# Orbiter-Finance/Plonky2-lib

Hardware: AMD Instinct MI355X
Metric: proofs/sec for secp256k1 ECDSA-verify circuit; Goldilocks NTT GB/s vs HBM peak (higher is better)
Workload: dtype u64 (Goldilocks, 64-bit modular integer)

## Files before the change

### plonky2-lib_amd/csrc/prover.hip

```cpp
#include <algorithm>
#include <string.h>
#include "batch.h"
#include "common.h"
#include "merkle.h"
#include "ntt.h"
#include "poseidon.h"
#include "prover_types.h"

namespace {
void make_layout(const glp_circuit_desc &c, Layout &L) {
    const u32 cap = 1u << c.cap_height, nch = c.num_challenges;
    memset(&L, 0, sizeof(L));
    L.oracle_cols[0] = c.num_constants + c.num_routed_wires;
    L.oracle_cols[1] = c.num_wires;
    L.oracle_cols[2] = nch * (1 + c.num_partial_products);
    L.oracle_cols[3] = nch * c.quotient_degree_factor;
    L.nopen = (size_t)c.num_constants + c.num_routed_wires + c.num_wires + 2 * nch + nch * c.num_partial_products +
              nch * c.quotient_degree_factor;
    L.openings = 3 * (size_t)cap * 4;
    L.fri_caps = L.openings + 2 * L.nopen;
    L.queries = L.fri_caps + (size_t)c.num_reductions * cap * 4;
    const u32 lgN = c.degree_bits + c.rate_bits;
    L.depth0 = lgN - c.cap_height;
    size_t q = 0;
// ... 113 lines not shown
            const u32 col = (u32)chunk < a.npp ? nch + c * a.npp + chunk : c;
            const size_t o = (size_t)col * n + i;
            const u64 v = mul(a.zp[o], ipd);
            a.zp[o] = v;
            if ((u32)chunk == a.npp) rowp[(size_t)c * n + i] = v;
            ipd = mul(ipd, dn[(size_t)chunk * n]);
        }
    }
    __syncthreads();
    if (threadIdx.x < nch) {
        const u32 c = threadIdx.x;
        u64 acc = 1;
        for (u32 i = 0; i < n; i++) { const u64 r = rowp[(size_t)c * n + i]; zrow[(size_t)c * n + i] = acc; acc = mul(acc, r); }
    }
    __syncthreads();
    for (u32 u = threadIdx.x; u < units; u += 256) {
        const u32 i = u % n, k = (u / n) % nchunks, c = u / (n * nchunks);
        const u64 z = zrow[(size_t)c * n + i];
        if (k < a.npp) { const size_t o = (size_t)(nch + c * a.npp + k) * n + i; a.zp[o] = mul(a.zp[o], z); }
        else a.zp[(size_t)c * n + i] = z;
    }
}
__global__ __launch_bounds__(256) void k_pp_block_tot(const u64 *zp, u64 *tot, u32 lg, u32 nblocks, size_t zp_stride) {
    __shared__ u64 sh[256];
    zp += (size_t)blockIdx.z * zp_stride; tot += (size_t)blockIdx.z * gridDim.y * nblocks;
    const size_t n = (size_t)1 << lg;
    const u32 c = blockIdx.y, b = blockIdx.x, t = threadIdx.x;
    const size_t i = (size_t)b * 256 + t;
    sh[t] = i < n ? zp[(size_t)c * n + i] : 1;
    __syncthreads();
    for (int s = 128; s > 0; s >>= 1) { if (t < s) sh[t] = mul(sh[t], sh[t + s]); __syncthreads(); }
    if (t == 0) tot[(size_t)c * nblocks + b] = sh[0];
}
__global__ __launch_bounds__(256) void k_pp_scan_tot(u64 *tot, u32 nblocks) {
    __shared__ u64 sh[256];
    const u32 c = blockIdx.x, t = threadIdx.x;
    u64 *v = tot + ((size_t)blockIdx.y * gridDim.x + c) * nblocks;
    const u32 m = (nblocks + 255) / 256;
    u64 loc = 1;
    for (u32 k = t * m; k < min((t + 1) * m, nblocks); k++) loc = mul(loc, v[k]);
    sh[t] = loc;
    __syncthreads();
    if (t == 0) { u64 acc = 1; for (int k = 0; k < 256; k++) { u64 x = sh[k]; sh[k] = acc; acc = mul(acc, x); } }
    __syncthreads();
    u64 acc = sh[t];
    for (u32 k = t * m; k < min((t + 1) * m, nblocks); k++) { u64 x = v[k]; v[k] = acc; acc = mul(acc, x); }
}
__global__ __launch_bounds__(256) void k_pp_apply(u64 *zp, const u64 *tot, u32 lg, u32 nblocks, u32 nch, u32 npp, size_t zp_stride) {
    __shared__ u64 sh[2][256];
    zp += (size_t)blockIdx.z * zp_stride; tot += (size_t)blockIdx.z * gridDim.y * nblocks;
    const size_t n = (size_t)1 << lg;
    const u32 c = blockIdx.y, b = blockIdx.x, t = threadIdx.x;
    const size_t i = (size_t)b * 256 + t;
    const u64 mine = i < n ? zp[(size_t)c * n + i] : 1;
    int cur = 0;
    sh[0][t] = mine;
    __syncthreads();
    for (int off = 1; off < 256; off <<= 1) {
        u64 v = sh[cur][t];
        if (t >= off) v = mul(sh[cur][t - off], v);
        sh[cur ^ 1][t] = v;
        cur ^= 1;
        __syncthreads();
    }
    const u64 excl = t ? sh[cur][t - 1] : 1;
    if (i >= n) return;
    const u64 z = mul(tot[(size_t)c * nblocks + b], excl);
    zp[(size_t)c * n + i] = z;
    for (u32 k = 0; k < npp; k++) {
        const size_t o = (size_t)(nch + c * npp + k) * n + i;
        zp[o] = mul(zp[o], z);
    }
}

__device__ __forceinline__ u64 range_product(u64 v, u32 bound) {
    if (bound == 4) {
        const u64 u = mul_nc(v, add_cnc(v, P - 3));
        return mul_nc(u, add_cnc(2, u));
    }
    u64 p = v;
    for (u32 x = 1; x + 1 < bound; x++) p = mul(p, sub(v, (u64)x));
    return bound > 1 ? mul_nc(p, sub(v, (u64)(bound - 1))) : p;
}
struct Base4Sum { u64 lo, hi; };
__device__ __forceinline__ void b4_zero(Base4Sum &b) { b.lo = 0; b.hi = 0; }
__device__ __forceinline__ void b4_add(Base4Sum &b, u64 limb, u32 j ) {
    const u32 w = 1u << (2 * j);
    b.lo += (u64)(u32)limb * w;
    b.hi += (u64)(u32)(limb >> 32) * w;
}
__device__ __forceinline__ u64 b4_value(const Base4Sum &b) {
    const u64 l = b.lo + (b.hi << 32);
    const u32 h = (u32)(b.hi >> 32) + (l < b.lo ? 1u : 0u);
    return canon(fold96_nc(l, h));
}
struct Acc160 { u32 w0, w1, w2, w3, w4; };
__device__ __forceinline__ void acc_zero(Acc160 &a) { a.w0 = a.w1 = a.w2 = a.w3 = a.w4 = 0; }
__device__ __forceinline__ void acc_fma(Acc160 &a, u64 v, u64 m) {
    const u32 v0 = (u32)v, v1 = (u32)(v >> 32), m0 = (u32)m, m1 = (u32)(m >> 32);
    const u64 p00 = (u64)v0 * m0;
    const u64 p01 = (u64)v0 * m1 + (p00 >> 32);
    const u64 p10 = (u64)v1 * m0 + (u32)p01;
    const u64 p11 = (u64)v1 * m1 + (p01 >> 32) + (p10 >> 32);
    u32 c;
    a.w0 = __builtin_addc(a.w0, (u32)p00, 0u, &c);
    a.w1 = __builtin_addc(a.w1, (u32)p10, c, &c);
    a.w2 = __builtin_addc(a.w2, (u32)p11, c, &c);
    a.w3 = __builtin_addc(a.w3, (u32)(p11 >> 32), c, &c);
    a.w4 += c;
}
__device__ __forceinline__ u64 acc_reduce(const Acc160 &a) {
    const u64 h = fold96_nc(((u64)a.w3 << 32) | a.w2, a.w4);
    return canon(fold128_nc(a.w0, a.w1, (u32)h, (u32)(h >> 32)));
}

constexpr u32 ACC_MAX_TERMS = 1024;
struct AccLimb { u64 a00, a01, a10, a11, a20, a21; };
__device__ __forceinline__ void acc2_zero(AccLimb &a) { a.a00 = a.a01 = a.a10 = a.a11 = a.a20 = a.a21 = 0; }
__device__ __forceinline__ void acc2_fma(AccLimb &a, u32 v0, u32 v1, u32 v2, u64 m) {
    const u32 m0 = (u32)m, m1 = (u32)(m >> 32);
    a.a00 += (u64)v0 * m0; a.a01 += (u64)v0 * m1;
    a.a10 += (u64)v1 * m0; a.a11 += (u64)v1 * m1;
    a.a20 += (u64)v2 * m0; a.a21 += (u64)v2 * m1;
}
template <int E> __device__ __forceinline__ void acc_add_shifted(Acc160 &w, u64 x) {
    constexpr int idx = E / 32, sh = E % 32;
    const u64 lo = x << sh;
    const u32 t0 = (u32)lo, t1 = (u32)(lo >> 32);
    u32 t2 = 0;
    if constexpr (sh != 0) t2 = (u32)(x >> (64 - sh));
    u32 *W[5] = {&w.w0, &w.w1, &w.w2, &w.w3, &w.w4};
    u32 c;
    *W[idx] = __builtin_addc(*W[idx], t0, 0u, &c);
    *W[idx + 1] = __builtin_addc(*W[idx + 1], t1, c, &c);
    *W[idx + 2] = __builtin_addc(*W[idx + 2], t2, c, &c);
    if constexpr (idx + 3 < 5) *W[idx + 3] = __builtin_addc(*W[idx + 3], 0u, c, &c);
    if constexpr (idx + 4 < 5) *W[idx + 4] = __builtin_addc(*W[idx + 4], 0u, c, &c);
}
__device__ __forceinline__ u64 acc2_reduce(const AccLimb &a) {
    Acc160 w;
    acc_zero(w);
    acc_add_shifted<0>(w, a.a00); acc_add_shifted<22>(w, a.a10); acc_add_shifted<32>(w, a.a01);
    acc_add_shifted<44>(w, a.a20); acc_add_shifted<54>(w, a.a11); acc_add_shifted<76>(w, a.a21);
    return acc_reduce(w);
}

struct AccHL { u64 c0, c1, c2; };
constexpr u32 ACC3_MAX_TERMS = 512;
inline void apl_words(u64 m, u64 out[4]) {
    const u64 mp = glf::mul(m, 1ull << 32);
    out[0] = (m & 0x3FFFFFull) | (((m >> 22) & 0x3FFFFFull) << 32); out[1] = m >> 44;
    out[2] = (mp & 0x3FFFFFull) | (((mp >> 22) & 0x3FFFFFull) << 32); out[3] = mp >> 44;
}
__device__ __forceinline__ void acc3_zero(AccHL &a) { a.c0 = a.c1 = a.c2 = 0; }
__device__ __forceinline__ void acc3_fma(AccHL &a, u64 v, const u64 *ml) {
    const u32 vlo = (u32)v, vhi = (u32)(v >> 32);
    const u64 w0 = ml[0], w1 = ml[1], w2 = ml[2], w3 = ml[3];
    a.c0 += (u64)vlo * (u32)w0; a.c1 += (u64)vlo * (u32)(w0 >> 32); a.c2 += (u64)vlo * (u32)w1;
    a.c0 += (u64)vhi * (u32)w2; a.c1 += (u64)vhi * (u32)(w2 >> 32); a.c2 += (u64)vhi * (u32)w3;
}
__device__ __forceinline__ u64 acc3_reduce(const AccHL &a) {
    Acc160 w;
    acc_zero(w);
    acc_add_shifted<0>(w, a.c0); acc_add_shifted<22>(w, a.c1); acc_add_shifted<44>(w, a.c2);
    return acc_reduce(w);
}

struct QArgs {
    const u64 *cs;
    const DevGate *gates;
    const u64 *k_is;
    u64 shift_r[MAXR], zh[MAXR], zh_inv[MAXR];
    u64 w_n, n_field;
    u32 lg, rb, step, nc, nsel, nr, nw, nch, npp, qdf, num_gates, nterms, many_selectors, gate_mode;
    u32 k_ratio;
    const u64 *l0;
};
struct QProof {
    const u64 *wl, *zl;
    u64 *out;
    const u64 *apow;
    const u64 *apl;
    u64 betas[MAXCH], gammas[MAXCH], pih[4];
};
struct QBatch { const u64 *pp; size_t wl_stride, zl_stride, out_stride, apow_stride; };
static_assert(MAXCH == 4, "pp layout: 4 betas, 4 gammas, 4 words of the public-input hash");
__device__ __forceinline__ QProof q_proof(const QProof &p0, const QBatch &b) {
    QProof p = p0;
    if (b.pp) {
        const size_t k = blockIdx.z;
        p.wl += k * b.wl_stride; p.zl += k * b.zl_stride; p.out += k * b.out_stride; p.apow += k * b.apow_stride; p.apl += APL_WORDS * k * b.apow_stride;
        const u64 *q = b.pp + k * 3 * MAXCH;
        _Pragma("unroll") for (int c = 0; c < MAXCH; c++) { p.betas[c] = q[c]; p.gammas[c] = q[MAXCH + c]; p.pih[c] = q[2 * MAXCH + c]; }
    }
    return p;
}
__global__ __launch_bounds__(256) void k_l0_table(QArgs a, u64 *out, u32 Rq) {
    const size_t n = (size_t)1 << a.lg;
    const size_t q = (size_t)blockIdx.x * 256 + threadIdx.x;
    if (q >= n) return;
    const u64 wq = dpow(a.w_n, q);
    u64 d[MAXR], pre[MAXR];
    u64 run = 1;
    for (u32 rq = 0; rq < Rq; rq++) {
        d[rq] = mul(a.n_field, sub(mul(a.shift_r[rq], wq), 1));
        pre[rq] = run;
        run = mul(run, d[rq]);
    }
    u64 iv = inv(run);
    for (int rq = (int)Rq - 1; rq >= 0; rq--) {
        out[(size_t)rq * n + q] = mul(a.zh[rq], mul(iv, pre[rq]));
        iv = mul(iv, d[rq]);
    }
}
__device__ __forceinline__ u64 gate_filter(const QArgs &a, const DevGate &g, size_t N, size_t slot) {
    const u64 s = a.cs[(size_t)g.selector_index * N + slot];
    u64 filter = 1;
    for (u32 i = g.group_start; i < g.group_end; i++)
        if (i != g.row) filter = mul(filter, sub((u64)i, s));
    if (a.many_selectors) filter = mul(filter, sub(0xFFFFFFFFull, s));
    return filter;
}
template <int NCH, int TYPE, bool HEAD_ONLY = false>
__device__ __forceinline__ void gate_terms(const QArgs &a, const QProof &p, const DevGate &g, size_t N, size_t slot, u32 k0, AccHL (&ga)[MAXCH]) {
    const u32 nt = a.nterms;
    const u64 *W = p.wl + slot;
    const u64 *GC = a.cs + (size_t)a.nsel * N + slot;
    {
        const u64 *ap = p.apl + APL_WORDS * (size_t)k0;
#define EMIT(k, v)                                                                     \
    do {                                                                               \
        const u64 _v = (v);                                                            \
        _Pragma("unroll") for (int c2 = 0; c2 < NCH; c2++) acc3_fma(ga[c2], _v, ap + APL_WORDS * ((size_t)c2 * nt + (k)));   \
    } while (0)
#define LIMBS4_DESC(LIMBS, COUNT, SPLIT, KIDX, ACCLO, ACCHI)                                                      \
    {                                                                                                             \
        Base4Sum _slo, _shi;                                                                                      \
        b4_zero(_slo); b4_zero(_shi);                                                                             \
        for (int _j0 = (int)(COUNT); _j0 > 0; _j0 -= 8) {                                                         \
            u64 _lv[8];                                                                                            \
            _Pragma("unroll") for (int _t = 0; _t < 8; _t++) if (_t < _j0) _lv[_t] = (LIMBS)[(size_t)(_j0 - 1 - _t) * N]; \
            _Pragma("unroll") for (int _t = 0; _t < 8; _t++) if (_t < _j0) {                                      \
                const int _j = _j0 - 1 - _t;                                                                      \
                EMIT((KIDX), range_product(_lv[_t], 4));                                                           \
                if (_j < (int)(SPLIT)) b4_add(_slo, _lv[_t], (u32)_j); else b4_add(_shi, _lv[_t], (u32)(_j - (int)(SPLIT))); \
            }                                                                                                     \
        }                                                                                                         \
        ACCLO = b4_value(_slo);                                                                                   \
        if ((int)(COUNT) > (int)(SPLIT)) ACCHI = b4_value(_shi);                                                  \
    }
        switch (TYPE >= 0 ? (u32)TYPE : g.type) {
        case GLP_GATE_CONSTANT:
            for (u32 i = 0; i < g.p0; i++) EMIT(i, sub(GC[(size_t)i * N], W[(size_t)i * N]));
            break;
        case GLP_GATE_PUBLIC_INPUT:
            for (u32 i = 0; i < 4; i++) EMIT(i, sub(W[(size_t)i * N], p.pih[i]));
            break;
        case GLP_GATE_ARITHMETIC: {
            const u64 c0 = GC[0], c1 = GC[N];
            for (u32 i = 0; i < g.p0; i++) {
                const u64 m0 = W[(size_t)(4 * i) * N], m1 = W[(size_t)(4 * i + 1) * N];
                const u64 ad = W[(size_t)(4 * i + 2) * N], o = W[(size_t)(4 * i + 3) * N];
                EMIT(i, sub(o, add(mul(mul(m0, m1), c0), mul(ad, c1))));
            }
            break;
        }
        case GLP_GATE_POSEIDON: {
#if defined(__HIP_DEVICE_COMPILE__)
            u32 k = 0;
            u64 st[12];
            const u64 swap = W[(size_t)24 * N];
            EMIT(k, mul_nc(swap, sub(swap, 1))); k++;
            for (u32 i = 0; i < 4; i++) {
                const u64 lhs = W[(size_t)i * N], rhs = W[(size_t)(i + 4) * N], dl = W[(size_t)(25 + i) * N];
                EMIT(k, sub(mul(swap, sub(rhs, lhs)), dl)); k++;
                st[i] = add(lhs, dl); st[i + 4] = sub(rhs, dl);
            }
            for (u32 i = 8; i < 12; i++) st[i] = W[(size_t)i * N];
            for (u32 i = 0; i < 12; i++) st[i] = add(st[i], pos::RC[i]);
            pos::sbox_layer_nc(st);
            pos::mds_add_nc(st, pos::RCN.k[0]);
            for (u32 r = 1; r < 4; r++) {
                for (u32 i = 0; i < 12; i++) { const u64 in = W[(size_t)(29 + 12 * (r - 1) + i) * N]; EMIT(k, add_cnc(neg(in), st[i])); k++; st[i] = in; }
                pos::sbox_layer_nc(st);
                if (r < 3) pos::mds_add_nc(st, pos::RCN.k[r]);
            }
            u32 pr = 0;
            auto wire_in = [&](int j, u64 z) {
                const u64 in = W[(size_t)(65 + pr + (u32)j) * N];
                EMIT(k, add_cnc(neg(in), z)); k++;
                return in;
            };
            pos::partial_block_nc<3, true>(st, pos::PBM[0], wire_in); pr += 3;
            for (int b = 0; b < 4; b++) { pos::partial_block_nc<4, false>(st, pos::PB4[b], wire_in); pr += 4; }
            pos::partial_block_nc<3, false>(st, pos::PB3[0], wire_in);
            for (u32 r = 0; r < 4; r++) {
                for (u32 i = 0; i < 12; i++) { const u64 in = W[(size_t)(87 + 12 * r + i) * N]; EMIT(k, add_cnc(neg(in), st[i])); k++; st[i] = in; }
                pos::sbox_layer_nc(st);
                pos::mds_add_nc(st, r < 3 ? pos::RCN.k[4 + r] : pos::RC_ZERO);
            }
            for (u32 i = 0; i < 12; i++) { EMIT(k, add_cnc(neg(W[(size_t)(12 + i) * N]), st[i])); k++; }
#endif
            break;
        }
        case GLP_GATE_U32_INTERLEAVE: {
            u32 k = 0;
            for (u32 i = 0; i < g.p0; i++) {
                const u64 xw = W[(size_t)(2 * i) * N], xi = W[(size_t)(2 * i + 1) * N];
                const u64 *bits = W + (size_t)(2 * g.p0 + 32 * i) * N;
                u64 cx = 0, cxi = 0;
                const u32 kb = k + 2;
                for (u32 b = 0; b < 32; b++) {
                    const u64 bit = bits[(size_t)b * N];
                    cx = add(dbl(cx), bit);
                    cxi = add(dbl(dbl(cxi)), bit);
                    EMIT(kb + b, mul_nc(bit, sub(bit, 1)));
                }
                EMIT(k, sub(cx, xw));
                EMIT(k + 1, sub(cxi, xi));
                k += 34;
            }
            break;
        }
        case GLP_GATE_UNINTERLEAVE_U32:
        case GLP_GATE_UNINTERLEAVE_B32: {
            u32 k = 0;
            for (u32 i = 0; i < g.p0; i++) {
                const u64 xi = W[(size_t)(3 * i) * N], xe = W[(size_t)(3 * i + 1) * N], xo = W[(size_t)(3 * i + 2) * N];
                const u64 *bits = W + (size_t)(3 * g.p0 + 64 * i) * N;
                u64 cxi = 0, ce = 0, co = 0;
                const u32 kb = k + 3;
                for (u32 j = 0; j < 32; j++) {
                    const u64 be = bits[(size_t)(2 * j) * N], bo = bits[(size_t)(2 * j + 1) * N];
                    cxi = add(dbl(add(dbl(cxi), be)), bo);
                    if (g.type == GLP_GATE_UNINTERLEAVE_U32) { ce = add(dbl(ce), be); co = add(dbl(co), bo); }
                    else { ce = add(dbl(dbl(ce)), be); co = add(dbl(dbl(co)), bo); }
                    EMIT(kb + 2 * j, mul_nc(be, sub(be, 1)));
                    EMIT(kb + 2 * j + 1, mul_nc(bo, sub(bo, 1)));
                }
                EMIT(k, sub(cxi, xi));
                EMIT(k + 1, sub(ce, xe));
                EMIT(k + 2, sub(co, xo));
                k += 67;
            }
// ... 142 lines not shown
                        l2[q4] = add(f0, mul(b1, sub(f1, f0)));
                    }
                    const u64 g0 = add(l2[0], mul(b2, sub(l2[1], l2[0]))), g1 = add(l2[2], mul(b2, sub(l2[3], l2[2])));
                    sel = add(g0, mul(b3, sub(g1, g0)));
                } else {
                    for (u32 b = 0; b < bits; b++) { const u64 bit = bw[(size_t)b * N]; EMIT(k, mul_nc(bit, sub(bit, 1))); k++; }
                    for (int b = (int)bits - 1; b >= 0; b--) idx = add(dbl(idx), bw[(size_t)b * N]);
                    EMIT(k, sub(idx, bse[0])); k++;
                    sel = 0;
                    for (u32 j = 0; j < vs; j++) {
                        u64 ind = 1;
                        for (u32 b = 0; b < bits; b++) { const u64 bit = bw[(size_t)b * N]; ind = mul(ind, ((j >> b) & 1) ? bit : sub(1, bit)); }
                        sel = add(sel, mul(ind, bse[(size_t)(2 + j) * N]));
                    }
                }
                EMIT(k, sub(sel, bse[N])); k++;
            }
            for (u32 e = 0; e < nextra; e++) { EMIT(k, sub(GC[(size_t)e * N], W[(size_t)((2 + vs) * copies + e) * N])); k++; }
            break;
        }
        default: break;
        }
#undef LIMBS4_DESC
#undef EMIT
    }
}
template <int NCH, int TYPE>
__device__ __forceinline__ void gate_contrib(const QArgs &a, const QProof &p, const DevGate &g, size_t N, size_t slot, u32 k0, u64 (&acc)[MAXCH]) {
    const u64 filter = gate_filter(a, g, N, slot);
    AccHL ga[MAXCH];
    _Pragma("unroll") for (int c = 0; c < NCH; c++) acc3_zero(ga[c]);
    gate_terms<NCH, TYPE, false>(a, p, g, N, slot, k0, ga);
    _Pragma("unroll") for (int c = 0; c < NCH; c++) acc[c] = add(acc[c], mul(filter, acc3_reduce(ga[c])));
}

struct LightArgs { u32 count; u32 gi[8]; u32 arith_gi, arith_ops; };
template <int NCH>
__device__ __forceinline__ void light_gates(const QArgs &a, const QProof &p, const LightArgs &la, size_t N, size_t slot, u32 k0, u64 (&acc)[MAXCH]) {
    for (u32 t = 0; t < la.count; t++) {
        const DevGate g = a.gates[la.gi[t]];
        switch (g.type) {
        case GLP_GATE_CONSTANT: gate_contrib<NCH, GLP_GATE_CONSTANT>(a, p, g, N, slot, k0, acc); break;
        case GLP_GATE_PUBLIC_INPUT: gate_contrib<NCH, GLP_GATE_PUBLIC_INPUT>(a, p, g, N, slot, k0, acc); break;
        case GLP_GATE_ARITHMETIC: gate_contrib<NCH, GLP_GATE_ARITHMETIC>(a, p, g, N, slot, k0, acc); break;
        case GLP_GATE_BASE_SUM: gate_contrib<NCH, GLP_GATE_BASE_SUM>(a, p, g, N, slot, k0, acc); break;
        case GLP_GATE_RANDOM_ACCESS: gate_contrib<NCH, GLP_GATE_RANDOM_ACCESS>(a, p, g, N, slot, k0, acc); break;
        default: break;
        }
    }
}
template <int NCH, int GATES>
__global__ __launch_bounds__(256, GATES == 1 ? 3 : 4) void k_quotient(QArgs a, QProof p0, QBatch qb, LightArgs la) {
    const QProof p = q_proof(p0, qb);
    const size_t n = (size_t)1 << a.lg, N = n << a.rb;
    const size_t q = (size_t)blockIdx.x * 256 + threadIdx.x;
    if (q >= n) return;
    const u32 rq = blockIdx.y, r = rq * a.step;
    const size_t slot = (size_t)r * n + q, slot_next = (size_t)r * n + ((q + 1) & (n - 1));
    const u64 x = mul(a.shift_r[rq], dpow(a.w_n, q));
    constexpr u32 nch = NCH; const u32 nchunks = a.npp + 1, nt = a.nterms;
    u64 acc[MAXCH], zx[MAXCH], zg[MAXCH];
    Acc160 pa[MAXCH];
    _Pragma("unroll") for (int c = 0; c < NCH; c++) { acc_zero(pa[c]); zx[c] = p.zl[(size_t)c * N + slot]; zg[c] = p.zl[(size_t)c * N + slot_next]; }
    const u64 l0 = a.l0[(size_t)rq * n + q];
    _Pragma("unroll") for (int c = 0; c < NCH; c++) {
        const u64 t = mul(l0, sub(zx[c], 1));
        _Pragma("unroll") for (int c2 = 0; c2 < NCH; c2++) acc_fma(pa[c2], t, p.apow[c2 * nt + c]);
    }
    u64 bkx[MAXCH];
    _Pragma("unroll") for (int c = 0; c < NCH; c++) bkx[c] = mul_nc(p.betas[c], x);
    const u32 k0 = nch + nch * nchunks;
    const u32 ar_ops = GATES == 2 ? la.arith_ops : 0;
    AccHL gar[MAXCH];
    u64 ar_c0 = 0, ar_c1 = 0;
    if (GATES == 2) {
        _Pragma("unroll") for (int c = 0; c < NCH; c++) acc3_zero(gar[c]);
        if (ar_ops) { ar_c0 = a.cs[(size_t)a.nsel * N + slot]; ar_c1 = a.cs[(size_t)(a.nsel + 1) * N + slot]; }
    }
    for (u32 chunk = 0; chunk < nchunks; chunk++) {
        u64 num[MAXCH], den[MAXCH];
        _Pragma("unroll") for (int c = 0; c < NCH; c++) { num[c] = 1; den[c] = 1; }
        const u32 j0 = chunk * a.qdf, j1 = min((chunk + 1) * a.qdf, a.nr);
        for (u32 jb = j0; jb < j1; jb += 8) {
            u64 w8[8], s8[8];
#pragma unroll
            for (int t = 0; t < 8; t++)
                if (jb + t < j1) { w8[t] = p.wl[(size_t)(jb + t) * N + slot]; s8[t] = a.cs[(size_t)(a.nc + jb + t) * N + slot]; }
            if (GATES == 2 && ar_ops) {
#pragma unroll
                for (int t = 0; t < 8; t += 4)
                    if (jb + t + 3 < j1 && (jb + t) / 4 < ar_ops) {
                        const u32 i = (jb + t) / 4;
                        const u64 v = sub(w8[t + 3], add(mul(mul(w8[t], w8[t + 1]), ar_c0), mul(w8[t + 2], ar_c1)));
                        _Pragma("unroll") for (int c2 = 0; c2 < NCH; c2++) acc3_fma(gar[c2], v, p.apl + APL_WORDS * ((size_t)c2 * nt + k0 + i));
                    }
            }
#pragma unroll
            for (int t = 0; t < 8; t++)
                if (jb + t < j1) {
                    u64 kx = 0;
                    if (!a.k_ratio) kx = mul_nc(a.k_is[jb + t], x);
                    _Pragma("unroll") for (int c = 0; c < NCH; c++) {
                        const u64 wg = add(w8[t], p.gammas[c]);
                        const u64 bk = a.k_ratio ? bkx[c] : mul_nc(p.betas[c], kx);
                        num[c] = mul_nc_cc(num[c], add_cnc(wg, bk));
                        den[c] = mul_nc_cc(den[c], add_cnc(wg, mul_nc_cc(p.betas[c], s8[t])));
                        if (a.k_ratio) bkx[c] = mul_small_nc(bkx[c], a.k_ratio);
                    }
                }
        }
        _Pragma("unroll") for (int c = 0; c < NCH; c++) {
            const u64 prev = chunk == 0 ? zx[c] : p.zl[(size_t)(nch + c * a.npp + chunk - 1) * N + slot];
            const u64 next = chunk == nchunks - 1 ? zg[c] : p.zl[(size_t)(nch + c * a.npp + chunk) * N + slot];
            const u64 t = sub(mul(prev, num[c]), mul(next, den[c]));
            const u32 k = nch + c * nchunks + chunk;
            _Pragma("unroll") for (int c2 = 0; c2 < NCH; c2++) acc_fma(pa[c2], t, p.apow[c2 * nt + k]);
        }
    }
    _Pragma("unroll") for (int c = 0; c < NCH; c++) acc[c] = acc_reduce(pa[c]);
    if (GATES == 2 && ar_ops) {
        const u64 filter = gate_filter(a, a.gates[la.arith_gi], N, slot);
        _Pragma("unroll") for (int c = 0; c < NCH; c++) acc[c] = add(acc[c], mul(filter, acc3_reduce(gar[c])));
    }
    if constexpr (GATES == 1) {
        for (u32 gi = 0; gi < a.num_gates; gi++) {
            const DevGate g = a.gates[gi];
            gate_contrib<NCH, -1>(a, p, g, N, slot, k0, acc);
        }
    }
    if constexpr (GATES == 2) light_gates<NCH>(a, p, la, N, slot, k0, acc);
    const size_t Rq = (size_t)gridDim.y;
    _Pragma("unroll") for (int c = 0; c < NCH; c++) p.out[((size_t)c * Rq + rq) * n + q] = mul(acc[c], a.zh_inv[rq]);
}

template <int NCH, int TYPE>
__global__ __launch_bounds__(256) void k_quotient_gate(QArgs a, QProof p0, QBatch qb, u32 gi) {
    const QProof p = q_proof(p0, qb);
    const size_t n = (size_t)1 << a.lg, N = n << a.rb;
    const size_t q = (size_t)blockIdx.x * 256 + threadIdx.x;
    if (q >= n) return;
    const u32 rq = blockIdx.y, r = rq * a.step;
    const size_t slot = (size_t)r * n + q;
    u64 acc[MAXCH];
    _Pragma("unroll") for (int c = 0; c < NCH; c++) acc[c] = 0;
    const DevGate g = a.gates[gi];
    gate_contrib<NCH, TYPE>(a, p, g, N, slot, (u32)NCH + (u32)NCH * (a.npp + 1), acc);
    const size_t Rq = (size_t)gridDim.y;
    _Pragma("unroll") for (int c = 0; c < NCH; c++) {
        u64 *o = p.out + ((size_t)c * Rq + rq) * n + q;
        *o = add(*o, mul(acc[c], a.zh_inv[rq]));
    }
}

constexpr int LIMB_SLOTS = 5, LIMB_GROUPS = 4;
struct LimbArgs { const u64 *desc; u32 groups, num_wires; u32 count[LIMB_GROUPS], jlo[LIMB_GROUPS], jhi[LIMB_GROUPS]; u32 gi[LIMB_GROUPS][LIMB_SLOTS]; u32 extra_count, extra_gi[4]; };
inline void limb_args(const glp_circuit *cc, LimbArgs &la) {
    la.desc = cc->dev_limb_desc; la.groups = cc->limb_groups; la.num_wires = cc->d.num_wires;
    for (int g = 0; g < LIMB_GROUPS; g++) {
        la.count[g] = cc->limb_gcount[g]; la.jlo[g] = cc->limb_jlo[g]; la.jhi[g] = cc->limb_jhi[g];
        for (int i = 0; i < LIMB_SLOTS; i++) la.gi[g][i] = cc->limb_gi[g * LIMB_SLOTS + i];
    }
}
template <int NCH>
__global__ __launch_bounds__(256, 2) void k_quotient_limbs(QArgs a, QProof p0, QBatch qb, LimbArgs la) {
    const QProof p = q_proof(p0, qb);
    const size_t n = (size_t)1 << a.lg, N = n << a.rb;
    const size_t q = (size_t)blockIdx.x * 256 + threadIdx.x;
    if (q >= n) return;
    const u32 rq = blockIdx.y, r = rq * a.step;
    const size_t slot = (size_t)r * n + q;
    const u32 k0 = (u32)NCH + (u32)NCH * (a.npp + 1), nt = a.nterms;
    const u64 *W = p.wl + slot;
    const u64 *ap = p.apl + APL_WORDS * (size_t)k0;
    u64 acc[MAXCH];
    _Pragma("unroll") for (int c = 0; c < NCH; c++) acc[c] = 0;
#define LIMB_EMIT(S, K, V)                                                                                     \
    do {                                                                                                       \
        const u64 _v = (V);                                                                                    \
        _Pragma("unroll") for (int c2 = 0; c2 < NCH; c2++) acc3_fma(ga[S][c2], _v, ap + APL_WORDS * ((size_t)c2 * nt + (K)));   \
    } while (0)
#pragma unroll 1
    for (u32 grp = 0; grp < la.groups; grp++) {
        const u32 gcount = la.count[grp], jlo = la.jlo[grp], jhi = la.jhi[grp];
        const u64 *desc = la.desc + (size_t)grp * la.num_wires * LIMB_SLOTS;
        AccHL ga[LIMB_SLOTS][MAXCH];
        Base4Sum bs[LIMB_SLOTS];
        _Pragma("unroll") for (int s = 0; s < LIMB_SLOTS; s++) {
            b4_zero(bs[s]);
            _Pragma("unroll") for (int c = 0; c < NCH; c++) acc3_zero(ga[s][c]);
        }
        _Pragma("unroll") for (int s = 0; s < LIMB_SLOTS; s++) {
            if ((u32)s < gcount) {
                const DevGate g = a.gates[la.gi[grp][s]];
                switch (g.type) {
                case GLP_GATE_U32_ARITHMETIC: gate_terms<NCH, GLP_GATE_U32_ARITHMETIC, true>(a, p, g, N, slot, k0, ga[s]); break;
                case GLP_GATE_U32_ADD_MANY: gate_terms<NCH, GLP_GATE_U32_ADD_MANY, true>(a, p, g, N, slot, k0, ga[s]); break;
                case GLP_GATE_U32_SUBTRACTION: gate_terms<NCH, GLP_GATE_U32_SUBTRACTION, true>(a, p, g, N, slot, k0, ga[s]); break;
                default: break;
                }
            }
        }
        for (u32 j0 = jlo; j0 <= jhi; j0 += 8) {
            u64 lv[8];
            _Pragma("unroll") for (int t = 0; t < 8; t++) if (j0 + t <= jhi) lv[t] = W[(size_t)(j0 + t) * N];
            _Pragma("unroll") for (int t = 0; t < 8; t++) if (j0 + t <= jhi) {
                const u64 v = lv[t];
                const u64 *dj = desc + (size_t)(j0 + t) * LIMB_SLOTS;
                const u64 rp = range_product(v, 4);
                _Pragma("unroll") for (int s = 0; s < LIMB_SLOTS; s++) {
                    const u64 d = dj[s];
                    if (d & 1) {
                        const u32 kl = (u32)(d >> 6) & 0x3FFu;
                        _Pragma("unroll") for (int c2 = 0; c2 < NCH; c2++) acc3_fma(ga[s][c2], rp, ap + APL_WORDS * ((size_t)c2 * nt + kl));
                        b4_add(bs[s], v, (u32)(d >> 1) & 15u);
                        if (d & 32) {
                            const u32 kf = (u32)(d >> 16) & 0x3FFu, ref = (u32)(d >> 26) & 0xFFu;
                            LIMB_EMIT(s, kf, sub(b4_value(bs[s]), W[(size_t)ref * N]));
                            b4_zero(bs[s]);
                        }
                    }
                }
            }
        }
        _Pragma("unroll") for (int s = 0; s < LIMB_SLOTS; s++) {
            if ((u32)s < gcount) {
                const u64 filter = gate_filter(a, a.gates[la.gi[grp][s]], N, slot);
                _Pragma("unroll") for (int c = 0; c < NCH; c++) acc[c] = add(acc[c], mul(filter, acc3_reduce(ga[s][c])));
            }
        }
    }
#undef LIMB_EMIT
    for (u32 t = 0; t < la.extra_count; t++) {
        const DevGate g = a.gates[la.extra_gi[t]];
        if (g.type == GLP_GATE_COMPARISON) gate_contrib<NCH, GLP_GATE_COMPARISON>(a, p, g, N, slot, k0, acc);
    }
    const size_t Rq = (size_t)gridDim.y;
    _Pragma("unroll") for (int c = 0; c < NCH; c++) {
        u64 *o = p.out + ((size_t)c * Rq + rq) * n + q;
        *o = add(*o, mul(acc[c], a.zh_inv[rq]));
    }
}

struct QCArgs { const u64 *V; u64 *out; u64 wM_inv, wR_inv, g_inv, rq_inv; u64 gn_inv_pow[MAXR]; u32 lg, Rq; };
__global__ __launch_bounds__(256) void k_quotient_combine(QCArgs a) {
    const size_t n = (size_t)1 << a.lg;
    const size_t p = (size_t)blockIdx.x * 256 + threadIdx.x;
    if (p >= n) return;
    const u32 ch = blockIdx.y, Rq = a.Rq;
    const u32 kp = bitrev32((u32)p, a.lg);
    const u64 tw = dpow(a.wM_inv, kp);
    const u64 gk = mul(dpow(a.g_inv, kp), a.rq_inv);
    u64 y[MAXR];
    u64 t = 1;
    for (u32 r = 0; r < Rq; r++) { y[r] = mul(a.V[((size_t)ch * Rq + r) * n + p], t); t = mul(t, tw); }
    u64 wc = 1;
    for (u32 c = 0; c < Rq; c++) {
        u64 s = 0, w = 1;
        for (u32 r = 0; r < Rq; r++) { s = add(s, mul(y[r], w)); w = mul(w, wc); }
        a.out[((size_t)ch * Rq + c) * n + p] = mul(s, mul(gk, a.gn_inv_pow[c]));
        wc = mul(wc, a.wR_inv);
    }
}

struct ZTArgs { u64 *zt; ext2 zp2[24]; u32 lg; const u64 *zeta_b; size_t zeta_stride; };
template <bool BATCH>
__global__ __launch_bounds__(256) void k_zeta_table(ZTArgs a) {
    const size_t n = (size_t)1 << a.lg;
    const size_t p = (size_t)blockIdx.x * 256 + threadIdx.x;
    if (p >= n) return;
    const u32 k = bitrev32((u32)p, a.lg);
    ext2 acc = e_from(1);
    if constexpr (BATCH) {
        const u64 *z = a.zeta_b + (size_t)blockIdx.y * a.zeta_stride;
        ext2 sq = e_make(z[0], z[1]);
        for (u32 b = 0; b < a.lg; b++) { if ((k >> b) & 1) acc = e_mul(acc, sq); sq = e_sqr(sq); }
        a.zt += (size_t)blockIdx.y * 2 * n;
    } else {
        for (u32 b = 0; b < a.lg; b++) if ((k >> b) & 1) acc = e_mul(acc, a.zp2[b]);
    }
    a.zt[2 * p] = acc.a; a.zt[2 * p + 1] = acc.b;
}
constexpr int OPEN_BLOCKS = 32;
inline u32 open_blocks(size_t n) { return (u32)std::max<size_t>(1, std::min<size_t>(OPEN_BLOCKS, n / 256)); }
__global__ __launch_bounds__(256) void k_open_dot(const u64 *coeffs, const u64 *zt, u64 *partial, u32 lg, size_t coeffs_bstride,
                                                  size_t zt_bstride, size_t partial_bstride) {
    __shared__ u64 sa[256], sb[256];
    coeffs += (size_t)blockIdx.z * coeffs_bstride; zt += (size_t)blockIdx.z * zt_bstride; partial += (size_t)blockIdx.z * partial_bstride;
    const size_t n = (size_t)1 << lg;
    const u32 col = blockIdx.y, t = threadIdx.x;
    u64 a = 0, b = 0;
    AccLimb xa, xb;
    acc2_zero(xa); acc2_zero(xb);
    u32 terms = 0;
    for (size_t p = (size_t)blockIdx.x * 256 + t; p < n; p += (size_t)gridDim.x * 256) {
        const u64 c = coeffs[(size_t)col * n + p];
        const u32 c0 = (u32)c & 0x3FFFFFu, c1 = (u32)(c >> 22) & 0x3FFFFFu, c2 = (u32)(c >> 44);
        acc2_fma(xa, c0, c1, c2, zt[2 * p]);
        acc2_fma(xb, c0, c1, c2, zt[2 * p + 1]);
        if (++terms == ACC_MAX_TERMS) {
            a = add(a, acc2_reduce(xa)); b = add(b, acc2_reduce(xb));
            acc2_zero(xa); acc2_zero(xb); terms = 0;
        }
    }
    a = add(a, acc2_reduce(xa)); b = add(b, acc2_reduce(xb));
    sa[t] = a; sb[t] = b;
    __syncthreads();
    for (int s = 128; s > 0; s >>= 1) { if (t < s) { sa[t] = add(sa[t], sa[t + s]); sb[t] = add(sb[t], sb[t + s]); } __syncthreads(); }
    if (t == 0) { partial[2 * ((size_t)col * gridDim.x + blockIdx.x)] = sa[0]; partial[2 * ((size_t)col * gridDim.x + blockIdx.x) + 1] = sb[0]; }
}

struct FVArgs {
    const u64 *lde[4]; u32 ncols[4];
    const u64 *apow;
    u64 *out;
    ext2 red0, red1, zeta, zeta_next, shift_acc;
    u64 w_n, g;
    u32 lg, rb, nch;
    const u64 *pp;
    size_t lde_stride[4], apow_stride, out_stride;
};
__global__ __launch_bounds__(256) void k_final_values(FVArgs a) {
    const size_t n = (size_t)1 << a.lg, N = n << a.rb;
    const size_t q = (size_t)blockIdx.x * 256 + threadIdx.x;
    if (q >= n) return;
    if (a.pp) {
        const size_t pk = blockIdx.y;
        const u64 *v = a.pp + pk * 10;
        a.red0 = e_make(v[0], v[1]); a.red1 = e_make(v[2], v[3]); a.zeta = e_make(v[4], v[5]); a.zeta_next = e_make(v[6], v[7]);
        a.shift_acc = e_make(v[8], v[9]);
        _Pragma("unroll") for (int k = 0; k < 4; k++) a.lde[k] += pk * a.lde_stride[k];
        a.apow += pk * a.apow_stride; a.out += pk * a.out_stride;
    }
    ext2 acc0 = e_from(0), acc1 = e_from(0);
    AccLimb xa, xb;
    acc2_zero(xa); acc2_zero(xb);
    u32 j = 0, terms = 0;
    for (int k = 0; k < 4; k++) {
        const u64 *l = a.lde[k] + q;
        for (u32 c = 0; c < a.ncols[k]; c++, j++) {
            const u64 v = l[(size_t)c * N];
            const u32 v0 = (u32)v & 0x3FFFFFu, v1 = (u32)(v >> 22) & 0x3FFFFFu, v2 = (u32)(v >> 44);
            acc2_fma(xa, v0, v1, v2, a.apow[2 * j]);
            acc2_fma(xb, v0, v1, v2, a.apow[2 * j + 1]);
            if (++terms == ACC_MAX_TERMS) {
                acc0 = e_add(acc0, e_make(acc2_reduce(xa), acc2_reduce(xb)));
                acc2_zero(xa); acc2_zero(xb); terms = 0;
            }
            if (k == 2 && c < a.nch) {
                const ext2 ap1 = e_make(a.apow[2 * c], a.apow[2 * c + 1]);
                acc1 = e_add(acc1, e_scale(ap1, v));
            }
        }
    }
    acc0 = e_add(acc0, e_make(acc2_reduce(xa), acc2_reduce(xb)));
    const u64 x = mul(a.g, dpow(a.w_n, q));
    const ext2 d0 = e_inv(e_sub(e_from(x), a.zeta)), d1 = e_inv(e_sub(e_from(x), a.zeta_next));
    ext2 f = e_mul(e_mul(e_sub(acc0, a.red0), d0), a.shift_acc);
    f = e_add(f, e_mul(e_sub(acc1, a.red1), d1));
    a.out[q] = f.a; a.out[n + q] = f.b;
}

__global__ __launch_bounds__(256) void k_final_values_small(FVArgs a) {
    const u32 n = 1u << a.lg, lpp = 256u >> a.lg;
    const size_t N = (size_t)n << a.rb;
    const u32 q = threadIdx.x / lpp, t = threadIdx.x % lpp;
    if (a.pp) {
        const size_t pk = blockIdx.y;
        const u64 *v = a.pp + pk * 10;
        a.red0 = e_make(v[0], v[1]); a.red1 = e_make(v[2], v[3]); a.zeta = e_make(v[4], v[5]); a.zeta_next = e_make(v[6], v[7]);
        a.shift_acc = e_make(v[8], v[9]);
        _Pragma("unroll") for (int k = 0; k < 4; k++) a.lde[k] += pk * a.lde_stride[k];
        a.apow += pk * a.apow_stride; a.out += pk * a.out_stride;
    }
    ext2 acc0 = e_from(0), acc1 = e_from(0);
    AccLimb xa, xb;
    acc2_zero(xa); acc2_zero(xb);
    u32 base = 0;
    for (int k = 0; k < 4; k++) {
        const u64 *l = a.lde[k] + q;
        for (u32 c = t; c < a.ncols[k]; c += lpp) {
            const u32 j = base + c;
            const u64 v = l[(size_t)c * N];
            const u32 v0 = (u32)v & 0x3FFFFFu, v1 = (u32)(v >> 22) & 0x3FFFFFu, v2 = (u32)(v >> 44);
            acc2_fma(xa, v0, v1, v2, a.apow[2 * j]);
            acc2_fma(xb, v0, v1, v2, a.apow[2 * j + 1]);
            if (k == 2 && c < a.nch) acc1 = e_add(acc1, e_scale(e_make(a.apow[2 * c], a.apow[2 * c + 1]), v));
        }
        base += a.ncols[k];
    }
    acc0 = e_make(acc2_reduce(xa), acc2_reduce(xb));
    for (u32 m = lpp >> 1; m >= 1; m >>= 1) {
        acc0 = e_add(acc0, e_make(pos::shfl_xor64(acc0.a, (int)m), pos::shfl_xor64(acc0.b, (int)m)));
// ... 274 lines not shown
    ~BatchHolder() { batch_destroy(b); }
};
inline unsigned nblk(size_t n) { return (unsigned)((n + 255) / 256); }
int pow_batch_launch(glp_ctx *c, Tmp &tmp, const u64 *dev_pst, const u32 *dev_ppos, u32 bits, u64 *dev_best, u64 *dev_next, u32 K) {
    u64 *dev_k;
    GLP_TRY(tmp.get(&dev_k, (size_t)K * 12 + 1));
    hipLaunchKernelGGL(k_pow_prepare, dim3((K + 63) / 64), dim3(64), 0, c->stream, dev_pst, dev_ppos, dev_k, K);
    GLP_HIP(hipGetLastError());
    constexpr u32 CHUNKS = 8;
    const double expected = (double)K * (bits >= 8 ? (double)(1ull << (bits - 8)) : 1.0);
    const u32 tail = (u32)c->num_cus * 4;
    const u32 body = (u32)std::min<double>(4.0 * expected / CHUNKS + 1.0, (double)(1u << 22));
    hipLaunchKernelGGL(k_pow_batch2, dim3(body + tail), dim3(256), 0, c->stream, dev_k, dev_ppos, bits,
                       (unsigned long long *)dev_best, (unsigned long long *)dev_next, K, CHUNKS, body);
    GLP_HIP(hipGetLastError());
    return GLP_OK;
}
int d2h(glp_ctx *c, void *dst, const void *src, size_t bytes) {
    GLP_HIP(hipMemcpyAsync(dst, src, bytes, hipMemcpyDeviceToHost, c->stream));
    GLP_HIP(hipStreamSynchronize(c->stream));
    return GLP_OK;
}
int h2d(glp_ctx *c, void *dst, const void *src, size_t bytes) {
    GLP_HIP(hipMemcpyAsync(dst, src, bytes, hipMemcpyHostToDevice, c->stream));
    GLP_HIP(hipStreamSynchronize(c->stream));
    return GLP_OK;
}
int batch_cap_host(glp_ctx *c, const glp_batch *b, std::vector<u64> &cap) {
    const size_t N = (size_t)1 << (b->lg + b->rate_bits);
    cap.resize((size_t)4 << b->cap_height);
    return d2h(c, cap.data(), b->digests + 4 * merkle_cap_offset(N, b->cap_height), cap.size() * 8);
}
int open_batch_launch(glp_ctx *c, const glp_batch *b, const u64 *dev_zt, u64 *dev_partial, u32 first_cols = 0 ) {
    dim3 g(open_blocks((size_t)1 << b->lg), first_cols ? first_cols : b->ncols);
    hipLaunchKernelGGL(k_open_dot, g, dim3(256), 0, c->stream, b->coeffs, dev_zt, dev_partial, (u32)b->lg, (size_t)0, (size_t)0, (size_t)0);
    GLP_HIP(hipGetLastError());
    return GLP_OK;
}
void open_batch_finish(const u64 *h, u32 ncols, u32 nob, std::vector<ext2> &out) {
    out.resize(ncols);
    for (u32 col = 0; col < ncols; col++) {
        u64 a = 0, bb = 0;
        for (u32 k = 0; k < nob; k++) { a = add(a, h[2 * ((size_t)col * nob + k)]); bb = add(bb, h[2 * ((size_t)col * nob + k) + 1]); }
        out[col] = e_make(a, bb);
    }
}
int zeta_table(glp_ctx *c, ext2 z, int lg, u64 *dev_zt) {
    ZTArgs za;
    za.zt = dev_zt; za.lg = (u32)lg; za.zeta_b = nullptr; za.zeta_stride = 0;
    ext2 p = z;
    for (int b = 0; b < 24; b++) { za.zp2[b] = p; p = e_sqr(p); }
    hipLaunchKernelGGL(HIP_KERNEL_NAME(k_zeta_table<false>), dim3(nblk((size_t)1 << lg)), dim3(256), 0, c->stream, za);
    GLP_HIP(hipGetLastError());
    return GLP_OK;
}
}

struct glp_session {
    glp_ctx *c;
    const glp_circuit *cc;
    const glp_circuit_desc &d;
    const Layout &L;
    const int lg, rb;
    const size_t n, N;
    const u32 nch, nr, nw, nc, qdf, npp, capn, nzp;
    const int hasher;
    Tmp tmp;
    u64 *owned_wires = nullptr;
    const u64 *dev_wires = nullptr;
    u64 pih[4] = {0, 0, 0, 0};
    BatchHolder wb, zb, qb;
    u64 betas[MAXCH] = {}, gammas[MAXCH] = {}, alphas[MAXCH] = {};
    ext2 zeta = {0, 0}, zeta_next = {0, 0};
    const glp_batch *ob[4] = {nullptr, nullptr, nullptr, nullptr};
    std::vector<ext2> open[4], zs_next;
    u64 *fcoef = nullptr;
    struct Layer { u64 *vals; u64 *dig; u32 lgL, ab; };
    std::vector<Layer> layers;
    u64 *cur = nullptr;
    int lgcur = 0;
    u64 shift = GEN;
    bool layer_open = false;
    std::vector<u64> proof_words;
    std::vector<u64> cap;
    enum Stage { S_NEW, S_WIRES, S_ZS, S_QUOTIENT, S_OPEN, S_FRI, S_FINAL, S_DONE } stage = S_NEW;

    glp_session(glp_ctx *ctx, const glp_circuit *circ)
        : c(ctx), cc(circ), d(circ->d), L(circ->L), lg((int)circ->d.degree_bits), rb((int)circ->d.rate_bits),
          n((size_t)1 << circ->d.degree_bits), N(((size_t)1 << circ->d.degree_bits) << circ->d.rate_bits),
          nch(circ->d.num_challenges), nr(circ->d.num_routed_wires), nw(circ->d.num_wires), nc(circ->d.num_constants),
          qdf(circ->d.quotient_degree_factor), npp(circ->d.num_partial_products), capn(1u << circ->d.cap_height),
          nzp(circ->d.num_challenges * (1 + circ->d.num_partial_products)), hasher((int)circ->d.hasher), tmp(ctx) {}
    ~glp_session() { if (owned_wires) { (void)hipStreamSynchronize(c->stream); c->release(owned_wires); } }
    u64 *proof() { return proof_words.data(); }

    int begin(const u64 *wires_dev, const u64 *public_inputs, const u64 *host_wires = nullptr) {
        GLP_REQUIRE(stage == S_NEW, "session already begun");
        proof_words.assign(L.total, 0);
        dev_wires = wires_dev;
        host_hash_no_pad(public_inputs, d.num_public_inputs, pih);
        if (d.num_public_inputs) memcpy(proof() + L.pis, public_inputs, (size_t)d.num_public_inputs * 8);
        GLP_TRY(batch_build(c, dev_wires, BATCH_VALUES, nw, lg, rb, (int)d.cap_height, &wb.b, host_wires, 1, hasher));
        GLP_TRY(batch_cap_host(c, wb.b, cap));
        memcpy(proof() + L.caps, cap.data(), capn * 32);
        stage = S_WIRES;
        return GLP_OK;
    }
    int partial_products(const u64 *betas_in, const u64 *gammas_in) {
        GLP_REQUIRE(stage == S_WIRES, "partial_products: call after begin");
        for (u32 i = 0; i < nch; i++) { betas[i] = betas_in[i]; gammas[i] = gammas_in[i]; }
        u64 *zp, *tot;
        const u32 nblocks = nblk(n);
        u64 *dens;
        GLP_TRY(tmp.get(&zp, (size_t)nzp * n));
        GLP_TRY(tmp.get(&dens, (size_t)nzp * n));
        GLP_TRY(tmp.get(&tot, (size_t)nch * nblocks));
        {
            StageScope st(c, "partial_products", 8.0 * n * (2.0 * nr + nzp));
            PPArgs a;
            a.wires = dev_wires; a.sigmas = cc->dev_sigmas; a.k_is = cc->dev_k_is; a.zp = zp; a.dens = dens;
            for (u32 i = 0; i < nch; i++) { a.betas[i] = betas[i]; a.gammas[i] = gammas[i]; }
            a.w_n = root_of_unity(lg); a.lg = (u32)lg; a.nr = nr; a.nch = nch; a.npp = npp; a.qdf = qdf;
            a.chal = nullptr; a.wires_stride = 0; a.zp_stride = 0;
            const size_t small_lds = (size_t)2 * nch * (npp + 2) * n * sizeof(u64);
            const bool small = lg <= 7 && small_lds <= 64 * 1024;
            if (small) hipLaunchKernelGGL(k_pp_rows_small, dim3(1, 1), dim3(256), small_lds, c->stream, a);
            else switch (nch) {
            case 1: hipLaunchKernelGGL(HIP_KERNEL_NAME(k_pp_rows<1>), dim3(nblocks), dim3(256), 0, c->stream, a); break;
            case 2: hipLaunchKernelGGL(HIP_KERNEL_NAME(k_pp_rows<2>), dim3(nblocks), dim3(256), 0, c->stream, a); break;
            case 3: hipLaunchKernelGGL(HIP_KERNEL_NAME(k_pp_rows<3>), dim3(nblocks), dim3(256), 0, c->stream, a); break;
            default: hipLaunchKernelGGL(HIP_KERNEL_NAME(k_pp_rows<4>), dim3(nblocks), dim3(256), 0, c->stream, a); break;
            }
            GLP_HIP(hipGetLastError());
            if (!small) {
                hipLaunchKernelGGL(k_pp_block_tot, dim3(nblocks, nch), dim3(256), 0, c->stream, zp, tot, (u32)lg, nblocks, (size_t)0);
                hipLaunchKernelGGL(k_pp_scan_tot, dim3(nch), dim3(256), 0, c->stream, tot, nblocks);
                hipLaunchKernelGGL(k_pp_apply, dim3(nblocks, nch), dim3(256), 0, c->stream, zp, tot, (u32)lg, nblocks, nch, npp, (size_t)0);
                GLP_HIP(hipGetLastError());
            }
        }
        GLP_TRY(batch_build(c, zp, BATCH_VALUES, nzp, lg, rb, (int)d.cap_height, &zb.b, nullptr, 1, hasher));
        GLP_TRY(batch_cap_host(c, zb.b, cap));
        memcpy(proof() + L.caps + capn * 4, cap.data(), capn * 32);
        stage = S_ZS;
        return GLP_OK;
    }
    int quotient(const u64 *alphas_in) {
        GLP_REQUIRE(stage == S_ZS, "quotient: call after partial_products");
        for (u32 i = 0; i < nch; i++) alphas[i] = alphas_in[i];
        int qdb = 0;
        while ((1u << qdb) < qdf) qdb++;
        const u32 Rq = 1u << qdb, step = 1u << (rb - qdb);
        const u32 nchunks = npp + 1, nterms = nch + nch * nchunks + d.num_gate_constraints;
        std::vector<u64> apow((size_t)(1 + APL_WORDS) * nch * nterms);
        for (u32 i = 0; i < nch; i++) {
            u64 x = 1;
            for (u32 k = 0; k < nterms; k++) {
                const size_t e = (size_t)i * nterms + k;
                apow[e] = x;
                apl_words(x, &apow[(size_t)nch * nterms + APL_WORDS * e]);
                x = mul(x, alphas[i]);
            }
        }
        u64 *dev_apow, *qv, *qV, *qc;
        GLP_TRY(tmp.get(&dev_apow, apow.size()));
        GLP_TRY(h2d(c, dev_apow, apow.data(), apow.size() * 8));
        GLP_TRY(tmp.get(&qv, (size_t)nch * Rq * n));
        GLP_TRY(tmp.get(&qV, (size_t)nch * Rq * n));
        GLP_TRY(tmp.get(&qc, (size_t)nch * Rq * n));
        QArgs a;
        QProof qp;
        QBatch qbt;
        memset(&qp, 0, sizeof(qp));
        memset(&qbt, 0, sizeof(qbt));
        a.cs = cc->cs->lde; qp.wl = wb.b->lde; qp.zl = zb.b->lde; qp.out = qv;
        a.gates = cc->dev_gates; a.k_is = cc->dev_k_is; qp.apow = dev_apow; qp.apl = dev_apow + (size_t)nch * nterms; a.k_ratio = cc->k_ratio;
        for (u32 i = 0; i < nch; i++) { qp.betas[i] = betas[i]; qp.gammas[i] = gammas[i]; }
        memcpy(qp.pih, pih, 32);
        const u64 WN = root_of_unity(lg + rb), gn = pow(GEN, (u64)n), wR = root_of_unity(rb);
        for (u32 rq = 0; rq < Rq; rq++) {
            const u32 r = rq * step;
            a.shift_r[rq] = mul(GEN, pow(WN, (u64)r));
            a.zh[rq] = sub(mul(gn, pow(wR, (u64)r)), 1);
            a.zh_inv[rq] = inv(a.zh[rq]);
        }
        a.w_n = root_of_unity(lg); a.n_field = (u64)n % P;
        a.lg = (u32)lg; a.rb = (u32)rb; a.step = step; a.nc = nc; a.nsel = d.num_selectors; a.nr = nr; a.nw = nw;
        a.nch = nch; a.npp = npp; a.qdf = qdf; a.num_gates = d.num_gates; a.nterms = nterms;
        a.many_selectors = d.num_selectors > 1;
        {
            StageScope st(c, "quotient_eval", 8.0 * n * Rq * (nc + nr + nw + nzp + 2.0 * nch));
            a.gate_mode = nch == 2 ? 1 : 0;
            u64 *l0t;
            GLP_TRY(tmp.get(&l0t, (size_t)Rq * n));
            a.l0 = l0t;
            hipLaunchKernelGGL(k_l0_table, dim3(nblk(n)), dim3(256), 0, c->stream, a, l0t, Rq);
            GLP_HIP(hipGetLastError());
            LightArgs lg_;
            lg_.count = cc->light_count; lg_.arith_gi = cc->arith_gi; lg_.arith_ops = cc->arith_ops;
            for (u32 i = 0; i < 8; i++) lg_.gi[i] = cc->light_gi[i];
            switch (nch) {
            case 1: hipLaunchKernelGGL(HIP_KERNEL_NAME(k_quotient<1, 1>), dim3(nblk(n), Rq), dim3(256), 0, c->stream, a, qp, qbt, lg_); break;
            case 2:
                if (cc->light_count || cc->arith_ops) hipLaunchKernelGGL(HIP_KERNEL_NAME(k_quotient<2, 2>), dim3(nblk(n), Rq), dim3(256), 0, c->stream, a, qp, qbt, lg_);
                else hipLaunchKernelGGL(HIP_KERNEL_NAME(k_quotient<2, 0>), dim3(nblk(n), Rq), dim3(256), 0, c->stream, a, qp, qbt, lg_);
                break;
            case 3: hipLaunchKernelGGL(HIP_KERNEL_NAME(k_quotient<3, 1>), dim3(nblk(n), Rq), dim3(256), 0, c->stream, a, qp, qbt, lg_); break;
            default: hipLaunchKernelGGL(HIP_KERNEL_NAME(k_quotient<4, 1>), dim3(nblk(n), Rq), dim3(256), 0, c->stream, a, qp, qbt, lg_); break;
            }
            GLP_HIP(hipGetLastError());
            if (a.gate_mode == 1) {
                if (cc->limb_count) {
                    LimbArgs la;
                    limb_args(cc, la);
                    la.extra_count = cc->limb_extra_count;
                    for (int i = 0; i < 4; i++) la.extra_gi[i] = cc->limb_extra_gi[i];
                    hipLaunchKernelGGL(HIP_KERNEL_NAME(k_quotient_limbs<2>), dim3(nblk(n), Rq), dim3(256), 0, c->stream, a, qp, qbt, la);
                    GLP_HIP(hipGetLastError());
                }
                for (u32 gi : cc->single_gates) {
#define GLP_GATE_LAUNCH(T) case T: hipLaunchKernelGGL(HIP_KERNEL_NAME(k_quotient_gate<2, T>), dim3(nblk(n), Rq), dim3(256), 0, c->stream, a, qp, qbt, gi); break;
                    switch (cc->gates[gi].type) {
                        GLP_GATE_LAUNCH(GLP_GATE_CONSTANT) GLP_GATE_LAUNCH(GLP_GATE_PUBLIC_INPUT) GLP_GATE_LAUNCH(GLP_GATE_ARITHMETIC)
                        GLP_GATE_LAUNCH(GLP_GATE_POSEIDON) GLP_GATE_LAUNCH(GLP_GATE_U32_INTERLEAVE) GLP_GATE_LAUNCH(GLP_GATE_UNINTERLEAVE_U32)
                        GLP_GATE_LAUNCH(GLP_GATE_UNINTERLEAVE_B32) GLP_GATE_LAUNCH(GLP_GATE_U32_ARITHMETIC) GLP_GATE_LAUNCH(GLP_GATE_U32_ADD_MANY)
                        GLP_GATE_LAUNCH(GLP_GATE_U32_SUBTRACTION) GLP_GATE_LAUNCH(GLP_GATE_U32_RANGE_CHECK) GLP_GATE_LAUNCH(GLP_GATE_COMPARISON)
                        GLP_GATE_LAUNCH(GLP_GATE_BASE_SUM) GLP_GATE_LAUNCH(GLP_GATE_RANDOM_ACCESS)
                    default: break;
                    }
#undef GLP_GATE_LAUNCH
                    GLP_HIP(hipGetLastError());
                }
            }
            GLP_HIP(hipGetLastError());
        }
        {
            StageScope st(c, "quotient_intt", 16.0 * n * Rq * nch);
            GLP_TRY(intt_values_to_coeffs(c, qv, qV, nch * Rq, lg));
            QCArgs q;
            q.V = qV; q.out = qc; q.lg = (u32)lg; q.Rq = Rq;
            q.wM_inv = inv(root_of_unity(lg + qdb)); q.wR_inv = inv(root_of_unity(qdb)); q.g_inv = inv(GEN);
            q.rq_inv = inv((u64)Rq);
            const u64 gni = inv(gn);
            u64 x = 1;
            for (u32 cidx = 0; cidx < Rq; cidx++) { q.gn_inv_pow[cidx] = x; x = mul(x, gni); }
            hipLaunchKernelGGL(k_quotient_combine, dim3(nblk(n), nch), dim3(256), 0, c->stream, q);
            GLP_HIP(hipGetLastError());
        }
        GLP_TRY(batch_build(c, qc, BATCH_COEFFS_BITREV, nch * qdf, lg, rb, (int)d.cap_height, &qb.b, nullptr, 1, hasher));
        GLP_TRY(batch_cap_host(c, qb.b, cap));
        memcpy(proof() + L.caps + 2 * capn * 4, cap.data(), capn * 32);
        stage = S_QUOTIENT;
        return GLP_OK;
    }
    int open_at(ext2 zeta_in) {
        GLP_REQUIRE(stage == S_QUOTIENT, "open: call after quotient");
        zeta = zeta_in;
        {
            ext2 zp = zeta;
            for (int i = 0; i < lg; i++) zp = e_sqr(zp);
            if (e_eq(zp, e_from(1))) return set_error(GLP_ERR_PROVE, "Opening point is in the subgroup.");
        }
        zeta_next = e_scale(zeta, root_of_unity(lg));
        ob[0] = cc->cs; ob[1] = wb.b; ob[2] = zb.b; ob[3] = qb.b;
        {
        StageScope st(c, "openings", 8.0 * n * (L.oracle_cols[0] + L.oracle_cols[1] + L.oracle_cols[2] + L.oracle_cols[3] + nch));
        u64 *zt, *partial;
        GLP_TRY(tmp.get(&zt, 2 * n));
        const u32 nob = open_blocks(n);
        size_t poff[6] = {0, 0, 0, 0, 0, 0};
        for (int k = 0; k < 5; k++) poff[k + 1] = poff[k] + (size_t)(k < 4 ? ob[k]->ncols : nch) * nob * 2;
        GLP_TRY(tmp.get(&partial, poff[5]));
        GLP_TRY(zeta_table(c, zeta, lg, zt));
        for (int k = 0; k < 4; k++) GLP_TRY(open_batch_launch(c, ob[k], zt, partial + poff[k]));
        GLP_TRY(zeta_table(c, zeta_next, lg, zt));
        GLP_TRY(open_batch_launch(c, zb.b, zt, partial + poff[4], nch));
        std::vector<u64> hp(poff[5]);
        GLP_TRY(d2h(c, hp.data(), partial, hp.size() * 8));
        for (int k = 0; k < 4; k++) open_batch_finish(hp.data() + poff[k], ob[k]->ncols, nob, open[k]);
        std::vector<ext2> all;
        open_batch_finish(hp.data() + poff[4], nch, nob, all);
        zs_next.assign(all.begin(), all.begin() + nch);
    }
        {
            u64 *op = proof() + L.openings;
            size_t o = 0;
            auto put = [&](ext2 e) { op[o++] = e.a; op[o++] = e.b; };
            for (u32 k = 0; k < nc + nr; k++) put(open[0][k]);
            for (u32 k = 0; k < nw; k++) put(open[1][k]);
            for (u32 k = 0; k < nch; k++) put(open[2][k]);
            for (u32 k = 0; k < nch; k++) put(zs_next[k]);
            for (u32 k = 0; k < nch * npp; k++) put(open[2][nch + k]);
            for (u32 k = 0; k < nch * qdf; k++) put(open[3][k]);
        }
        stage = S_OPEN;
        return GLP_OK;
    }
    int fri_combine(ext2 alpha) {
        GLP_REQUIRE(stage == S_OPEN, "fri_combine: call after open");
        GLP_TRY(tmp.get(&fcoef, 2 * n));
    {
        StageScope st(c, "fri_combine", 8.0 * n * (L.oracle_cols[0] + L.oracle_cols[1] + L.oracle_cols[2] + L.oracle_cols[3]));
        size_t total_cols = 0;
        for (int k = 0; k < 4; k++) total_cols += ob[k]->ncols;
        std::vector<u64> ap(2 * total_cols);
        ext2 x = e_from(1), red0 = e_from(0), red1 = e_from(0);
        size_t j = 0;
        for (int k = 0; k < 4; k++)
            for (u32 col = 0; col < ob[k]->ncols; col++, j++) {
                ap[2 * j] = x.a; ap[2 * j + 1] = x.b;
                red0 = e_add(red0, e_mul(x, open[k][col]));
                x = e_mul(x, alpha);
            }
        x = e_from(1);
        for (u32 col = 0; col < nch; col++) { red1 = e_add(red1, e_mul(x, zs_next[col])); x = e_mul(x, alpha); }
        u64 *dev_ap, *fv;
        GLP_TRY(tmp.get(&dev_ap, ap.size()));
        GLP_TRY(h2d(c, dev_ap, ap.data(), ap.size() * 8));
        GLP_TRY(tmp.get(&fv, 2 * n));
        FVArgs a;
        for (int k = 0; k < 4; k++) { a.lde[k] = ob[k]->lde; a.ncols[k] = ob[k]->ncols; }
        a.apow = dev_ap; a.out = fv; a.red0 = red0; a.red1 = red1; a.zeta = zeta; a.zeta_next = zeta_next;
        a.shift_acc = e_pow(alpha, nch);
        a.w_n = root_of_unity(lg); a.g = GEN; a.lg = (u32)lg; a.rb = (u32)rb; a.nch = nch;
        a.pp = nullptr; a.apow_stride = a.out_stride = 0;
        for (int k = 0; k < 4; k++) a.lde_stride[k] = 0;
        if (lg >= 2 && lg <= 7) hipLaunchKernelGGL(k_final_values_small, dim3(1, 1), dim3(256), 0, c->stream, a);
        else hipLaunchKernelGGL(k_final_values, dim3(nblk(n)), dim3(256), 0, c->stream, a);
        GLP_HIP(hipGetLastError());
        GLP_TRY(intt_values_to_coeffs(c, fv, fcoef, 2, lg));
        hipLaunchKernelGGL(k_scale_bitrev_pow, dim3(nblk(n), 2), dim3(256), 0, c->stream, fcoef, inv(GEN), (u32)lg);
        GLP_HIP(hipGetLastError());
    }

        cur = fcoef; lgcur = lg; shift = GEN;
        stage = S_FRI;
        return GLP_OK;
    }
    int fri_commit_layer() {
        GLP_REQUIRE(stage == S_FRI && !layer_open && layers.size() < d.num_reductions, "fri_commit: no layer left or beta pending");
        StageScope st(c, "fri_commit", 0.0);
        const u32 r = (u32)layers.size();
        const u32 ab = d.reduction_arity_bits[r];
        const u32 lgL = (u32)(lgcur + rb);
        const size_t Lsz = (size_t)1 << lgL, nleaves = Lsz >> ab;
        Layer ly;
        ly.lgL = lgL; ly.ab = ab;
        GLP_TRY(tmp.get(&ly.vals, 2 * Lsz));
        GLP_TRY(tmp.get(&ly.dig, merkle_num_digests(nleaves, (int)d.cap_height) * 4));
        GLP_TRY(lde_coeffs(c, cur, ly.vals, 2, lgcur, rb, shift));
        if (hasher == GLP_HASH_KECCAK25)
            hipLaunchKernelGGL(k_fri_leaf_hash_keccak, dim3(nblk(nleaves)), dim3(256), 0, c->stream, ly.vals, ly.dig, lgL, (u32)rb, ab, (size_t)0,
                               (size_t)0);
        else if (nleaves <= c->merkle_coop_max)
            hipLaunchKernelGGL(k_fri_leaf_hash_coop, dim3((unsigned)((nleaves + 15) / 16)), dim3(256), 0, c->stream, ly.vals, ly.dig, lgL,
                               (u32)rb, ab, (size_t)0, (size_t)0);
        else if (nleaves <= c->merkle_quad_max)
            hipLaunchKernelGGL(k_fri_leaf_hash_quad, dim3((unsigned)((nleaves + 63) / 64)), dim3(256), 0, c->stream, ly.vals, ly.dig, lgL,
                               (u32)rb, ab, (size_t)0, (size_t)0);
        else
            hipLaunchKernelGGL(k_fri_leaf_hash, dim3(nblk(nleaves)), dim3(256), 0, c->stream, ly.vals, ly.dig, lgL, (u32)rb, ab, (size_t)0,
                               (size_t)0);
        GLP_HIP(hipGetLastError());
        GLP_TRY(merkle_levels(c, ly.dig, nleaves, (int)d.cap_height, 1, 0, hasher));
        cap.resize((size_t)capn * 4);
        GLP_TRY(d2h(c, cap.data(), ly.dig + 4 * merkle_cap_offset(nleaves, (int)d.cap_height), (size_t)capn * 32));
        memcpy(proof() + L.fri_caps + (size_t)r * capn * 4, cap.data(), (size_t)capn * 32);
        layers.push_back(ly);
        layer_open = true;
// ... 20 lines not shown
        std::vector<u64> h(2 * fl);
        GLP_TRY(d2h(c, h.data(), cur, h.size() * 8));
        for (size_t p = 0; p < fl; p++) {
            const size_t k = bitrev32((u32)p, lgcur);
            proof()[L.final_poly + 2 * k] = h[p];
            proof()[L.final_poly + 2 * k + 1] = h[fl + p];
        }
        stage = S_FINAL;
        return GLP_OK;
    }
    int queries(u64 pow_witness, const u64 *indices, u32 nq) {
        GLP_REQUIRE(stage == S_FINAL, "queries: call after fri_final_poly");
        GLP_REQUIRE(nq == d.num_query_rounds, "queries: %u indices, the circuit has %u query rounds", nq, d.num_query_rounds);
        proof()[L.pow] = pow_witness;
        StageScope st(c, "fri_queries", 0.0);
        std::vector<u64> xi(indices, indices + nq);
        for (u32 q = 0; q < nq; q++) GLP_REQUIRE(xi[q] < (u64)N, "query index %llu outside the LDE domain", (unsigned long long)xi[q]);
        u64 *dev_idx, *dev_q;
        const size_t stride = L.query_stride;
        GLP_TRY(tmp.get(&dev_idx, nq));
        GLP_TRY(tmp.get(&dev_q, (size_t)nq * stride));
        GLP_TRY(h2d(c, dev_idx, xi.data(), nq * 8));
        size_t off = 0;
        for (int k = 0; k < 4; k++) {
            const u32 ncol = ob[k]->ncols;
            GLP_TRY(merkle_gather_lde_rows(c, ob[k]->lde, ncol, lg, rb, dev_idx, nq, dev_q + off, stride));
            off += ncol;
            GLP_TRY(merkle_gather_paths(c, ob[k]->digests, N, (int)d.cap_height, dev_idx, nq, dev_q + off, stride, 0));
            off += 4 * (size_t)L.depth0;
        }
        u32 shift_bits = 0;
        for (size_t r = 0; r < layers.size(); r++) {
            const Layer &ly = layers[r];
            const u32 arity = 1u << ly.ab;
            const size_t nleaves = ((size_t)1 << ly.lgL) >> ly.ab;
            shift_bits += ly.ab;
            hipLaunchKernelGGL(k_fri_gather_leaf, dim3(nblk((size_t)nq * arity)), dim3(256), 0, c->stream, ly.vals, ly.lgL, (u32)rb,
                               ly.ab, dev_idx, shift_bits, nq, dev_q + off, stride, (size_t)0, (size_t)0);
            GLP_HIP(hipGetLastError());
            off += 2 * (size_t)arity;
            GLP_TRY(merkle_gather_paths(c, ly.dig, nleaves, (int)d.cap_height, dev_idx, nq, dev_q + off, stride, shift_bits));
            off += 4 * (size_t)L.step_depth[r];
        }
        if (off != stride) return set_error(GLP_ERR_ARG, "internal: query record layout mismatch");
        GLP_TRY(d2h(c, proof() + L.queries, dev_q, (size_t)nq * stride * 8));
        stage = S_DONE;
        return GLP_OK;
    }
};

constexpr u32 POW_MAX_BITS = 32;
static int pow_search(glp_ctx *c, const u64 st[12], const u64 *pending, u32 npending, u32 bits, u64 *witness, int hasher = GLP_HASH_POSEIDON) {
    StageScope stg(c, "fri_pow", 0.0);
    GLP_REQUIRE(npending < 8, "proof of work: %u pending inputs (the rate is 8)", npending);
    PowArgs a;
    memcpy(a.st, st, 96);
    for (u32 i = 0; i < npending; i++) a.st[i] = pending[i];
    a.pos = npending; a.bits = bits;
    Tmp tmp(c);
    u64 *best;
    GLP_TRY(tmp.get(&best, 1));
    a.best = (unsigned long long *)best;
    const u64 none = ~0ull;
    u64 found = none;
    const u64 batch = 1ull << std::min<u32>(20, std::max<u32>(14, bits + 2));
    for (u64 base = 0; found == none; base += batch) {
        if (base >= (1ull << 40)) return set_error(GLP_ERR_PROVE, "Proof of work failed. This is highly unlikely!");
        GLP_TRY(h2d(c, best, &none, 8));
        a.base = base;
        if (hasher == GLP_HASH_KECCAK25) hipLaunchKernelGGL(HIP_KERNEL_NAME(k_pow<GLP_HASH_KECCAK25>), dim3((unsigned)(batch / 256)), dim3(256), 0, c->stream, a);
        else hipLaunchKernelGGL(HIP_KERNEL_NAME(k_pow<GLP_HASH_POSEIDON>), dim3((unsigned)(batch / 256)), dim3(256), 0, c->stream, a);
        GLP_HIP(hipGetLastError());
        GLP_TRY(d2h(c, &found, best, 8));
    }
    *witness = found;
    return GLP_OK;
}

static int prove_impl(glp_ctx *c, const glp_circuit *cc, const u64 *dev_wires, const u64 *public_inputs, u64 *proof,
                      const u64 *host_wires = nullptr) {
    glp_session s(c, cc);
    const glp_circuit_desc &d = cc->d;
    const Layout &L = cc->L;
    const u32 nch = s.nch, nr = s.nr, nw = s.nw, nc = s.nc, qdf = s.qdf, npp = s.npp, capn = s.capn;
    GLP_TRY(s.begin(dev_wires, public_inputs, host_wires));
    Challenger ch((int)d.hasher);
    ch.observe_hashes(cc->digest, 1);
    ch.observe(s.pih, 4);
    ch.observe_hashes(s.cap.data(), capn);
    u64 betas[MAXCH], gammas[MAXCH], alphas[MAXCH];
    for (u32 i = 0; i < nch; i++) betas[i] = ch.get();
    for (u32 i = 0; i < nch; i++) gammas[i] = ch.get();
    GLP_TRY(s.partial_products(betas, gammas));
    ch.observe_hashes(s.cap.data(), capn);
    for (u32 i = 0; i < nch; i++) alphas[i] = ch.get();
    GLP_TRY(s.quotient(alphas));
    ch.observe_hashes(s.cap.data(), capn);
    GLP_TRY(s.open_at(ch.get_ext()));
    {
        const u64 *op = s.proof() + L.openings;
        const u64 *p_cs = op, *p_w = op + 2 * (nc + nr), *p_zs = p_w + 2 * nw, *p_zn = p_zs + 2 * nch;
        const u64 *p_pp = p_zn + 2 * nch, *p_q = p_pp + 2 * nch * npp;
        ch.observe(p_cs, 2 * (nc + nr)); ch.observe(p_w, 2 * nw); ch.observe(p_zs, 2 * nch);
        ch.observe(p_pp, 2 * (size_t)nch * npp); ch.observe(p_q, 2 * (size_t)nch * qdf); ch.observe(p_zn, 2 * nch);
    }
    GLP_TRY(s.fri_combine(ch.get_ext()));
    for (u32 r = 0; r < d.num_reductions; r++) {
        GLP_TRY(s.fri_commit_layer());
        ch.observe_hashes(s.cap.data(), capn);
        GLP_TRY(s.fri_fold(ch.get_ext()));
    }
    GLP_TRY(s.fri_final_poly());
    ch.observe(s.proof() + L.final_poly, 2 * L.final_len);
    u64 found;
    GLP_TRY(pow_search(c, ch.st, ch.in, (u32)ch.nin, d.proof_of_work_bits, &found, (int)d.hasher));
    ch.observe(&found, 1);
    const u64 resp = ch.get();
    if (d.proof_of_work_bits && (resp >> (64 - d.proof_of_work_bits)) != 0)
        return set_error(GLP_ERR_PROVE, "proof-of-work response check failed");
    std::vector<u64> xi(d.num_query_rounds);
    for (u32 q = 0; q < d.num_query_rounds; q++) xi[q] = ch.get() % (u64)s.N;
    GLP_TRY(s.queries(found, xi.data(), d.num_query_rounds));
    memcpy(proof, s.proof(), L.total * 8);
    return GLP_OK;
}

namespace {
enum { PW_FIELD = 0, PW_DIGESTS = 1, PW_PATH = 2 };
template <class F> void walk_proof(const glp_circuit *cc, F f) {
    const Layout &L = cc->L;
    const glp_circuit_desc &d = cc->d;
    f((size_t)0, L.openings, PW_DIGESTS);
    f(L.openings, L.fri_caps - L.openings, PW_FIELD);
    f(L.fri_caps, L.queries - L.fri_caps, PW_DIGESTS);
    for (u32 q = 0; q < d.num_query_rounds; q++) {
        size_t o = L.queries + (size_t)q * L.query_stride;
        for (int k = 0; k < 4; k++) {
            f(o, (size_t)L.oracle_cols[k], PW_FIELD); o += L.oracle_cols[k];
            f(o, 4 * (size_t)L.depth0, PW_PATH); o += 4 * (size_t)L.depth0;
        }
        for (u32 r = 0; r < d.num_reductions; r++) {
            const size_t ev = (size_t)2 << d.reduction_arity_bits[r];
            f(o, ev, PW_FIELD); o += ev;
            f(o, 4 * (size_t)L.step_depth[r], PW_PATH); o += 4 * (size_t)L.step_depth[r];
        }
    }
    f(L.final_poly, L.total - L.final_poly, PW_FIELD);
}
}


static int build_quotient_plan(glp_ctx *c, glp_circuit *cc) {
    const glp_circuit_desc &d = cc->d;
    std::vector<u64> desc((size_t)LIMB_GROUPS * d.num_wires * LIMB_SLOTS, 0);
    for (int g = 0; g < LIMB_GROUPS; g++) { cc->limb_jlo[g] = d.num_wires; cc->limb_jhi[g] = 0; }
    auto put = [&](u32 s, u32 col, u32 pos, u32 kl, bool flush, u32 kf, u32 ref) {
        const u32 grp = s / LIMB_SLOTS, slot = s % LIMB_SLOTS;
        desc[((size_t)grp * d.num_wires + col) * LIMB_SLOTS + slot] = 1ull | ((u64)pos << 1) | (flush ? 32ull : 0ull) | ((u64)kl << 6) | ((u64)kf << 16) | ((u64)ref << 26);
        cc->limb_jlo[grp] = std::min(cc->limb_jlo[grp], col); cc->limb_jhi[grp] = std::max(cc->limb_jhi[grp], col);
    };
    std::vector<u32> limb_list;
    auto fill = [&](u32 s, u32 gi) {
        const glp_gate &g = cc->gates[gi];
        cc->limb_gi[s] = gi;
        if (g.type == GLP_GATE_U32_ARITHMETIC) {
            for (u32 i = 0; i < g.p0; i++)
                for (u32 j = 0; j < 32; j++)
                    put(s, 6 * g.p0 + 32 * i + j, j & 15, 36 * i + 2 + (31 - j), (j & 15) == 15, 36 * i + 34 + (j >> 4), 6 * i + 3 + (j >> 4));
        } else if (g.type == GLP_GATE_U32_ADD_MANY) {
            const u32 na = g.p0, nops = g.p1, wd = na + 3;
            for (u32 i = 0; i < nops; i++)
                for (u32 j = 0; j < 18; j++)
                    put(s, wd * nops + 18 * i + j, j & 15, 21 * i + 1 + (17 - j), j == 15 || j == 17, 21 * i + 19 + (j >> 4), wd * i + na + 1 + (j >> 4));
        } else if (g.type == GLP_GATE_U32_SUBTRACTION) {
            for (u32 i = 0; i < g.p0; i++)
                for (u32 j = 0; j < 16; j++)
                    put(s, 5 * g.p0 + 16 * i + j, j, 19 * i + 1 + (15 - j), j == 15, 19 * i + 17, 5 * i + 3);
        } else {
            for (u32 i = 0; i < g.p0; i++)
                for (u32 j = 0; j < 16; j++)
                    put(s, g.p0 + 16 * i + j, j, 17 * i + 1 + j, j == 15, 17 * i, i);
        }
    };
    auto limb_weight = [&](u32 gi) -> u32 {
        const glp_gate &g = cc->gates[gi];
        return g.type == GLP_GATE_U32_ARITHMETIC ? 32 * g.p0 : g.type == GLP_GATE_U32_ADD_MANY ? 18 * g.p1 : 16 * g.p0;
    };
    for (u32 gi = 0; gi < d.num_gates; gi++) {
        const glp_gate &g = cc->gates[gi];
        const bool limb_gate = g.type == GLP_GATE_U32_ARITHMETIC || g.type == GLP_GATE_U32_ADD_MANY ||
                               g.type == GLP_GATE_U32_SUBTRACTION || g.type == GLP_GATE_U32_RANGE_CHECK;
        const bool light = g.type == GLP_GATE_CONSTANT || g.type == GLP_GATE_PUBLIC_INPUT || g.type == GLP_GATE_ARITHMETIC ||
                           g.type == GLP_GATE_BASE_SUM || g.type == GLP_GATE_RANDOM_ACCESS;
        if (limb_gate && limb_list.size() < (size_t)(LIMB_SLOTS * LIMB_GROUPS) && d.num_wires <= 256) {
            limb_list.push_back(gi);
        } else if (g.type == GLP_GATE_ARITHMETIC && cc->arith_ops == 0 && 4 * g.p0 <= d.num_routed_wires && d.quotient_degree_factor % 4 == 0 &&
                   d.num_selectors + 2 <= d.num_constants) {
            cc->arith_gi = gi; cc->arith_ops = g.p0;
        } else if (light && cc->light_count < 8) {
            cc->light_gi[cc->light_count++] = gi;
        } else if (g.type != GLP_GATE_NOOP) {
            cc->single_gates.push_back(gi);
        }
    }
    if (limb_list.size() == 1) {
        cc->single_gates.push_back(limb_list[0]);
        limb_list.clear();
    }
    if (!limb_list.empty()) {
        const u32 cnt = (u32)limb_list.size();
        const u32 G = (cnt + LIMB_SLOTS - 1) / LIMB_SLOTS;
        u32 used[LIMB_GROUPS] = {0, 0, 0, 0};
        auto limb_start = [&](u32 gi) -> u32 {
            const glp_gate &g = cc->gates[gi];
            return g.type == GLP_GATE_U32_ARITHMETIC ? 6 * g.p0 : g.type == GLP_GATE_U32_ADD_MANY ? (g.p0 + 3) * g.p1 : g.type == GLP_GATE_U32_SUBTRACTION ? 5 * g.p0 : g.p0;
        };
        std::stable_sort(limb_list.begin(), limb_list.end(), [&](u32 x, u32 y) {
            return limb_start(x) != limb_start(y) ? limb_start(x) < limb_start(y) : limb_weight(x) > limb_weight(y); });
        for (u32 t = 0; t < cnt; t++) {
            const u32 grp = t / LIMB_SLOTS;
            fill(grp * LIMB_SLOTS + used[grp], limb_list[t]);
            used[grp]++;
        }
        cc->limb_count = cnt; cc->limb_groups = G;
        for (u32 g = 0; g < G; g++) cc->limb_gcount[g] = used[g];
    }
    if (cc->limb_count) {
        std::vector<u32> keep;
        for (u32 gi : cc->single_gates) {
            if (cc->gates[gi].type == GLP_GATE_COMPARISON && cc->limb_extra_count < 4) cc->limb_extra_gi[cc->limb_extra_count++] = gi;
            else keep.push_back(gi);
        }
        cc->single_gates.swap(keep);
    }
    if (cc->limb_count) {
        GLP_TRY(c->alloc((void **)&cc->dev_limb_desc, desc.size() * 8));
        GLP_TRY(h2d(c, cc->dev_limb_desc, desc.data(), desc.size() * 8));
    }
    return GLP_OK;
}

extern "C" {

void glp_circuit_free(glp_circuit *cc) {
    if (!cc) return;
    glp_ctx *c = cc->ctx;
    (void)hipSetDevice(c->device);
    (void)hipStreamSynchronize(c->stream);
    batch_destroy(cc->cs);
    c->release(cc->dev_sigmas);
    c->release(cc->dev_k_is);
    c->release(cc->dev_gates);
    c->release(cc->dev_limb_desc);
    c->release(cc->dev_consts);
    delete cc;
}

int glp_circuit_create(glp_ctx *c, const glp_circuit_desc *desc, glp_circuit **out) {
    GLP_REQUIRE(c && desc && out, "null argument");
    *out = nullptr;
    GLP_TRY(bind(c));
    const glp_circuit_desc &d = *desc;
    GLP_REQUIRE(d.gates && d.k_is && d.constants && d.sigmas, "null array in circuit description");
    GLP_REQUIRE(d.num_challenges >= 1 && d.num_challenges <= (u32)MAXCH, "num_challenges=%u outside 1..%d", d.num_challenges, MAXCH);
    if (d.hasher != GLP_HASH_POSEIDON && d.hasher != GLP_HASH_KECCAK25) return set_error(GLP_ERR_UNSUPPORTED, "hasher %u is not one of GLP_HASH_*", d.hasher);
    GLP_REQUIRE(d.rate_bits >= 1 && d.rate_bits <= 4, "rate_bits=%u outside 1..4", d.rate_bits);
    GLP_REQUIRE(d.num_routed_wires <= d.num_wires && d.num_routed_wires > 0, "bad wire counts");
    if ((int)d.degree_bits > NTT_MAX_LG) return set_error(GLP_ERR_UNSUPPORTED, "degree_bits=%u > %d", d.degree_bits, NTT_MAX_LG);
    const u32 qdf = d.quotient_degree_factor;
    if (qdf == 0 || (qdf & (qdf - 1)) || qdf > (1u << d.rate_bits))
        return set_error(GLP_ERR_UNSUPPORTED, "quotient_degree_factor=%u must be a power of two <= 2^rate_bits", qdf);
    GLP_REQUIRE(d.num_partial_products == (d.num_routed_wires + qdf - 1) / qdf - 1, "num_partial_products inconsistent");
    GLP_REQUIRE(d.num_reductions <= 16 && d.cap_height <= d.degree_bits + d.rate_bits, "bad FRI parameters");
    GLP_REQUIRE(d.proof_of_work_bits <= POW_MAX_BITS, "proof_of_work_bits=%u: this build searches at most 2^40 candidates and accepts up to %u bits",
                d.proof_of_work_bits, POW_MAX_BITS);
    u32 sum_ab = 0;
    for (u32 i = 0; i < d.num_reductions; i++) {
        GLP_REQUIRE(d.reduction_arity_bits[i] >= 1 && d.reduction_arity_bits[i] <= 5, "arity_bits outside 1..5");
        sum_ab += d.reduction_arity_bits[i];
        GLP_REQUIRE(sum_ab <= d.degree_bits && d.degree_bits + d.rate_bits - sum_ab >= d.cap_height, "FRI reduction deeper than the domain");
    }
    auto gate_shape = [](const glp_gate &g, u32 &wires, u32 &consts, u32 &constraints) -> bool {
        const u32 p0 = g.p0, p1 = g.p1;
        consts = 0;
        switch (g.type) {
        case GLP_GATE_NOOP: wires = 0; constraints = 0; return true;
        case GLP_GATE_CONSTANT: wires = p0; consts = p0; constraints = p0; return true;
        case GLP_GATE_PUBLIC_INPUT: wires = 4; constraints = 4; return true;
        case GLP_GATE_ARITHMETIC: wires = 4 * p0; consts = 2; constraints = p0; return true;
        case GLP_GATE_POSEIDON: wires = 135; constraints = 123; return true;
        case GLP_GATE_U32_INTERLEAVE: wires = 34 * p0; constraints = 34 * p0; return true;
        case GLP_GATE_UNINTERLEAVE_U32: case GLP_GATE_UNINTERLEAVE_B32: wires = 67 * p0; constraints = 67 * p0; return true;
        case GLP_GATE_U32_ARITHMETIC: wires = 38 * p0; constraints = 36 * p0; return true;
        case GLP_GATE_U32_ADD_MANY: wires = (p0 + 3 + 18) * p1; constraints = 21 * p1; return p0 >= 1 && p0 <= 16;
        case GLP_GATE_U32_SUBTRACTION: wires = 21 * p0; constraints = 19 * p0; return true;
        case GLP_GATE_U32_RANGE_CHECK: wires = 17 * p0; constraints = 17 * p0; return true;
        case GLP_GATE_COMPARISON: {
            if (p1 == 0 || p0 == 0 || p0 > 64) return false;
            const u32 cb = (p0 + p1 - 1) / p1;
            if (cb > 4) return false;
            wires = 4 + 5 * p1 + cb + 1; constraints = 2 + 5 * p1 + 1 + (cb + 1) + 2; return true;
        }
        case GLP_GATE_BASE_SUM: wires = 1 + p0; constraints = 1 + p0; return p1 >= 2 && p1 <= 16;
        case GLP_GATE_RANDOM_ACCESS: {
            const u32 copies = p1 & 0xFFFF, nextra = p1 >> 16;
            if (p0 < 1 || p0 > 5) return false;
            wires = (2 + (1u << p0)) * copies + nextra + p0 * copies; consts = nextra; constraints = copies * (p0 + 2) + nextra;
            return true;
        }
        default: return false;
        }
    };
    u32 maxc = 0;
    for (u32 i = 0; i < d.num_gates; i++) {
        const glp_gate &g = d.gates[i];
        {
            u32 gw = 0, gcn = 0, gk = 0;
            if (!gate_shape(g, gw, gcn, gk))
                return set_error(g.type > GLP_GATE_RANDOM_ACCESS ? GLP_ERR_UNSUPPORTED : GLP_ERR_ARG,
                                 "gate %u: type %u with parameters (%u, %u) is not supported", i, g.type, g.p0, g.p1);
            GLP_REQUIRE(gw <= d.num_wires, "gate %u (type %u) needs %u wires, circuit has %u", i, g.type, gw, d.num_wires);
            GLP_REQUIRE(d.num_selectors + gcn <= d.num_constants, "gate %u (type %u) needs %u constants", i, g.type, gcn);
            GLP_REQUIRE(gk == g.num_constraints, "gate %u (type %u): num_constraints %u, expected %u", i, g.type, g.num_constraints, gk);
        }
        switch (g.type) {
        case GLP_GATE_NOOP: case GLP_GATE_CONSTANT: case GLP_GATE_PUBLIC_INPUT: case GLP_GATE_ARITHMETIC:
        case GLP_GATE_POSEIDON: if (g.type == GLP_GATE_POSEIDON && d.num_wires < 135) return set_error(GLP_ERR_ARG, "PoseidonGate needs 135 wires"); break;
        case GLP_GATE_U32_INTERLEAVE: case GLP_GATE_UNINTERLEAVE_U32: case GLP_GATE_UNINTERLEAVE_B32: break;
        case GLP_GATE_U32_ARITHMETIC: case GLP_GATE_U32_ADD_MANY: case GLP_GATE_U32_SUBTRACTION:
        case GLP_GATE_U32_RANGE_CHECK: case GLP_GATE_COMPARISON: case GLP_GATE_BASE_SUM: break;
        case GLP_GATE_RANDOM_ACCESS:
            GLP_REQUIRE(g.p0 >= 1 && g.p0 <= 5, "RandomAccessGate bits outside 1..5");
            break;
        default: break;
        }
        GLP_REQUIRE(g.selector_index < d.num_selectors && g.group_start <= g.row && g.row < g.group_end, "bad selector data for gate %u", i);
        GLP_REQUIRE(g.num_constraints <= ACC3_MAX_TERMS, "gate %u: %u constraints exceed the %u the quotient accumulators hold", i,
                    g.num_constraints, ACC3_MAX_TERMS);
        maxc = std::max(maxc, g.num_constraints);
    }
    GLP_REQUIRE(maxc <= d.num_gate_constraints, "num_gate_constraints smaller than a gate's constraint count");
    {
        const size_t nrows = (size_t)1 << d.degree_bits;
        const u64 *sec[3] = {d.k_is, d.constants, d.sigmas};
        const size_t cnt[3] = {d.num_routed_wires, (size_t)d.num_constants * nrows, (size_t)d.num_routed_wires * nrows};
        const char *names[3] = {"k_is", "constants", "sigmas"};
        for (int i = 0; i < 3; i++) {
            const size_t bad = first_noncanonical(sec[i], cnt[i]);
            GLP_REQUIRE(bad == cnt[i], "%s[%zu] = 0x%016llx is not a canonical field element (>= p)", names[i], bad, (unsigned long long)sec[i][bad]);
        }
    }

    std::unique_ptr<glp_circuit, void (*)(glp_circuit *)> cc(new glp_circuit(), glp_circuit_free);
    cc->ctx = c;
    cc->d = d;
    cc->gates.assign(d.gates, d.gates + d.num_gates);
    cc->k_is.assign(d.k_is, d.k_is + d.num_routed_wires);
    if (cc->k_is.size() >= 2 && cc->k_is[0] == 1 && cc->k_is[1] > 1 && cc->k_is[1] < (1ull << 32)) {
        cc->k_ratio = (u32)cc->k_is[1];
        for (size_t j = 1; j < cc->k_is.size(); j++)
            if (cc->k_is[j] != mul(cc->k_is[j - 1], (u64)cc->k_ratio)) { cc->k_ratio = 0; break; }
    }
    cc->d.gates = cc->gates.data(); cc->d.k_is = cc->k_is.data(); cc->d.constants = nullptr; cc->d.sigmas = nullptr;
    make_layout(cc->d, cc->L);
    const size_t n = (size_t)1 << d.degree_bits;
    const u32 nc = d.num_constants, nr = d.num_routed_wires;
    GLP_TRY(c->alloc((void **)&cc->dev_gates, sizeof(DevGate) * std::max<u32>(d.num_gates, 1)));
    GLP_TRY(c->alloc((void **)&cc->dev_k_is, (size_t)nr * 8));
    GLP_TRY(c->alloc((void **)&cc->dev_sigmas, (size_t)nr * n * 8));
    static_assert(sizeof(DevGate) == sizeof(glp_gate), "gate layout");
    GLP_TRY(h2d(c, cc->dev_gates, cc->gates.data(), sizeof(DevGate) * d.num_gates));
    GLP_TRY(h2d(c, cc->dev_k_is, cc->k_is.data(), (size_t)nr * 8));
    GLP_TRY(h2d(c, cc->dev_sigmas, d.sigmas, (size_t)nr * n * 8));
    GLP_TRY(c->alloc((void **)&cc->dev_consts, (size_t)nc * n * 8));
    GLP_TRY(h2d(c, cc->dev_consts, d.constants, (size_t)nc * n * 8));
    GLP_TRY(build_quotient_plan(c, cc.get()));
    {
        void *v = nullptr;
        GLP_TRY(c->alloc(&v, (size_t)(nc + nr) * n * 8));
        u64 *csv = (u64 *)v;
        int rc = GLP_OK;
        {
            hipError_t e = hipMemcpyAsync(csv, cc->dev_consts, (size_t)nc * n * 8, hipMemcpyDeviceToDevice, c->stream);
            if (e != hipSuccess) rc = set_error(GLP_ERR_HIP, "D2D copy: %s", hipGetErrorString(e));
        }
        if (rc == GLP_OK) {
            hipError_t e = hipMemcpyAsync(csv + (size_t)nc * n, cc->dev_sigmas, (size_t)nr * n * 8, hipMemcpyDeviceToDevice, c->stream);
            if (e != hipSuccess) rc = set_error(GLP_ERR_HIP, "D2D copy: %s", hipGetErrorString(e));
        }
        if (rc == GLP_OK) rc = batch_build(c, csv, BATCH_VALUES, nc + nr, (int)d.degree_bits, (int)d.rate_bits, (int)d.cap_height, &cc->cs, nullptr, 1, (int)d.hasher);
// ... 291 lines not shown
```

### plonky2-lib_amd/csrc/prover_batch.inc

```
#include <chrono>
#include "host_pool.h"

namespace {

int caps_to_host(glp_ctx *c, const u64 *dev_digests, size_t dig_stride_words, size_t cap_off_digests, u32 capn, u32 K, std::vector<u64> &out) {
    out.resize((size_t)K * capn * 4);
    GLP_HIP(hipMemcpy2DAsync(out.data(), (size_t)capn * 32, dev_digests + 4 * cap_off_digests, dig_stride_words * 8, (size_t)capn * 32, K,
                             hipMemcpyDeviceToHost, c->stream));
    GLP_HIP(hipStreamSynchronize(c->stream));
    return GLP_OK;
}

int prove_batch_impl(glp_ctx *c, const glp_circuit *cc, u32 K, const u64 *dev_wires, const u64 *public_inputs, u64 *proofs_out) {
    const glp_circuit_desc &d = cc->d;
    const Layout &L = cc->L;
    const int lg = (int)d.degree_bits, rb = (int)d.rate_bits;
    const size_t n = (size_t)1 << lg, N = n << rb;
    const u32 nch = d.num_challenges, nr = d.num_routed_wires, nw = d.num_wires, nc = d.num_constants, qdf = d.quotient_degree_factor;
    const u32 npp = d.num_partial_products, capn = 1u << d.cap_height, nzp = nch * (1 + npp), npi = d.num_public_inputs;
    const u32 nred = d.num_reductions, nq = d.num_query_rounds;
    GLP_REQUIRE(nch == 2, "glp_prove_batch: num_challenges = %u (the batch path evaluates the quotient with the two-challenge kernels)", nch);
    GLP_REQUIRE(K >= 1 && K <= 4096, "glp_prove_batch: batch of %u proofs outside 1..4096", K);
    GLP_REQUIRE((size_t)K * nw * N * 8 <= ((size_t)64 << 30), "glp_prove_batch: batch too large (K * num_wires * 2^(degree_bits + rate_bits) words)");
    HostPool &pool = ctx_host_pool(c);
    const bool trace = getenv("GLP_BATCH_TRACE") != nullptr;
    auto t_last = std::chrono::steady_clock::now();
    auto mark = [&](const char *what) {
        if (!trace) return;
        (void)hipStreamSynchronize(c->stream);
        const auto now = std::chrono::steady_clock::now();
        fprintf(stderr, "[glp_prove_batch K=%u] %-28s %8.3f ms\n", K, what, std::chrono::duration<double, std::milli>(now - t_last).count());
        t_last = now;
    };
    Tmp tmp(c);
    auto P = [&](u32 k) { return proofs_out + (size_t)k * L.total; };
    const int hasher = (int)d.hasher;
    std::vector<Challenger> ch(K, Challenger(hasher));
    std::vector<u64> pih((size_t)K * 4, 0), caps;
    BatchHolder wb, zb, qb;

    pool.run(K, [&](size_t k) {
        host_hash_no_pad(public_inputs + k * npi, npi, &pih[4 * k]);
        if (npi) memcpy(P((u32)k) + L.pis, public_inputs + k * npi, (size_t)npi * 8);
    });
    mark("pi hashes (host)");
    GLP_TRY(batch_build(c, dev_wires, BATCH_VALUES, nw, lg, rb, (int)d.cap_height, &wb.b, nullptr, K, hasher));
    const size_t ndig = wb.b->ndigests, cap_off = merkle_cap_offset(N, (int)d.cap_height);
    GLP_TRY(caps_to_host(c, wb.b->digests, ndig * 4, cap_off, capn, K, caps));
    mark("wires commit + caps");
    std::vector<u64> chal((size_t)K * 2 * MAXCH, 0);
    pool.run(K, [&](size_t k) {
        memcpy(P((u32)k) + L.caps, &caps[k * capn * 4], (size_t)capn * 32);
        ch[k].observe_hashes(cc->digest, 1);
        ch[k].observe(&pih[4 * k], 4);
        ch[k].observe_hashes(&caps[k * capn * 4], capn);
        for (u32 i = 0; i < nch; i++) chal[k * 2 * MAXCH + i] = ch[k].get();
        for (u32 i = 0; i < nch; i++) chal[k * 2 * MAXCH + MAXCH + i] = ch[k].get();
    });

    mark("transcript 1 (host)");
    u64 *dev_chal, *zp, *dens, *tot;
    const u32 nblocks = nblk(n);
    GLP_TRY(tmp.get(&dev_chal, chal.size()));
    GLP_TRY(h2d(c, dev_chal, chal.data(), chal.size() * 8));
    GLP_TRY(tmp.get(&zp, (size_t)K * nzp * n));
    GLP_TRY(tmp.get(&dens, (size_t)K * nzp * n));
    GLP_TRY(tmp.get(&tot, (size_t)K * nch * nblocks));
    {
        PPArgs a;
        a.wires = dev_wires; a.sigmas = cc->dev_sigmas; a.k_is = cc->dev_k_is; a.zp = zp; a.dens = dens;
        for (int i = 0; i < MAXCH; i++) a.betas[i] = a.gammas[i] = 0;
        a.w_n = root_of_unity(lg); a.lg = (u32)lg; a.nr = nr; a.nch = nch; a.npp = npp; a.qdf = qdf;
        a.chal = dev_chal; a.wires_stride = (size_t)nw * n; a.zp_stride = (size_t)nzp * n;
        hipLaunchKernelGGL(HIP_KERNEL_NAME(k_pp_rows<2>), dim3(nblocks, K), dim3(256), 0, c->stream, a);
        GLP_HIP(hipGetLastError());
        hipLaunchKernelGGL(k_pp_block_tot, dim3(nblocks, nch, K), dim3(256), 0, c->stream, zp, tot, (u32)lg, nblocks, a.zp_stride);
        hipLaunchKernelGGL(k_pp_scan_tot, dim3(nch, K), dim3(256), 0, c->stream, tot, nblocks);
        hipLaunchKernelGGL(k_pp_apply, dim3(nblocks, nch, K), dim3(256), 0, c->stream, zp, tot, (u32)lg, nblocks, nch, npp, a.zp_stride);
        GLP_HIP(hipGetLastError());
    }
    GLP_TRY(batch_build(c, zp, BATCH_VALUES, nzp, lg, rb, (int)d.cap_height, &zb.b, nullptr, K, hasher));
    GLP_TRY(caps_to_host(c, zb.b->digests, ndig * 4, cap_off, capn, K, caps));

    mark("partial products + commit");
    int qdb = 0;
    while ((1u << qdb) < qdf) qdb++;
    const u32 Rq = 1u << qdb, step = 1u << (rb - qdb);
    const u32 nchunks = npp + 1, nterms = nch + nch * nchunks + d.num_gate_constraints;
    const size_t apn = (size_t)nch * nterms;
    std::vector<u64> apow((size_t)(1 + APL_WORDS) * K * apn), qpp((size_t)K * 3 * MAXCH, 0);
    pool.run(K, [&](size_t k) {
        memcpy(P((u32)k) + L.caps + capn * 4, &caps[k * capn * 4], (size_t)capn * 32);
        ch[k].observe_hashes(&caps[k * capn * 4], capn);
        for (u32 i = 0; i < nch; i++) {
            const u64 alpha = ch[k].get();
            u64 x = 1;
            for (u32 t = 0; t < nterms; t++) {
                const size_t e = (k * nch + i) * nterms + t;
                apow[e] = x;
                apl_words(x, &apow[(size_t)K * apn + APL_WORDS * e]);
                x = mul(x, alpha);
            }
        }
        for (u32 i = 0; i < nch; i++) { qpp[k * 3 * MAXCH + i] = chal[k * 2 * MAXCH + i]; qpp[k * 3 * MAXCH + MAXCH + i] = chal[k * 2 * MAXCH + MAXCH + i]; }
        memcpy(&qpp[k * 3 * MAXCH + 2 * MAXCH], &pih[4 * k], 32);
    });
    mark("transcript 2 + alpha powers (host)");
    u64 *dev_apow, *dev_qpp, *qv, *qV, *qc, *l0t;
    GLP_TRY(tmp.get(&dev_apow, apow.size()));
    GLP_TRY(h2d(c, dev_apow, apow.data(), apow.size() * 8));
    GLP_TRY(tmp.get(&dev_qpp, qpp.size()));
    GLP_TRY(h2d(c, dev_qpp, qpp.data(), qpp.size() * 8));
    const size_t qstride = (size_t)nch * Rq * n;
    GLP_TRY(tmp.get(&qv, (size_t)K * qstride));
    GLP_TRY(tmp.get(&qV, (size_t)K * qstride));
    GLP_TRY(tmp.get(&qc, (size_t)K * qstride));
    GLP_TRY(tmp.get(&l0t, (size_t)Rq * n));
    const u64 gn = pow(GEN, (u64)n);
    {
        QArgs a;
        QProof qp;
        QBatch qbt;
        memset(&qp, 0, sizeof(qp));
        a.cs = cc->cs->lde; a.gates = cc->dev_gates; a.k_is = cc->dev_k_is; a.k_ratio = cc->k_ratio;
        qp.wl = wb.b->lde; qp.zl = zb.b->lde; qp.out = qv; qp.apow = dev_apow; qp.apl = dev_apow + (size_t)K * apn;
        qbt.pp = dev_qpp; qbt.wl_stride = (size_t)nw * N; qbt.zl_stride = (size_t)nzp * N; qbt.out_stride = qstride; qbt.apow_stride = (size_t)nch * nterms;
        const u64 WN = root_of_unity(lg + rb), wR = root_of_unity(rb);
        for (u32 rq = 0; rq < Rq; rq++) {
            const u32 r = rq * step;
            a.shift_r[rq] = mul(GEN, pow(WN, (u64)r));
            a.zh[rq] = sub(mul(gn, pow(wR, (u64)r)), 1);
            a.zh_inv[rq] = inv(a.zh[rq]);
        }
        a.w_n = root_of_unity(lg); a.n_field = (u64)n % glf::P;
        a.lg = (u32)lg; a.rb = (u32)rb; a.step = step; a.nc = nc; a.nsel = d.num_selectors; a.nr = nr; a.nw = nw;
        a.nch = nch; a.npp = npp; a.qdf = qdf; a.num_gates = d.num_gates; a.nterms = nterms;
        a.many_selectors = d.num_selectors > 1; a.gate_mode = 1; a.l0 = l0t;
        hipLaunchKernelGGL(k_l0_table, dim3(nblk(n)), dim3(256), 0, c->stream, a, l0t, Rq);
        GLP_HIP(hipGetLastError());
        LightArgs lg_;
        lg_.count = cc->light_count; lg_.arith_gi = cc->arith_gi; lg_.arith_ops = cc->arith_ops;
        for (u32 i = 0; i < 8; i++) lg_.gi[i] = cc->light_gi[i];
        const dim3 g(nblk(n), Rq, K);
        if (cc->light_count || cc->arith_ops) hipLaunchKernelGGL(HIP_KERNEL_NAME(k_quotient<2, 2>), g, dim3(256), 0, c->stream, a, qp, qbt, lg_);
        else hipLaunchKernelGGL(HIP_KERNEL_NAME(k_quotient<2, 0>), g, dim3(256), 0, c->stream, a, qp, qbt, lg_);
        GLP_HIP(hipGetLastError());
        if (cc->limb_count) {
            LimbArgs la;
            limb_args(cc, la);
            la.extra_count = cc->limb_extra_count;
            for (int i = 0; i < 4; i++) la.extra_gi[i] = cc->limb_extra_gi[i];
            hipLaunchKernelGGL(HIP_KERNEL_NAME(k_quotient_limbs<2>), g, dim3(256), 0, c->stream, a, qp, qbt, la);
            GLP_HIP(hipGetLastError());
        }
        for (u32 gi : cc->single_gates) {
#define GLP_GATE_LAUNCH(T) case T: hipLaunchKernelGGL(HIP_KERNEL_NAME(k_quotient_gate<2, T>), g, dim3(256), 0, c->stream, a, qp, qbt, gi); break;
            switch (cc->gates[gi].type) {
                GLP_GATE_LAUNCH(GLP_GATE_CONSTANT) GLP_GATE_LAUNCH(GLP_GATE_PUBLIC_INPUT) GLP_GATE_LAUNCH(GLP_GATE_ARITHMETIC)
                GLP_GATE_LAUNCH(GLP_GATE_POSEIDON) GLP_GATE_LAUNCH(GLP_GATE_U32_INTERLEAVE) GLP_GATE_LAUNCH(GLP_GATE_UNINTERLEAVE_U32)
                GLP_GATE_LAUNCH(GLP_GATE_UNINTERLEAVE_B32) GLP_GATE_LAUNCH(GLP_GATE_U32_ARITHMETIC) GLP_GATE_LAUNCH(GLP_GATE_U32_ADD_MANY)
                GLP_GATE_LAUNCH(GLP_GATE_U32_SUBTRACTION) GLP_GATE_LAUNCH(GLP_GATE_U32_RANGE_CHECK) GLP_GATE_LAUNCH(GLP_GATE_COMPARISON)
                GLP_GATE_LAUNCH(GLP_GATE_BASE_SUM) GLP_GATE_LAUNCH(GLP_GATE_RANDOM_ACCESS)
            default: break;
            }
#undef GLP_GATE_LAUNCH
            GLP_HIP(hipGetLastError());
        }
    }
    {
        GLP_TRY(intt_values_to_coeffs(c, qv, qV, K * nch * Rq, lg));
        QCArgs q;
        q.V = qV; q.out = qc; q.lg = (u32)lg; q.Rq = Rq;
        q.wM_inv = inv(root_of_unity(lg + qdb)); q.wR_inv = inv(root_of_unity(qdb)); q.g_inv = inv(GEN);
        q.rq_inv = inv((u64)Rq);
        const u64 gni = inv(gn);
        u64 x = 1;
        for (u32 cidx = 0; cidx < Rq; cidx++) { q.gn_inv_pow[cidx] = x; x = mul(x, gni); }
        hipLaunchKernelGGL(k_quotient_combine, dim3(nblk(n), K * nch), dim3(256), 0, c->stream, q);
        GLP_HIP(hipGetLastError());
    }
    GLP_TRY(batch_build(c, qc, BATCH_COEFFS_BITREV, nch * qdf, lg, rb, (int)d.cap_height, &qb.b, nullptr, K, hasher));
    GLP_TRY(caps_to_host(c, qb.b->digests, ndig * 4, cap_off, capn, K, caps));

    mark("quotient + commit");
    std::vector<u64> zetas((size_t)K * 4);
    std::vector<int> err(K, 0);
    const u64 wn = root_of_unity(lg);
    pool.run(K, [&](size_t k) {
        memcpy(P((u32)k) + L.caps + 2 * capn * 4, &caps[k * capn * 4], (size_t)capn * 32);
        ch[k].observe_hashes(&caps[k * capn * 4], capn);
        const ext2 zeta = ch[k].get_ext();
        ext2 zp2 = zeta;
        for (int i = 0; i < lg; i++) zp2 = e_sqr(zp2);
        if (e_eq(zp2, e_from(1))) err[k] = 1;
        const ext2 zn = e_scale(zeta, wn);
        zetas[4 * k] = zeta.a; zetas[4 * k + 1] = zeta.b; zetas[4 * k + 2] = zn.a; zetas[4 * k + 3] = zn.b;
    });
    for (u32 k = 0; k < K; k++) if (err[k]) return set_error(GLP_ERR_PROVE, "Opening point is in the subgroup. (proof %u of the batch)", k);
    mark("transcript 3 (host)");
    const glp_batch *ob[4] = {cc->cs, wb.b, zb.b, qb.b};
    const size_t ostride[4] = {0, 1, 1, 1};
    u64 *dev_zetas, *zt, *partial;
    GLP_TRY(tmp.get(&dev_zetas, zetas.size()));
    GLP_TRY(h2d(c, dev_zetas, zetas.data(), zetas.size() * 8));
    GLP_TRY(tmp.get(&zt, (size_t)K * 2 * n));
    const u32 nob = open_blocks(n);
    size_t poff[6] = {0, 0, 0, 0, 0, 0};
    for (int b = 0; b < 5; b++) poff[b + 1] = poff[b] + (size_t)(b < 4 ? ob[b]->ncols : nch) * nob * 2;
    GLP_TRY(tmp.get(&partial, (size_t)K * poff[5]));
    auto zeta_tables = [&](size_t which) -> int {
        ZTArgs za;
        za.zt = zt; za.lg = (u32)lg; za.zeta_b = dev_zetas + 2 * which; za.zeta_stride = 4;
        for (int b = 0; b < 24; b++) za.zp2[b] = e_from(0);
        hipLaunchKernelGGL(HIP_KERNEL_NAME(k_zeta_table<true>), dim3(nblk(n), K), dim3(256), 0, c->stream, za);
        GLP_HIP(hipGetLastError());
        return GLP_OK;
    };
    auto open_launch = [&](const glp_batch *b, size_t bstride, size_t off, u32 cols) -> int {
        hipLaunchKernelGGL(k_open_dot, dim3(nob, cols, K), dim3(256), 0, c->stream, b->coeffs, zt, partial + off, (u32)lg,
                           bstride * b->ncols * n, (size_t)2 * n, poff[5]);
        GLP_HIP(hipGetLastError());
        return GLP_OK;
    };
    GLP_TRY(zeta_tables(0));
    for (int b = 0; b < 4; b++) GLP_TRY(open_launch(ob[b], ostride[b], poff[b], ob[b]->ncols));
    GLP_TRY(zeta_tables(1));
    GLP_TRY(open_launch(zb.b, 1, poff[4], nch));
    std::vector<u64> hp((size_t)K * poff[5]);
    GLP_TRY(d2h(c, hp.data(), partial, hp.size() * 8));
    mark("openings (device + copy)");
    size_t total_cols = 0;
    for (int b = 0; b < 4; b++) total_cols += ob[b]->ncols;
    std::vector<u64> fap((size_t)K * 2 * total_cols), fpp((size_t)K * 10);
    pool.run(K, [&](size_t k) {
        const u64 *h = hp.data() + k * poff[5];
        std::vector<ext2> open[4], all;
        for (int b = 0; b < 4; b++) open_batch_finish(h + poff[b], ob[b]->ncols, nob, open[b]);
        open_batch_finish(h + poff[4], nch, nob, all);
        u64 *op = P((u32)k) + L.openings;
        size_t o = 0;
        auto put = [&](ext2 e) { op[o++] = e.a; op[o++] = e.b; };
        for (u32 i = 0; i < nc + nr; i++) put(open[0][i]);
        for (u32 i = 0; i < nw; i++) put(open[1][i]);
        for (u32 i = 0; i < nch; i++) put(open[2][i]);
        for (u32 i = 0; i < nch; i++) put(all[i]);
        for (u32 i = 0; i < nch * npp; i++) put(open[2][nch + i]);
        for (u32 i = 0; i < nch * qdf; i++) put(open[3][i]);
        const u64 *p_cs = op, *p_w = op + 2 * (nc + nr), *p_zs = p_w + 2 * nw, *p_zn = p_zs + 2 * nch;
        const u64 *p_pp = p_zn + 2 * nch, *p_q = p_pp + 2 * nch * npp;
        ch[k].observe(p_cs, 2 * (nc + nr)); ch[k].observe(p_w, 2 * nw); ch[k].observe(p_zs, 2 * nch);
        ch[k].observe(p_pp, 2 * (size_t)nch * npp); ch[k].observe(p_q, 2 * (size_t)nch * qdf); ch[k].observe(p_zn, 2 * nch);
        const ext2 alpha = ch[k].get_ext();
        u64 *ap = &fap[k * 2 * total_cols];
        ext2 x = e_from(1), red0 = e_from(0), red1 = e_from(0);
        size_t j = 0;
        for (int b = 0; b < 4; b++)
            for (u32 col = 0; col < ob[b]->ncols; col++, j++) {
                ap[2 * j] = x.a; ap[2 * j + 1] = x.b;
                red0 = e_add(red0, e_mul(x, open[b][col]));
                x = e_mul(x, alpha);
            }
        x = e_from(1);
        for (u32 col = 0; col < nch; col++) { red1 = e_add(red1, e_mul(x, all[col])); x = e_mul(x, alpha); }
        const ext2 sa = e_pow(alpha, nch);
        u64 *v = &fpp[k * 10];
        v[0] = red0.a; v[1] = red0.b; v[2] = red1.a; v[3] = red1.b;
        v[4] = zetas[4 * k]; v[5] = zetas[4 * k + 1]; v[6] = zetas[4 * k + 2]; v[7] = zetas[4 * k + 3];
        v[8] = sa.a; v[9] = sa.b;
    });

    mark("transcript 4 + fri alpha powers (host)");
    u64 *dev_fap, *dev_fpp, *fv, *fcoef;
    GLP_TRY(tmp.get(&dev_fap, fap.size()));
    GLP_TRY(h2d(c, dev_fap, fap.data(), fap.size() * 8));
    GLP_TRY(tmp.get(&dev_fpp, fpp.size()));
    GLP_TRY(h2d(c, dev_fpp, fpp.data(), fpp.size() * 8));
    GLP_TRY(tmp.get(&fv, (size_t)K * 2 * n));
    GLP_TRY(tmp.get(&fcoef, (size_t)K * 2 * n));
    {
        FVArgs a;
        for (int b = 0; b < 4; b++) { a.lde[b] = ob[b]->lde; a.ncols[b] = ob[b]->ncols; a.lde_stride[b] = ostride[b] * ob[b]->ncols * N; }
        a.apow = dev_fap; a.out = fv;
        a.red0 = a.red1 = a.zeta = a.zeta_next = a.shift_acc = e_from(0);
        a.w_n = wn; a.g = GEN; a.lg = (u32)lg; a.rb = (u32)rb; a.nch = nch;
        a.pp = dev_fpp; a.apow_stride = 2 * total_cols; a.out_stride = 2 * n;
        hipLaunchKernelGGL(k_final_values, dim3(nblk(n), K), dim3(256), 0, c->stream, a);
        GLP_HIP(hipGetLastError());
        GLP_TRY(intt_values_to_coeffs(c, fv, fcoef, 2 * K, lg));
        hipLaunchKernelGGL(k_scale_bitrev_pow, dim3(nblk(n), 2 * K), dim3(256), 0, c->stream, fcoef, inv(GEN), (u32)lg);
        GLP_HIP(hipGetLastError());
    }
    struct BLayer { u64 *vals, *dig; u32 lgL, ab; size_t ndig; };
    std::vector<BLayer> layers;
    u64 *cur = fcoef;
    int lgcur = lg;
    u64 shift = GEN;
    u64 *dev_betas;
    GLP_TRY(tmp.get(&dev_betas, (size_t)K * 2));
    std::vector<u64> betas_h((size_t)K * 2);
    for (u32 r = 0; r < nred; r++) {
        const u32 ab = d.reduction_arity_bits[r], lgL = (u32)(lgcur + rb);
        const size_t Lsz = (size_t)1 << lgL, nleaves = Lsz >> ab;
        BLayer ly;
        ly.lgL = lgL; ly.ab = ab; ly.ndig = merkle_num_digests(nleaves, (int)d.cap_height);
// ... 128 lines not shown
```

### plonky2-lib_amd/csrc/prover_batch_dev.inc

```
#include "transcript_dev.h"
namespace {

int prove_batch_impl_dev(glp_ctx *c, const glp_circuit *cc, u32 K, const u64 *dev_wires, const u64 *public_inputs, u64 *proofs_out) {
    const glp_circuit_desc &d = cc->d;
    const Layout &L = cc->L;
    const int lg = (int)d.degree_bits, rb = (int)d.rate_bits;
    const size_t n = (size_t)1 << lg, N = n << rb;
    const u32 nch = d.num_challenges, nr = d.num_routed_wires, nw = d.num_wires, nc = d.num_constants, qdf = d.quotient_degree_factor;
    const u32 npp = d.num_partial_products, capn = 1u << d.cap_height, nzp = nch * (1 + npp), npi = d.num_public_inputs;
    const u32 nred = d.num_reductions, nq = d.num_query_rounds;
    GLP_REQUIRE(nch == 2, "glp_prove_batch: num_challenges = %u (the batch path evaluates the quotient with the two-challenge kernels)", nch);
    GLP_REQUIRE(K >= 1 && K <= 4096, "glp_prove_batch: batch of %u proofs outside 1..4096", K);
    GLP_REQUIRE((size_t)K * nw * N * 8 <= ((size_t)64 << 30), "glp_prove_batch: batch too large (K * num_wires * 2^(degree_bits + rate_bits) words)");
    const bool trace = getenv("GLP_BATCH_TRACE") != nullptr;
    auto t_last = std::chrono::steady_clock::now();
    auto mark = [&](const char *what) {
        if (!trace) return;
        (void)hipStreamSynchronize(c->stream);
        const auto now = std::chrono::steady_clock::now();
        fprintf(stderr, "[glp_prove_batch K=%u dev] %-28s %8.3f ms\n", K, what, std::chrono::duration<double, std::milli>(now - t_last).count());
        t_last = now;
    };
    Tmp tmp(c);
    const int hasher = (int)d.hasher;
    BatchHolder wb, zb, qb;
    const unsigned tgrid = (K + 15) / 16;
    u64 *dch, *image;
    u32 *dev_err;
    GLP_TRY(tmp.get(&dch, (size_t)K * DCH_WORDS));
    GLP_TRY(tmp.get(&image, (size_t)K * L.total));
    { u64 *e; GLP_TRY(tmp.get(&e, (K + 1) / 2 + 1)); dev_err = (u32 *)e; }
    GLP_HIP(hipMemsetAsync(dev_err, 0, (size_t)K * 4, c->stream));
    if (npi) GLP_HIP(hipMemcpy2DAsync(image + L.pis, L.total * 8, public_inputs, (size_t)npi * 8, (size_t)npi * 8, K, hipMemcpyHostToDevice, c->stream));
    TrGeo g;
    g.dch = dch; g.image = image; g.total = L.total; g.K = K; g.capn = capn; g.nch = nch;

    GLP_TRY(batch_build(c, dev_wires, BATCH_VALUES, nw, lg, rb, (int)d.cap_height, &wb.b, nullptr, K, hasher));
    const size_t ndig = wb.b->ndigests, cap_off = merkle_cap_offset(N, (int)d.cap_height);
    u64 *dev_chal, *dev_qpp;
    GLP_TRY(tmp.get(&dev_chal, (size_t)K * 2 * MAXCH));
    GLP_TRY(tmp.get(&dev_qpp, (size_t)K * 3 * MAXCH));
    GLP_HIP(hipMemsetAsync(dev_chal, 0, (size_t)K * 2 * MAXCH * 8, c->stream));
    GLP_HIP(hipMemsetAsync(dev_qpp, 0, (size_t)K * 3 * MAXCH * 8, c->stream));
    hipLaunchKernelGGL(k_tr_begin, dim3(tgrid), dim3(256), 0, c->stream, g, cc->digest[0], cc->digest[1], cc->digest[2], cc->digest[3], L.pis, npi,
                       wb.b->digests + 4 * cap_off, ndig * 4, L.caps, dev_chal, dev_qpp);
    GLP_HIP(hipGetLastError());
    mark("wires commit + transcript 1");

    u64 *zp, *dens, *tot;
    const u32 nblocks = nblk(n);
    GLP_TRY(tmp.get(&zp, (size_t)K * nzp * n));
    GLP_TRY(tmp.get(&dens, (size_t)K * nzp * n));
    GLP_TRY(tmp.get(&tot, (size_t)K * nch * nblocks));
    {
        PPArgs a;
        a.wires = dev_wires; a.sigmas = cc->dev_sigmas; a.k_is = cc->dev_k_is; a.zp = zp; a.dens = dens;
        for (int i = 0; i < MAXCH; i++) a.betas[i] = a.gammas[i] = 0;
        a.w_n = root_of_unity(lg); a.lg = (u32)lg; a.nr = nr; a.nch = nch; a.npp = npp; a.qdf = qdf;
        a.chal = dev_chal; a.wires_stride = (size_t)nw * n; a.zp_stride = (size_t)nzp * n;
        const size_t small_lds = (size_t)2 * nch * (npp + 2) * n * sizeof(u64);
        if (lg <= 7 && small_lds <= 64 * 1024) {
            hipLaunchKernelGGL(k_pp_rows_small, dim3(1, K), dim3(256), small_lds, c->stream, a);
        } else {
            hipLaunchKernelGGL(HIP_KERNEL_NAME(k_pp_rows<2>), dim3(nblocks, K), dim3(256), 0, c->stream, a);
            GLP_HIP(hipGetLastError());
            hipLaunchKernelGGL(k_pp_block_tot, dim3(nblocks, nch, K), dim3(256), 0, c->stream, zp, tot, (u32)lg, nblocks, a.zp_stride);
            hipLaunchKernelGGL(k_pp_scan_tot, dim3(nch, K), dim3(256), 0, c->stream, tot, nblocks);
            hipLaunchKernelGGL(k_pp_apply, dim3(nblocks, nch, K), dim3(256), 0, c->stream, zp, tot, (u32)lg, nblocks, nch, npp, a.zp_stride);
        }
        GLP_HIP(hipGetLastError());
    }
    GLP_TRY(batch_build(c, zp, BATCH_VALUES, nzp, lg, rb, (int)d.cap_height, &zb.b, nullptr, K, hasher));
    int qdb = 0;
    while ((1u << qdb) < qdf) qdb++;
    const u32 Rq = 1u << qdb, step = 1u << (rb - qdb);
    const u32 nchunks = npp + 1, nterms = nch + nch * nchunks + d.num_gate_constraints;
    const size_t apn = (size_t)nch * nterms;
    u64 *dev_apow, *qv, *qV, *qc, *l0t;
    GLP_TRY(tmp.get(&dev_apow, (size_t)(1 + APL_WORDS) * K * apn));
    hipLaunchKernelGGL(k_tr_alphas, dim3(tgrid), dim3(256), 0, c->stream, g, zb.b->digests + 4 * cap_off, ndig * 4, L.caps + (size_t)capn * 4, nterms, dev_apow,
                       dev_apow + (size_t)K * apn);
    GLP_HIP(hipGetLastError());
    mark("partial products + commit + transcript 2");

    const size_t qstride = (size_t)nch * Rq * n;
    GLP_TRY(tmp.get(&qv, (size_t)K * qstride));
    GLP_TRY(tmp.get(&qV, (size_t)K * qstride));
    GLP_TRY(tmp.get(&qc, (size_t)K * qstride));
    GLP_TRY(tmp.get(&l0t, (size_t)Rq * n));
    const u64 gn = pow(GEN, (u64)n);
    {
        QArgs a;
        QProof qp;
        QBatch qbt;
        memset(&qp, 0, sizeof(qp));
        a.cs = cc->cs->lde; a.gates = cc->dev_gates; a.k_is = cc->dev_k_is; a.k_ratio = cc->k_ratio;
        qp.wl = wb.b->lde; qp.zl = zb.b->lde; qp.out = qv; qp.apow = dev_apow; qp.apl = dev_apow + (size_t)K * apn;
        qbt.pp = dev_qpp; qbt.wl_stride = (size_t)nw * N; qbt.zl_stride = (size_t)nzp * N; qbt.out_stride = qstride; qbt.apow_stride = (size_t)nch * nterms;
        const u64 WN = root_of_unity(lg + rb), wR = root_of_unity(rb);
        for (u32 rq = 0; rq < Rq; rq++) {
            const u32 r = rq * step;
            a.shift_r[rq] = mul(GEN, pow(WN, (u64)r));
            a.zh[rq] = sub(mul(gn, pow(wR, (u64)r)), 1);
            a.zh_inv[rq] = inv(a.zh[rq]);
        }
        a.w_n = root_of_unity(lg); a.n_field = (u64)n % glf::P;
        a.lg = (u32)lg; a.rb = (u32)rb; a.step = step; a.nc = nc; a.nsel = d.num_selectors; a.nr = nr; a.nw = nw;
        a.nch = nch; a.npp = npp; a.qdf = qdf; a.num_gates = d.num_gates; a.nterms = nterms;
        a.many_selectors = d.num_selectors > 1; a.gate_mode = 1; a.l0 = l0t;
        hipLaunchKernelGGL(k_l0_table, dim3(nblk(n)), dim3(256), 0, c->stream, a, l0t, Rq);
        GLP_HIP(hipGetLastError());
        LightArgs lg_;
        lg_.count = cc->light_count; lg_.arith_gi = cc->arith_gi; lg_.arith_ops = cc->arith_ops;
        for (u32 i = 0; i < 8; i++) lg_.gi[i] = cc->light_gi[i];
        const dim3 gq(nblk(n), Rq, K);
        if (cc->light_count || cc->arith_ops) hipLaunchKernelGGL(HIP_KERNEL_NAME(k_quotient<2, 2>), gq, dim3(256), 0, c->stream, a, qp, qbt, lg_);
        else hipLaunchKernelGGL(HIP_KERNEL_NAME(k_quotient<2, 0>), gq, dim3(256), 0, c->stream, a, qp, qbt, lg_);
        GLP_HIP(hipGetLastError());
        if (cc->limb_count) {
            LimbArgs la;
            limb_args(cc, la);
            la.extra_count = cc->limb_extra_count;
            for (int i = 0; i < 4; i++) la.extra_gi[i] = cc->limb_extra_gi[i];
            hipLaunchKernelGGL(HIP_KERNEL_NAME(k_quotient_limbs<2>), gq, dim3(256), 0, c->stream, a, qp, qbt, la);
            GLP_HIP(hipGetLastError());
        }
        for (u32 gi : cc->single_gates) {
#define GLP_GATE_LAUNCH(T) case T: hipLaunchKernelGGL(HIP_KERNEL_NAME(k_quotient_gate<2, T>), gq, dim3(256), 0, c->stream, a, qp, qbt, gi); break;
            switch (cc->gates[gi].type) {
                GLP_GATE_LAUNCH(GLP_GATE_CONSTANT) GLP_GATE_LAUNCH(GLP_GATE_PUBLIC_INPUT) GLP_GATE_LAUNCH(GLP_GATE_ARITHMETIC)
                GLP_GATE_LAUNCH(GLP_GATE_POSEIDON) GLP_GATE_LAUNCH(GLP_GATE_U32_INTERLEAVE) GLP_GATE_LAUNCH(GLP_GATE_UNINTERLEAVE_U32)
                GLP_GATE_LAUNCH(GLP_GATE_UNINTERLEAVE_B32) GLP_GATE_LAUNCH(GLP_GATE_U32_ARITHMETIC) GLP_GATE_LAUNCH(GLP_GATE_U32_ADD_MANY)
                GLP_GATE_LAUNCH(GLP_GATE_U32_SUBTRACTION) GLP_GATE_LAUNCH(GLP_GATE_U32_RANGE_CHECK) GLP_GATE_LAUNCH(GLP_GATE_COMPARISON)
                GLP_GATE_LAUNCH(GLP_GATE_BASE_SUM) GLP_GATE_LAUNCH(GLP_GATE_RANDOM_ACCESS)
            default: break;
            }
#undef GLP_GATE_LAUNCH
            GLP_HIP(hipGetLastError());
        }
    }
    {
        GLP_TRY(intt_values_to_coeffs(c, qv, qV, K * nch * Rq, lg));
        QCArgs q;
        q.V = qV; q.out = qc; q.lg = (u32)lg; q.Rq = Rq;
        q.wM_inv = inv(root_of_unity(lg + qdb)); q.wR_inv = inv(root_of_unity(qdb)); q.g_inv = inv(GEN);
        q.rq_inv = inv((u64)Rq);
        const u64 gni = inv(gn);
        u64 x = 1;
        for (u32 cidx = 0; cidx < Rq; cidx++) { q.gn_inv_pow[cidx] = x; x = mul(x, gni); }
        hipLaunchKernelGGL(k_quotient_combine, dim3(nblk(n), K * nch), dim3(256), 0, c->stream, q);
        GLP_HIP(hipGetLastError());
    }
    GLP_TRY(batch_build(c, qc, BATCH_COEFFS_BITREV, nch * qdf, lg, rb, (int)d.cap_height, &qb.b, nullptr, K, hasher));
    const u64 wn = root_of_unity(lg);
    u64 *dev_zetas;
    GLP_TRY(tmp.get(&dev_zetas, (size_t)K * 4));
    hipLaunchKernelGGL(k_tr_zeta, dim3(tgrid), dim3(256), 0, c->stream, g, qb.b->digests + 4 * cap_off, ndig * 4, L.caps + 2 * (size_t)capn * 4, (u32)lg, wn, dev_zetas,
                       dev_err);
    GLP_HIP(hipGetLastError());
    mark("quotient + commit + transcript 3");

    const glp_batch *ob[4] = {cc->cs, wb.b, zb.b, qb.b};
    const size_t ostride[4] = {0, 1, 1, 1};
    u64 *zt, *partial;
    GLP_TRY(tmp.get(&zt, (size_t)K * 2 * n));
    const u32 nob = open_blocks(n);
    OpenGeo og;
    og.poff[0] = 0;
    for (int b = 0; b < 5; b++) og.poff[b + 1] = og.poff[b] + (size_t)(b < 4 ? ob[b]->ncols : nch) * nob * 2;
    for (int b = 0; b < 4; b++) og.cols[b] = ob[b]->ncols;
    og.openings_off = L.openings; og.nob = nob; og.nch = nch; og.npp = npp; og.nopen = (u32)L.nopen;
    GLP_TRY(tmp.get(&partial, (size_t)K * og.poff[5]));
    auto zeta_tables = [&](size_t which) -> int {
        ZTArgs za;
        za.zt = zt; za.lg = (u32)lg; za.zeta_b = dev_zetas + 2 * which; za.zeta_stride = 4;
        for (int b = 0; b < 24; b++) za.zp2[b] = e_from(0);
        hipLaunchKernelGGL(HIP_KERNEL_NAME(k_zeta_table<true>), dim3(nblk(n), K), dim3(256), 0, c->stream, za);
        GLP_HIP(hipGetLastError());
        return GLP_OK;
    };
    auto open_launch = [&](const glp_batch *b, size_t bstride, size_t off, u32 cols) -> int {
        hipLaunchKernelGGL(k_open_dot, dim3(nob, cols, K), dim3(256), 0, c->stream, b->coeffs, zt, partial + off, (u32)lg,
                           bstride * b->ncols * n, (size_t)2 * n, og.poff[5]);
        GLP_HIP(hipGetLastError());
        return GLP_OK;
    };
    GLP_TRY(zeta_tables(0));
    for (int b = 0; b < 4; b++) GLP_TRY(open_launch(ob[b], ostride[b], og.poff[b], ob[b]->ncols));
    GLP_TRY(zeta_tables(1));
    GLP_TRY(open_launch(zb.b, 1, og.poff[4], nch));
    hipLaunchKernelGGL(k_open_reduce, dim3(nblk((size_t)K * L.nopen)), dim3(256), 0, c->stream, g, og, partial);
    GLP_HIP(hipGetLastError());
    size_t total_cols = 0;
    for (int b = 0; b < 4; b++) total_cols += ob[b]->ncols;
    u64 *dev_fap, *dev_fpp, *fv, *fcoef;
    GLP_TRY(tmp.get(&dev_fap, (size_t)K * 2 * total_cols));
    GLP_TRY(tmp.get(&dev_fpp, (size_t)K * 10));
    hipLaunchKernelGGL(k_tr_fri_alpha, dim3(tgrid), dim3(256), 0, c->stream, g, og, dev_zetas, dev_fap, dev_fpp);
    GLP_HIP(hipGetLastError());
    mark("openings + transcript 4");

    GLP_TRY(tmp.get(&fv, (size_t)K * 2 * n));
    GLP_TRY(tmp.get(&fcoef, (size_t)K * 2 * n));
    {
        FVArgs a;
        for (int b = 0; b < 4; b++) { a.lde[b] = ob[b]->lde; a.ncols[b] = ob[b]->ncols; a.lde_stride[b] = ostride[b] * ob[b]->ncols * N; }
        a.apow = dev_fap; a.out = fv;
        a.red0 = a.red1 = a.zeta = a.zeta_next = a.shift_acc = e_from(0);
        a.w_n = wn; a.g = GEN; a.lg = (u32)lg; a.rb = (u32)rb; a.nch = nch;
        a.pp = dev_fpp; a.apow_stride = 2 * total_cols; a.out_stride = 2 * n;
        if (lg >= 2 && lg <= 7) hipLaunchKernelGGL(k_final_values_small, dim3(1, K), dim3(256), 0, c->stream, a);
        else hipLaunchKernelGGL(k_final_values, dim3(nblk(n), K), dim3(256), 0, c->stream, a);
        GLP_HIP(hipGetLastError());
        GLP_TRY(intt_values_to_coeffs(c, fv, fcoef, 2 * K, lg));
        hipLaunchKernelGGL(k_scale_bitrev_pow, dim3(nblk(n), 2 * K), dim3(256), 0, c->stream, fcoef, inv(GEN), (u32)lg);
        GLP_HIP(hipGetLastError());
    }
    struct BLayer { u64 *vals, *dig; u32 lgL, ab; size_t ndig; };
    std::vector<BLayer> layers;
    u64 *cur = fcoef;
    int lgcur = lg;
    u64 shift = GEN;
    u64 *dev_betas;
    GLP_TRY(tmp.get(&dev_betas, (size_t)K * 2));
    for (u32 r = 0; r < nred; r++) {
        const u32 ab = d.reduction_arity_bits[r], lgL = (u32)(lgcur + rb);
        const size_t Lsz = (size_t)1 << lgL, nleaves = Lsz >> ab;
        BLayer ly;
        ly.lgL = lgL; ly.ab = ab; ly.ndig = merkle_num_digests(nleaves, (int)d.cap_height);
        GLP_TRY(tmp.get(&ly.vals, (size_t)K * 2 * Lsz));
        GLP_TRY(tmp.get(&ly.dig, (size_t)K * ly.ndig * 4));
        GLP_TRY(lde_coeffs(c, cur, ly.vals, 2 * K, lgcur, rb, shift));
        if (nleaves * K <= c->merkle_coop_max)
            hipLaunchKernelGGL(k_fri_leaf_hash_coop, dim3((unsigned)((nleaves + 15) / 16), K), dim3(256), 0, c->stream, ly.vals, ly.dig, lgL, (u32)rb,
                               ab, 2 * Lsz, ly.ndig * 4);
        else if (nleaves * K <= c->merkle_quad_max)
            hipLaunchKernelGGL(k_fri_leaf_hash_quad, dim3((unsigned)((nleaves + 63) / 64), K), dim3(256), 0, c->stream, ly.vals, ly.dig, lgL, (u32)rb,
                               ab, 2 * Lsz, ly.ndig * 4);
        else
            hipLaunchKernelGGL(k_fri_leaf_hash, dim3(nblk(nleaves), K), dim3(256), 0, c->stream, ly.vals, ly.dig, lgL, (u32)rb, ab, 2 * Lsz,
                               ly.ndig * 4);
        GLP_HIP(hipGetLastError());
        GLP_TRY(merkle_levels(c, ly.dig, nleaves, (int)d.cap_height, K, ly.ndig * 4, hasher));
        hipLaunchKernelGGL(k_tr_beta, dim3(tgrid), dim3(256), 0, c->stream, g, ly.dig + 4 * merkle_cap_offset(nleaves, (int)d.cap_height), ly.ndig * 4,
                           L.fri_caps + (size_t)r * capn * 4, dev_betas);
        GLP_HIP(hipGetLastError());
        u64 *nxt;
        const size_t nnew = ((size_t)1 << lgcur) >> ab;
        GLP_TRY(tmp.get(&nxt, (size_t)K * 2 * nnew));
        hipLaunchKernelGGL(k_fri_fold, dim3(nblk(nnew), K), dim3(256), 0, c->stream, cur, nxt, e_from(0), (u32)lgcur, ab, (const u64 *)dev_betas);
        GLP_HIP(hipGetLastError());
        cur = nxt; lgcur -= (int)ab;
        shift = pow(shift, (u64)1 << ab);
        layers.push_back(ly);
    }
    const size_t fl = (size_t)1 << lgcur;
    if (fl != L.final_len) return set_error(GLP_ERR_ARG, "reduction_arity_bits inconsistent with degree_bits");
    u64 *dev_pst, *dev_best, *dev_next, *dev_ppos;
    GLP_TRY(tmp.get(&dev_pst, (size_t)K * 12));
    GLP_TRY(tmp.get(&dev_best, K));
    GLP_TRY(tmp.get(&dev_next, K));
    GLP_TRY(tmp.get(&dev_ppos, (K + 1) / 2));
    GLP_HIP(hipMemsetAsync(dev_next, 0, (size_t)K * 8, c->stream));
    GLP_HIP(hipMemsetAsync(dev_best, 0xFF, (size_t)K * 8, c->stream));
    hipLaunchKernelGGL(k_tr_final, dim3(tgrid), dim3(256), 0, c->stream, g, cur, (u32)lgcur, L.final_poly, dev_pst, (u32 *)dev_ppos, dev_err);
    GLP_HIP(hipGetLastError());
    mark("fri combine + layers + transcript 5");

    GLP_TRY(pow_batch_launch(c, tmp, dev_pst, (const u32 *)dev_ppos, d.proof_of_work_bits, dev_best, dev_next, K));
    u64 *dev_idx;
    GLP_TRY(tmp.get(&dev_idx, (size_t)K * nq));
    hipLaunchKernelGGL(k_tr_queries, dim3(tgrid), dim3(256), 0, c->stream, g, dev_best, d.proof_of_work_bits, L.pow, nq, (u64)N, dev_idx, dev_err);
    GLP_HIP(hipGetLastError());
    mark("proof of work + transcript 6");

    u64 *dev_q = image + L.queries;
// ... 61 lines not shown
```

### plonky2-lib_amd/csrc/prover_types.h

```cpp
#pragma once
#include <algorithm>
#include <string.h>
#include <vector>
#include "batch.h"
#include "common.h"
#include "keccak.h"
#include "poseidon.h"

using namespace glp;
using namespace glf;

constexpr int MAXCH = 4;
constexpr int MAXR = 16;
constexpr u32 APL_WORDS = 4;

struct DevGate { u32 type, selector_index, group_start, group_end, row, num_constraints, p0, p1; };

struct Layout {
    size_t caps, openings, fri_caps, queries, final_poly, pow, pis, total, nopen, query_stride;
    u32 oracle_cols[4], depth0, step_depth[16], final_len;
};

struct glp_circuit {
    glp_ctx *ctx = nullptr;
    glp_circuit_desc d;
    std::vector<glp_gate> gates;
    std::vector<u64> k_is;
    u64 digest[4];
    DevGate *dev_gates = nullptr;
    u64 *dev_k_is = nullptr;
    u32 k_ratio = 0;
    u64 *dev_sigmas = nullptr;
    u64 *dev_consts = nullptr;
    u64 *dev_limb_desc = nullptr;
    u32 limb_count = 0, limb_groups = 0, limb_gcount[4] = {0, 0, 0, 0}, limb_gi[20] = {0}, limb_jlo[4] = {0, 0, 0, 0}, limb_jhi[4] = {0, 0, 0, 0};
    u32 limb_extra_count = 0, limb_extra_gi[4] = {0, 0, 0, 0};
    u32 arith_gi = 0, arith_ops = 0;
    u32 light_count = 0, light_gi[8] = {0, 0, 0, 0, 0, 0, 0, 0};
    std::vector<u32> single_gates;
    glp_batch *cs = nullptr;
    std::vector<u64> cs_cap;
    Layout L;
};

struct Challenger {
    u64 st[12]; u64 in[8]; int nin = 0; u64 out[8]; int nout = 0;
    int hasher = GLP_HASH_POSEIDON;
    explicit Challenger(int hasher_ = GLP_HASH_POSEIDON) : hasher(hasher_) { memset(st, 0, sizeof(st)); }
    void duplex() {
        for (int i = 0; i < nin; i++) st[i] = in[i];
        nin = 0;
        if (hasher == GLP_HASH_KECCAK25) kec::permute(st); else pos::permute(st);
        memcpy(out, st, 64); nout = 8;
    }
    void observe_hashes(const u64 *digests, size_t count) {
        for (size_t i = 0; i < count; i++) {
            if (hasher == GLP_HASH_KECCAK25) { u64 e[4]; kec::digest_to_elements(digests + 4 * i, e); observe(e, 4); }
            else observe(digests + 4 * i, 4);
        }
    }
    void observe(const u64 *e, size_t n) {
        for (size_t i = 0; i < n; i++) { nout = 0; in[nin++] = e[i]; if (nin == 8) duplex(); }
    }
    u64 get() { if (nin > 0 || nout == 0) duplex(); return out[--nout]; }
    ext2 get_ext() { u64 a = get(); u64 b = get(); return e_make(a, b); }
};
inline void host_hash_no_pad(const u64 *in, size_t len, u64 out[4]) {
    u64 st[12] = {0};
    for (size_t off = 0; off < len; off += 8) {
        size_t c = std::min<size_t>(8, len - off);
        for (size_t i = 0; i < c; i++) st[i] = in[off + i];
        pos::permute(st);
    }
    memcpy(out, st, 32);
}
```

### plonky2-lib_amd/csrc/transcript_dev.h

```cpp
#pragma once
#include "poseidon.h"
#include "prover_types.h"

namespace {
__device__ __forceinline__ u64 tr_pow(u64 b, u64 e) {
    u64 r = 1;
    while (e) { if (e & 1) r = mul(r, b); b = sqr(b); e >>= 1; }
    return r;
}
constexpr u32 DCH_WORDS = 32;
struct DSponge { u64 st, inb; u32 nin, nout; };
__device__ __forceinline__ void ds_load(DSponge &s, const u64 *p, int l) {
    s.st = l < 12 ? p[l] : 0; s.inb = l < 8 ? p[12 + l] : 0; s.nin = (u32)p[28]; s.nout = (u32)p[29];
}
__device__ __forceinline__ void ds_store(const DSponge &s, u64 *p, int l, bool live) {
    if (!live) return;
    if (l < 12) p[l] = s.st;
    if (l < 8) p[12 + l] = s.inb;
    if (l == 0) { p[28] = s.nin; p[29] = s.nout; }
}
__device__ __noinline__ void ds_duplex(DSponge &s, int l, int gb) {
    if ((u32)l < s.nin) s.st = s.inb;
    s.nin = 0;
    s.st = pos::permute_coop(s.st, l, gb);
    s.nout = 8;
}
template <class F>
__device__ __forceinline__ void ds_observe_f(DSponge &s, u32 n, int l, int gb, F fetch) {
    u32 i = 0;
    while (i < n) {
        const u32 take = min(8u - s.nin, n - i);
        if ((u32)l >= s.nin && (u32)l < s.nin + take) s.inb = fetch(i + (u32)l - s.nin);
        s.nin += take; i += take; s.nout = 0;
        if (s.nin == 8) ds_duplex(s, l, gb);
    }
}
__device__ __forceinline__ void ds_observe(DSponge &s, const u64 *p, u32 n, int l, int gb) {
    ds_observe_f(s, n, l, gb, [p](u32 i) { return p[i]; });
}
__device__ __forceinline__ void ds_observe1(DSponge &s, u64 v, int l, int gb) {
    if ((u32)l == s.nin) s.inb = v;
    s.nin++; s.nout = 0;
    if (s.nin == 8) ds_duplex(s, l, gb);
}
__device__ __forceinline__ u64 ds_get(DSponge &s, int l, int gb) {
    if (s.nin > 0 || s.nout == 0) ds_duplex(s, l, gb);
    s.nout--;
    return pos::shfl64(s.st, gb + (int)s.nout);
}
__device__ __forceinline__ ext2 ds_get_ext(DSponge &s, int l, int gb) { const u64 a = ds_get(s, l, gb); const u64 b = ds_get(s, l, gb); return e_make(a, b); }
__device__ __forceinline__ ext2 dgroup_sum(ext2 v) {
#pragma unroll
    for (int m = 8; m >= 1; m >>= 1) v = e_add(v, e_make(pos::shfl_xor64(v.a, m), pos::shfl_xor64(v.b, m)));
    return v;
}

struct TrGeo {
    u64 *dch;
    u64 *image;
    size_t total;
    u32 K, capn, nch;
};
#define TR_PROLOGUE                                                                           \
    const int tid = threadIdx.x, l = tid & 15, gb = (tid & 63) & ~15;                         \
    const u32 k0 = blockIdx.x * 16 + (tid >> 4);                                              \
    const bool live = k0 < g.K;                                                               \
    const u32 k = live ? k0 : 0;                                                              \
    u64 *dch = g.dch + (size_t)k * DCH_WORDS, *img = g.image + (size_t)k * g.total;           \
    (void)img
__device__ __forceinline__ void tr_cap(DSponge &s, const u64 *cap, u64 *dst, u32 capn, bool live, int l, int gb) {
    if (live) for (u32 i = (u32)l; i < 4 * capn; i += 16) dst[i] = cap[i];
    ds_observe(s, cap, 4 * capn, l, gb);
}

__global__ __launch_bounds__(256) void k_tr_begin(TrGeo g, u64 d0, u64 d1, u64 d2, u64 d3, size_t pis_off, u32 npi, const u64 *cap_b, size_t cap_stride,
                                                  size_t caps_off, u64 *chal, u64 *qpp) {
    TR_PROLOGUE;
    u64 x = 0;
    for (u32 c0 = 0; c0 < npi; c0 += 8) {
        if (l < 8 && c0 + (u32)l < npi) x = img[pis_off + c0 + l];
        x = pos::permute_coop(x, l, gb);
    }
    const u64 pih0 = pos::shfl64(x, gb), pih1 = pos::shfl64(x, gb + 1), pih2 = pos::shfl64(x, gb + 2), pih3 = pos::shfl64(x, gb + 3);
    DSponge s;
    s.st = 0; s.inb = 0; s.nin = 0; s.nout = 0;
    ds_observe1(s, d0, l, gb); ds_observe1(s, d1, l, gb); ds_observe1(s, d2, l, gb); ds_observe1(s, d3, l, gb);
    ds_observe1(s, pih0, l, gb); ds_observe1(s, pih1, l, gb); ds_observe1(s, pih2, l, gb); ds_observe1(s, pih3, l, gb);
    tr_cap(s, cap_b + (size_t)k * cap_stride, img + caps_off, g.capn, live, l, gb);
    u64 *ck = chal + (size_t)k * 2 * MAXCH, *qk = qpp + (size_t)k * 3 * MAXCH;
    for (u32 i = 0; i < g.nch; i++) { const u64 b = ds_get(s, l, gb); if (live && l == 0) { ck[i] = b; qk[i] = b; } }
    for (u32 i = 0; i < g.nch; i++) { const u64 b = ds_get(s, l, gb); if (live && l == 0) { ck[MAXCH + i] = b; qk[MAXCH + i] = b; } }
    if (live && l == 0) { qk[2 * MAXCH] = pih0; qk[2 * MAXCH + 1] = pih1; qk[2 * MAXCH + 2] = pih2; qk[2 * MAXCH + 3] = pih3; }
    ds_store(s, dch, l, live);
}
__global__ __launch_bounds__(256) void k_tr_alphas(TrGeo g, const u64 *cap_b, size_t cap_stride, size_t caps_off, u32 nterms, u64 *apow, u64 *apl) {
    TR_PROLOGUE;
    DSponge s;
    ds_load(s, dch, l);
    tr_cap(s, cap_b + (size_t)k * cap_stride, img + caps_off, g.capn, live, l, gb);
    for (u32 i = 0; i < g.nch; i++) {
        const u64 alpha = ds_get(s, l, gb);
        u64 a16 = alpha;
#pragma unroll
        for (int j = 0; j < 4; j++) a16 = sqr(a16);
        u64 x = tr_pow(alpha, (u64)l);
        for (u32 t = (u32)l; t < nterms; t += 16) {
            const size_t e = ((size_t)k * g.nch + i) * nterms + t;
            if (live) {
                apow[e] = x;
                const u64 mp = mul(x, 1ull << 32);
                u64 *o = apl + APL_WORDS * e;
                o[0] = (x & 0x3FFFFFull) | (((x >> 22) & 0x3FFFFFull) << 32); o[1] = x >> 44;
                o[2] = (mp & 0x3FFFFFull) | (((mp >> 22) & 0x3FFFFFull) << 32); o[3] = mp >> 44;
            }
            x = mul(x, a16);
        }
    }
    ds_store(s, dch, l, live);
}
__global__ __launch_bounds__(256) void k_tr_zeta(TrGeo g, const u64 *cap_b, size_t cap_stride, size_t caps_off, u32 lg, u64 wn, u64 *zetas, u32 *err) {
    TR_PROLOGUE;
    DSponge s;
    ds_load(s, dch, l);
    tr_cap(s, cap_b + (size_t)k * cap_stride, img + caps_off, g.capn, live, l, gb);
    const ext2 zeta = ds_get_ext(s, l, gb);
    ext2 zp = zeta;
    for (u32 i = 0; i < lg; i++) zp = e_sqr(zp);
    const ext2 zn = e_scale(zeta, wn);
    if (live && l == 0) {
        u64 *z = zetas + 4 * (size_t)k;
        z[0] = zeta.a; z[1] = zeta.b; z[2] = zn.a; z[3] = zn.b;
        if (zp.a == 1 && zp.b == 0) err[k] |= 1u;
    }
    ds_store(s, dch, l, live);
}
struct OpenGeo { size_t poff[6], openings_off; u32 cols[4], nob, nch, npp, nopen; };
__global__ __launch_bounds__(256) void k_open_reduce(TrGeo g, OpenGeo og, const u64 *partial) {
    const size_t id = (size_t)blockIdx.x * 256 + threadIdx.x;
    if (id >= (size_t)g.K * og.nopen) return;
    const u32 k = (u32)(id / og.nopen);
    u32 o = (u32)(id % og.nopen), b, col;
    const u32 nzs = og.nch, npps = og.nch * og.npp;
    if (o < og.cols[0]) { b = 0; col = o; }
    else if ((o -= og.cols[0]) < og.cols[1]) { b = 1; col = o; }
    else if ((o -= og.cols[1]) < nzs) { b = 2; col = o; }
    else if ((o -= nzs) < nzs) { b = 4; col = o; }
    else if ((o -= nzs) < npps) { b = 2; col = nzs + o; }
    else { o -= npps; b = 3; col = o; }
    const u64 *p = partial + (size_t)k * og.poff[5] + og.poff[b] + 2 * (size_t)col * og.nob;
    u64 a = 0, bb = 0;
    for (u32 j = 0; j < og.nob; j++) { a = add(a, p[2 * j]); bb = add(bb, p[2 * j + 1]); }
    u64 *dst = g.image + (size_t)k * g.total + og.openings_off + 2 * (id % og.nopen);
    dst[0] = a; dst[1] = bb;
}
__global__ __launch_bounds__(256) void k_tr_fri_alpha(TrGeo g, OpenGeo og, const u64 *zetas, u64 *fap, u64 *fpp) {
    TR_PROLOGUE;
    DSponge s;
    ds_load(s, dch, l);
    const u64 *op = img + og.openings_off;
    const u32 nzs = og.nch, npps = og.nch * og.npp;
    const u64 *p_cs = op, *p_w = p_cs + 2 * og.cols[0], *p_zs = p_w + 2 * og.cols[1], *p_zn = p_zs + 2 * nzs, *p_pp = p_zn + 2 * nzs, *p_q = p_pp + 2 * npps;
    ds_observe(s, p_cs, 2 * og.cols[0], l, gb); ds_observe(s, p_w, 2 * og.cols[1], l, gb); ds_observe(s, p_zs, 2 * nzs, l, gb);
    ds_observe(s, p_pp, 2 * npps, l, gb); ds_observe(s, p_q, 2 * og.cols[3], l, gb); ds_observe(s, p_zn, 2 * nzs, l, gb);
    const ext2 alpha = ds_get_ext(s, l, gb);
    ext2 a16 = alpha;
#pragma unroll
    for (int j = 0; j < 4; j++) a16 = e_sqr(a16);
    const u32 total_cols = og.cols[0] + og.cols[1] + og.cols[2] + og.cols[3];
    ext2 x = e_pow(alpha, (u64)l), r0 = e_from(0);
    u64 *ap = fap + (size_t)k * 2 * total_cols;
    for (u32 j = (u32)l; j < total_cols; j += 16) {
        const u64 *src;
        u32 c = j;
        if (c < og.cols[0]) src = p_cs + 2 * c;
        else if ((c -= og.cols[0]) < og.cols[1]) src = p_w + 2 * c;
        else if ((c -= og.cols[1]) < og.cols[2]) src = c < nzs ? p_zs + 2 * c : p_pp + 2 * (c - nzs);
        else src = p_q + 2 * (c - og.cols[2]);
        if (live) { ap[2 * j] = x.a; ap[2 * j + 1] = x.b; }
        r0 = e_add(r0, e_mul(x, e_make(src[0], src[1])));
        x = e_mul(x, a16);
    }
    r0 = dgroup_sum(r0);
    ext2 r1 = e_from(0), y = e_from(1);
    for (u32 j = 0; j < nzs; j++) { r1 = e_add(r1, e_mul(y, e_make(p_zn[2 * j], p_zn[2 * j + 1]))); y = e_mul(y, alpha); }
    if (live && l == 0) {
        u64 *v = fpp + (size_t)k * 10;
        const u64 *z = zetas + 4 * (size_t)k;
        v[0] = r0.a; v[1] = r0.b; v[2] = r1.a; v[3] = r1.b; v[4] = z[0]; v[5] = z[1]; v[6] = z[2]; v[7] = z[3]; v[8] = y.a; v[9] = y.b;
    }
    ds_store(s, dch, l, live);
}
__global__ __launch_bounds__(256) void k_tr_beta(TrGeo g, const u64 *cap_b, size_t cap_stride, size_t caps_off, u64 *betas) {
    TR_PROLOGUE;
    DSponge s;
    ds_load(s, dch, l);
    tr_cap(s, cap_b + (size_t)k * cap_stride, img + caps_off, g.capn, live, l, gb);
    const ext2 beta = ds_get_ext(s, l, gb);
    if (live && l == 0) { betas[2 * (size_t)k] = beta.a; betas[2 * (size_t)k + 1] = beta.b; }
    ds_store(s, dch, l, live);
}
__global__ __launch_bounds__(256) void k_tr_final(TrGeo g, const u64 *cur, u32 lgf, size_t final_off, u64 *pst, u32 *ppos, u32 *err) {
    TR_PROLOGUE;
    DSponge s;
    ds_load(s, dch, l);
    const u32 fl = 1u << lgf;
    const u64 *h = cur + (size_t)k * 2 * fl;
    u64 *pf = img + final_off;
    if (live) for (u32 p = (u32)l; p < fl; p += 16) { const u32 kk = bitrev32(p, (int)lgf); pf[2 * kk] = h[p]; pf[2 * kk + 1] = h[fl + p]; }
    ds_observe_f(s, 2 * fl, l, gb, [h, fl, lgf](u32 e) { return h[(e & 1 ? fl : 0) + bitrev32(e >> 1, (int)lgf)]; });
    if (live) {
        if (l < 12) pst[(size_t)k * 12 + l] = ((u32)l < s.nin) ? s.inb : s.st;
        if (l == 0) { ppos[k] = s.nin; if (s.nin >= 8) err[k] |= 2u; }
    }
    ds_store(s, dch, l, live);
}
__global__ __launch_bounds__(256) void k_tr_queries(TrGeo g, const u64 *best, u32 pow_bits, size_t pow_off, u32 nq, u64 Nmask_plus1, u64 *idx, u32 *err) {
    TR_PROLOGUE;
    DSponge s;
    ds_load(s, dch, l);
    const u64 w = best[k];
    if (live && l == 0) { img[pow_off] = w; if (w == ~0ull) err[k] |= 4u; }
    ds_observe1(s, w, l, gb);
    const u64 resp = ds_get(s, l, gb);
    if (live && l == 0 && pow_bits && (resp >> (64 - pow_bits)) != 0) err[k] |= 8u;
    for (u32 q = 0; q < nq; q++) {
        const u64 x = ds_get(s, l, gb) % Nmask_plus1;
        if (live && l == 0) idx[(size_t)k * nq + q] = x;
    }
    ds_store(s, dch, l, live);
}
#undef TR_PROLOGUE

#define TR_PROLOGUE                                                                           \
    const int tid = threadIdx.x, l = tid & 15, gb = (tid & 63) & ~15;                         \
    const u32 k0 = blockIdx.x * 16 + (tid >> 4);                                              \
    const bool live = k0 < g.K;                                                               \
    const u32 k = live ? k0 : 0;                                                              \
    u64 *dch = g.dch + (size_t)k * DCH_WORDS, *img = g.image + (size_t)k * g.total;           \
    (void)img
__global__ __launch_bounds__(256) void k_trv_final(TrGeo g, size_t final_off, u32 nwords) {
    TR_PROLOGUE;
    DSponge s;
    ds_load(s, dch, l);
    ds_observe(s, img + final_off, nwords, l, gb);
    ds_store(s, dch, l, live);
}
__global__ __launch_bounds__(256) void k_trv_queries(TrGeo g, u32 pow_bits, size_t pow_off, u32 nq, u64 N, u64 *idx, u32 *err) {
    TR_PROLOGUE;
    DSponge s;
    ds_load(s, dch, l);
    ds_observe1(s, img[pow_off], l, gb);
    const u64 resp = ds_get(s, l, gb);
    if (live && l == 0 && pow_bits && (resp >> (64 - pow_bits)) != 0) err[k] |= 8u;
    for (u32 q = 0; q < nq; q++) {
        const u64 x = ds_get(s, l, gb) % N;
        if (live && l == 0) idx[(size_t)k * nq + q] = x;
    }
    ds_store(s, dch, l, live);
}
#undef TR_PROLOGUE
__global__ __launch_bounds__(256) void k_trv_pack(u32 K, u32 vstride, const u64 *fap, u32 total_cols, const u64 *fpp, const u64 *betas, u32 nred,
                                                  const u64 *idx, u32 nq, u64 *vc) {
    const u32 k = blockIdx.x * 256 + threadIdx.x;
    if (k >= K) return;
    u64 *o = vc + (size_t)k * vstride;
    const u64 *v = fpp + (size_t)k * 10, *ap = fap + (size_t)k * 2 * total_cols;
    o[0] = ap[2]; o[1] = ap[3];
    o[2] = v[4]; o[3] = v[5]; o[4] = v[6]; o[5] = v[7];
// ... 7 lines not shown
```

### plonky2-lib_amd/csrc/verifier.hip

```cpp
#include <chrono>
#include <string>
#include <thread>
#include "merkle.h"
#include "prover_types.h"
#include "transcript_dev.h"

namespace {

struct E {
    ext2 v;
    E() : v(e_from(0)) {}
    E(ext2 x) : v(x) {}
    explicit E(u64 x) : v(e_from(x % P)) {}
};
inline E operator+(E a, E b) { return E(e_add(a.v, b.v)); }
inline E operator-(E a, E b) { return E(e_sub(a.v, b.v)); }
inline E operator*(E a, E b) { return E(e_mul(a.v, b.v)); }
inline E operator*(E a, u64 s) { return E(e_scale(a.v, s % P)); }
inline bool operator==(E a, E b) { return e_eq(a.v, b.v); }
inline E rd(const u64 *p) { return E(e_make(p[0], p[1])); }
inline E inv(E a) { return E(e_inv(a.v)); }
inline E epow(E a, u64 e) { return E(e_pow(a.v, e)); }
const E ONE = E((u64)1), ZERO = E((u64)0);

// ... 575 lines not shown
    const ext2 alpha = rd2(vc + VC_ALPHA), zeta = rd2(vc + VC_ZETA), zeta_next = rd2(vc + VC_ZETA_NEXT);
    const u32 capn4 = 4u << a.cap_height;
    u32 code = 0;
#define VQ_FAIL(C) do { if (code == 0) code = (C); } while (0)
    ext2 a16 = alpha;
#pragma unroll
    for (int i = 0; i < 4; i++) a16 = e_sqr(a16);
    const ext2 al = e_pow(alpha, (u64)l);
    ext2 r0 = e_from(0), r1 = e_from(0), off = e_from(1);
    for (int t = 0; t < 4; t++) {
        const u32 ncols = a.oracle_cols[t];
        const u64 *cap = t == 0 ? a.cs_cap : proof + a.caps + (size_t)(t - 1) * capn4;
        if (merkle_bad<HASHER>(w, ncols, x_index, w + ncols, a.depth0, cap, l, gb)) VQ_FAIL(1 + (u32)t);
        ext2 part = e_from(0);
        if ((u32)l < ncols)
            for (int j = (int)(((ncols - 1 - (u32)l) >> 4) << 4) + l; j >= 0; j -= 16) part = e_add(e_mul(part, a16), e_from(w[j]));
        r0 = e_add(r0, e_mul(off, group_sum(e_mul(part, al))));
        off = e_mul(off, e_pow(alpha, (u64)ncols));
        if (t == 2) { ext2 ap = e_from(1); for (u32 j = 0; j < a.nch; j++) { r1 = e_add(r1, e_scale(ap, w[j])); ap = e_mul(ap, alpha); } }
        w += ncols + 4 * (size_t)a.depth0;
    }
    u64 subgroup_x = mul(GEN, dvpow(a.wN, (u64)(__brevll((unsigned long long)x_index) >> (64 - a.lgN))));
    ext2 old_eval;
    {
        const ext2 d0 = e_sub(e_from(subgroup_x), zeta), d1 = e_sub(e_from(subgroup_x), zeta_next);
        if ((d0.a == 0 && d0.b == 0) || (d1.a == 0 && d1.b == 0)) VQ_FAIL(5);
        ext2 sum = e_mul(e_sub(r0, rd2(vc + VC_RED0)), e_inv(d0));
        sum = e_add(e_mul(sum, rd2(vc + VC_SHIFT1)), e_mul(e_sub(r1, rd2(vc + VC_RED1)), e_inv(d1)));
        old_eval = sum;
    }
    for (u32 r = 0; r < a.nred; r++) {
        const u32 ab = a.ab[r], arity = 1u << ab;
        const u64 *ev = w, *path = w + 2 * (size_t)arity;
        const size_t coset_index = x_index >> ab, within = x_index & (arity - 1);
        if (!e_eq(rd2(ev + 2 * within), old_eval)) VQ_FAIL(6 + 2 * r);
        {
            const u64 gA = a.gA[r];
            const u32 rw = (u32)(__brev((unsigned)within) >> (32 - ab));
            const u64 coset_start = mul(subgroup_x, dvpow(gA, (u64)(arity - rw)));
            const ext2 beta = rd2(vc + VC_BETAS + 2 * r);
            ext2 acc = e_from(0);
            for (u32 i = (u32)l; i < arity; i += 16) {
                const u64 pi = mul(coset_start, dvpow(gA, (u64)i));
                ext2 num = e_from(1);
                u64 den = 1, pj = coset_start;
                for (u32 j = 0; j < arity; j++) {
                    if (j != i) { num = e_mul(num, e_sub(beta, e_from(pj))); den = mul(den, sub(pi, pj)); }
                    pj = mul(pj, gA);
                }
                const u32 bi = (u32)(__brev((unsigned)i) >> (32 - ab));
                acc = e_add(acc, e_scale(e_mul(rd2(ev + 2 * bi), num), glf::inv(den)));
            }
            old_eval = group_sum(acc);
        }
        const u64 *cap = proof + a.fri_caps + (size_t)r * capn4;
        if (merkle_bad<HASHER>(ev, 2 * arity, coset_index, path, a.step_depth[r], cap, l, gb)) VQ_FAIL(7 + 2 * r);
        for (u32 i = 0; i < ab; i++) subgroup_x = sqr(subgroup_x);
        x_index = coset_index;
        w += 2 * (size_t)arity + 4 * (size_t)a.step_depth[r];
    }
    {
        ext2 acc = e_from(0);
        for (u32 i = a.final_len; i-- > 0;) acc = e_add(e_scale(acc, subgroup_x), rd2(proof + a.final_poly + 2 * (size_t)i));
        if (!e_eq(acc, old_eval)) VQ_FAIL(6 + 2 * a.nred);
    }
#undef VQ_FAIL
    if (live && l == 0) a.status[grp] = code;
}
}

#include "host_pool.h"
extern "C" int glp_verify_batch(glp_ctx *c, const glp_circuit *cc, uint32_t K, const uint64_t *proofs, int32_t *status_out, char *reasons_out) {
    GLP_REQUIRE(c && cc && proofs && status_out, "null argument");
    GLP_REQUIRE(cc->ctx == c, "circuit belongs to another context");
    GLP_REQUIRE(K >= 1 && K <= 65536, "glp_verify_batch: batch of %u proofs outside 1..65536", K);
    GLP_TRY(bind(c));
    const glp_circuit_desc &d = cc->d;
    const Layout &L = cc->L;
    const u32 nq = d.num_query_rounds, nred = d.num_reductions;
    const u32 vstride = (VC_XIDX + nq + 3) & ~3u;
    std::vector<VChal> vcs(K);
    std::vector<int> rc(K, GLP_OK);
    std::vector<std::string> why(K);
    std::vector<u64> hv((size_t)K * vstride, 0);
    struct Scratch { glp_ctx *c; std::vector<void *> p; ~Scratch() { (void)hipStreamSynchronize(c->stream); for (void *q : p) c->release(q); } } sc{c, {}};
    auto get = [&](void **p, size_t bytes) -> int { int r = c->alloc(p, bytes); if (r == GLP_OK) sc.p.push_back(*p); return r; };
    u64 *dev_proofs = nullptr, *dev_vc = nullptr;
    u32 *dev_status = nullptr;
    GLP_TRY(get((void **)&dev_proofs, (size_t)K * L.total * 8));
    GLP_TRY(get((void **)&dev_vc, hv.size() * 8));
    GLP_TRY(get((void **)&dev_status, (size_t)K * nq * 4));
    const bool trace = getenv("GLP_BATCH_TRACE") != nullptr;
    const auto t_start = std::chrono::steady_clock::now();
    auto since = [&]() { return std::chrono::duration<double, std::milli>(std::chrono::steady_clock::now() - t_start).count(); };
    hipError_t up_err = hipSuccess;
    std::thread uploader([&] {
        up_err = hipSetDevice(c->device);
        if (up_err == hipSuccess) up_err = hipMemcpyAsync(dev_proofs, proofs, (size_t)K * L.total * 8, hipMemcpyHostToDevice, c->stream);
    });
    const bool dev_tr = d.hasher == GLP_HASH_POSEIDON && getenv("GLP_VERIFY_HOST_TRANSCRIPT") == nullptr;
    const u32 nch = d.num_challenges, capn = 1u << d.cap_height;
    u64 *dev_chal = nullptr, *dev_qpp = nullptr, *dev_apow = nullptr, *dev_zetas = nullptr;
    u32 *dev_err = nullptr;
    std::vector<u64> h_back;
    const u64 *h_chal = nullptr, *h_qpp = nullptr, *h_apow = nullptr, *h_zetas = nullptr;
    const u32 *h_err = nullptr;
    hipEvent_t ev_chal = nullptr;
    struct EvGuard { hipEvent_t &e; ~EvGuard() { if (e) (void)hipEventDestroy(e); } } evg{ev_chal};
    double t_front = 0, t_up = 0;
    if (!dev_tr) {
        ctx_host_pool(c).run(K, [&](size_t k) {
            rc[k] = verify_front(cc, proofs + k * L.total, vcs[k]);
            if (rc[k] != GLP_OK) { why[k] = g_last_error; return; }
            const VChal &v = vcs[k];
            u64 *o = &hv[k * vstride];
            auto put = [&](u32 at, const E &e) { o[at] = e.v.a; o[at + 1] = e.v.b; };
            put(VC_ALPHA, v.fri_alpha); put(VC_ZETA, v.zeta); put(VC_ZETA_NEXT, v.zeta_next); put(VC_RED0, v.red0); put(VC_RED1, v.red1); put(VC_SHIFT1, v.shift1);
            for (u32 r = 0; r < nred; r++) put(VC_BETAS + 2 * r, v.fri_betas[r]);
            for (u32 q = 0; q < nq; q++) o[VC_XIDX + q] = v.x_index[q];
        });
        t_front = since();
        uploader.join();
        t_up = since();
        if (up_err != hipSuccess) return set_error(GLP_ERR_HIP, "upload of the proofs: %s", hipGetErrorString(up_err));
        GLP_HIP(hipMemcpyAsync(dev_vc, hv.data(), hv.size() * 8, hipMemcpyHostToDevice, c->stream));
    } else {
        ctx_host_pool(c).run(K, [&](size_t k) {
            rc[k] = verify_canonical(cc, proofs + k * L.total);
            if (rc[k] != GLP_OK) why[k] = g_last_error;
        });
        t_front = since();
        uploader.join();
        t_up = since();
        if (up_err != hipSuccess) return set_error(GLP_ERR_HIP, "upload of the proofs: %s", hipGetErrorString(up_err));
        const u32 total_cols = L.oracle_cols[0] + L.oracle_cols[1] + L.oracle_cols[2] + L.oracle_cols[3];
        u64 *dch, *dev_apl, *dev_fap, *dev_fpp, *dev_betas, *dev_idx;
        GLP_TRY(get((void **)&dch, (size_t)K * DCH_WORDS * 8));
        const size_t w_chal = (size_t)K * 2 * MAXCH, w_qpp = (size_t)K * 3 * MAXCH, w_apow = (size_t)K * nch * 2, w_zetas = (size_t)K * 4, w_err = (K + 1) / 2;
        u64 *dev_back;
        GLP_TRY(get((void **)&dev_back, (w_chal + w_qpp + w_apow + w_zetas + w_err) * 8));
        dev_chal = dev_back; dev_qpp = dev_chal + w_chal; dev_apow = dev_qpp + w_qpp; dev_zetas = dev_apow + w_apow; dev_err = (u32 *)(dev_zetas + w_zetas);
        GLP_TRY(get((void **)&dev_apl, (size_t)K * nch * 2 * APL_WORDS * 8));
        GLP_TRY(get((void **)&dev_fap, (size_t)K * 2 * total_cols * 8));
        GLP_TRY(get((void **)&dev_fpp, (size_t)K * 10 * 8));
        GLP_TRY(get((void **)&dev_betas, (size_t)std::max<u32>(nred, 1) * K * 2 * 8));
        GLP_TRY(get((void **)&dev_idx, (size_t)K * nq * 8));
        GLP_HIP(hipMemsetAsync(dev_back, 0, (w_chal + w_qpp + w_apow + w_zetas + w_err) * 8, c->stream));
        TrGeo g;
        g.dch = dch; g.image = dev_proofs; g.total = L.total; g.K = K; g.capn = capn; g.nch = nch;
        const dim3 tg((K + 15) / 16), tb(256);
        const size_t cap4 = (size_t)capn * 4;
        hipLaunchKernelGGL(k_tr_begin, tg, tb, 0, c->stream, g, cc->digest[0], cc->digest[1], cc->digest[2], cc->digest[3], L.pis, d.num_public_inputs,
                           dev_proofs + L.caps, L.total, L.caps, dev_chal, dev_qpp);
        hipLaunchKernelGGL(k_tr_alphas, tg, tb, 0, c->stream, g, dev_proofs + L.caps + cap4, L.total, L.caps + cap4, 2u, dev_apow, dev_apl);
        hipLaunchKernelGGL(k_tr_zeta, tg, tb, 0, c->stream, g, dev_proofs + L.caps + 2 * cap4, L.total, L.caps + 2 * cap4, d.degree_bits,
                           root_of_unity((int)d.degree_bits), dev_zetas, dev_err);
        OpenGeo og;
        memset(&og, 0, sizeof(og));
        for (int b = 0; b < 4; b++) og.cols[b] = L.oracle_cols[b];
        og.openings_off = L.openings; og.nch = nch; og.npp = d.num_partial_products; og.nopen = (u32)L.nopen;
        hipLaunchKernelGGL(k_tr_fri_alpha, tg, tb, 0, c->stream, g, og, dev_zetas, dev_fap, dev_fpp);
        for (u32 r = 0; r < nred; r++)
            hipLaunchKernelGGL(k_tr_beta, tg, tb, 0, c->stream, g, dev_proofs + L.fri_caps + r * cap4, L.total, L.fri_caps + r * cap4, dev_betas + (size_t)r * K * 2);
        hipLaunchKernelGGL(k_trv_final, tg, tb, 0, c->stream, g, L.final_poly, 2u * L.final_len);
        hipLaunchKernelGGL(k_trv_queries, tg, tb, 0, c->stream, g, d.proof_of_work_bits, L.pow, nq, (u64)1 << (d.degree_bits + d.rate_bits), dev_idx, dev_err);
        hipLaunchKernelGGL(k_trv_pack, dim3((K + 255) / 256), dim3(256), 0, c->stream, K, vstride, dev_fap, total_cols, dev_fpp, dev_betas, nred, dev_idx, nq, dev_vc);
        GLP_HIP(hipGetLastError());
        h_back.resize(w_chal + w_qpp + w_apow + w_zetas + w_err);
        GLP_HIP(hipMemcpyAsync(h_back.data(), dev_back, h_back.size() * 8, hipMemcpyDeviceToHost, c->stream));
        GLP_HIP(hipEventCreateWithFlags(&ev_chal, hipEventDisableTiming));
        GLP_HIP(hipEventRecord(ev_chal, c->stream));
        h_chal = h_back.data(); h_qpp = h_chal + w_chal; h_apow = h_qpp + w_qpp; h_zetas = h_apow + w_apow; h_err = (const u32 *)(h_zetas + w_zetas);
    }
    VQArgs a;
    memset(&a, 0, sizeof(a));
    a.proofs = dev_proofs; a.vchal = dev_vc; a.status = dev_status;
    const size_t N = (size_t)1 << (d.degree_bits + d.rate_bits);
    a.cs_cap = cc->cs->digests + 4 * merkle_cap_offset(N, (int)d.cap_height);
    a.total = L.total; a.caps = L.caps; a.fri_caps = L.fri_caps; a.queries = L.queries; a.query_stride = L.query_stride; a.final_poly = L.final_poly;
    a.vstride = vstride; a.nq = nq; a.K = K; a.nch = d.num_challenges; a.lgN = d.degree_bits + d.rate_bits; a.cap_height = d.cap_height;
    a.depth0 = L.depth0; a.nred = nred; a.final_len = L.final_len;
    for (int t = 0; t < 4; t++) a.oracle_cols[t] = L.oracle_cols[t];
    for (u32 r = 0; r < nred; r++) { a.ab[r] = d.reduction_arity_bits[r]; a.step_depth[r] = L.step_depth[r]; a.gA[r] = root_of_unity((int)d.reduction_arity_bits[r]); }
    a.wN = root_of_unity((int)a.lgN);
    {
        StageScope st(c, "verify_queries", 8.0 * K * L.total);
        const unsigned nblocks = (unsigned)(((size_t)K * nq + 15) / 16);
        if (d.hasher == GLP_HASH_KECCAK25) hipLaunchKernelGGL(HIP_KERNEL_NAME(k_verify_queries<GLP_HASH_KECCAK25>), dim3(nblocks), dim3(256), 0, c->stream, a);
        else hipLaunchKernelGGL(HIP_KERNEL_NAME(k_verify_queries<GLP_HASH_POSEIDON>), dim3(nblocks), dim3(256), 0, c->stream, a);
        GLP_HIP(hipGetLastError());
    }
    std::vector<u32> hs((size_t)K * nq);
    double t_chal = 0, t_van = 0;
    if (dev_tr) {
        GLP_HIP(hipEventSynchronize(ev_chal));
        t_chal = since();
        ctx_host_pool(c).run(K, [&](size_t k) {
            if (rc[k] != GLP_OK) return;
            if (h_err[k] & 8u) { rc[k] = set_error(GLP_ERR_PROVE, "Invalid proof of work witness."); why[k] = g_last_error; return; }
            u64 alphas[MAXCH] = {0, 0, 0, 0};
            for (u32 i = 0; i < nch; i++) alphas[i] = h_apow[(k * nch + i) * 2 + 1];
            const E zeta(e_make(h_zetas[4 * k], h_zetas[4 * k + 1]));
            rc[k] = verify_vanishing(cc, proofs + k * L.total, &h_chal[k * 2 * MAXCH], &h_chal[k * 2 * MAXCH + MAXCH], alphas, zeta, &h_qpp[k * 3 * MAXCH + 2 * MAXCH]);
            if (rc[k] != GLP_OK) why[k] = g_last_error;
        });
        t_van = since();
    }
    GLP_HIP(hipMemcpyAsync(hs.data(), dev_status, hs.size() * 4, hipMemcpyDeviceToHost, c->stream));
    GLP_HIP(hipStreamSynchronize(c->stream));
    if (trace) {
        if (dev_tr) fprintf(stderr, "[glp_verify_batch K=%u dev] canonical scan %.3f ms | upload done at %.3f | challenges back at %.3f | identity at zeta done at %.3f | query rounds done at %.3f ms\n",
                            K, t_front, t_up, t_chal, t_van, since());
        else fprintf(stderr, "[glp_verify_batch K=%u] host half %.3f ms | upload done at %.3f | query rounds done at %.3f ms\n", K, t_front, t_up, since());
    }
    for (u32 k = 0; k < K; k++) {
        if (rc[k] == GLP_OK)
            for (u32 q = 0; q < nq && rc[k] == GLP_OK; q++)
                if (hs[(size_t)k * nq + q]) { rc[k] = query_failure(q, hs[(size_t)k * nq + q], nred); why[k] = g_last_error; }
        status_out[k] = rc[k];
        if (reasons_out) {
            char *o = reasons_out + (size_t)k * GLP_REASON_LEN;
            memset(o, 0, GLP_REASON_LEN);
            if (rc[k] != GLP_OK) strncpy(o, why[k].c_str(), GLP_REASON_LEN - 1);
        }
    }
    return GLP_OK;
}

extern "C" int glp_verify(const glp_circuit *cc, const uint64_t *proof_words) {
    GLP_REQUIRE(cc && proof_words, "null argument");
    return verify_impl(cc, proof_words);
}
extern "C" int glp_verify_n(const glp_circuit *cc, const uint64_t *proof_words, size_t num_words) {
    GLP_REQUIRE(cc && proof_words, "null argument");
    GLP_REQUIRE(num_words == cc->L.total, "proof has %zu words, a proof of this circuit has %zu", num_words, (size_t)cc->L.total);
    return verify_impl(cc, proof_words);
}
```

Baseline: 9.108.

## Restructure limb quotient kernel around per-column events with alpha-power offset tables

Rewrites the U32 limb-gate quotient kernel so it makes a single pass over limb columns for all limb gates at once, instead of looping over groups of up to five gate slots. Range-check products go into shared prefix/suffix accumulators (pm/pp), and the alpha powers they need are shifted using a new extended table of positive and negative alpha powers (apx). Gate filters are cached in shared memory, and the launch-bounds occupancy hint rises from 2 to 4. The aim is to cut redundant per-slot work and register pressure, at the cost of more complex event decoding, a larger alpha-power table, and extra transcript-kernel work to build it.

Result: no change. 9.150 (median of 6 runs) (+0.5%).

```diff
diff --git a/plonky2-lib_amd/csrc/prover.hip b/plonky2-lib_amd/csrc/prover.hip
--- a/plonky2-lib_amd/csrc/prover.hip
+++ b/plonky2-lib_amd/csrc/prover.hip
@@ -289,6 +289,13 @@
     out[0] = (m & 0x3FFFFFull) | (((m >> 22) & 0x3FFFFFull) << 32); out[1] = m >> 44;
     out[2] = (mp & 0x3FFFFFull) | (((mp >> 22) & 0x3FFFFFull) << 32); out[3] = mp >> 44;
 }
+inline void apx_words(u64 alpha, u32 nterms, u32 nw, u64 *out) {
+    const u64 ai = glf::inv(alpha);
+    u64 y = 1;
+    for (u32 m = 1; m <= nw; m++) { y = glf::mul(y, ai); apl_words(y, out + APL_WORDS * (size_t)(nw - m)); }
+    u64 x = 1;
+    for (u32 e = 0; e < nterms + nw; e++) { apl_words(x, out + APL_WORDS * (size_t)(nw + e)); x = glf::mul(x, alpha); }
+}
 __device__ __forceinline__ void acc3_zero(AccHL &a) { a.c0 = a.c1 = a.c2 = 0; }
 __device__ __forceinline__ void acc3_fma(AccHL &a, u64 v, const u64 *ml) {
     const u32 vlo = (u32)v, vhi = (u32)(v >> 32);
@@ -318,15 +325,16 @@
     u64 *out;
     const u64 *apow;
     const u64 *apl;
+    const u64 *apx;
     u64 betas[MAXCH], gammas[MAXCH], pih[4];
 };
-struct QBatch { const u64 *pp; size_t wl_stride, zl_stride, out_stride, apow_stride; };
+struct QBatch { const u64 *pp; size_t wl_stride, zl_stride, out_stride, apow_stride, apx_stride; };
 static_assert(MAXCH == 4, "pp layout: 4 betas, 4 gammas, 4 words of the public-input hash");
 __device__ __forceinline__ QProof q_proof(const QProof &p0, const QBatch &b) {
     QProof p = p0;
     if (b.pp) {
         const size_t k = blockIdx.z;
-        p.wl += k * b.wl_stride; p.zl += k * b.zl_stride; p.out += k * b.out_stride; p.apow += k * b.apow_stride; p.apl += APL_WORDS * k * b.apow_stride;
+        p.wl += k * b.wl_stride; p.zl += k * b.zl_stride; p.out += k * b.out_stride; p.apow += k * b.apow_stride; p.apl += APL_WORDS * k * b.apow_stride; p.apx += k * b.apx_stride;
         const u64 *q = b.pp + k * 3 * MAXCH;
         _Pragma("unroll") for (int c = 0; c < MAXCH; c++) { p.betas[c] = q[c]; p.gammas[c] = q[MAXCH + c]; p.pih[c] = q[2 * MAXCH + c]; }
     }
@@ -775,92 +783,107 @@
     }
 }
 
-constexpr int LIMB_SLOTS = 5, LIMB_GROUPS = 4;
-struct LimbArgs { const u64 *desc; u32 groups, num_wires; u32 count[LIMB_GROUPS], jlo[LIMB_GROUPS], jhi[LIMB_GROUPS]; u32 gi[LIMB_GROUPS][LIMB_SLOTS]; u32 extra_count, extra_gi[4]; };
+constexpr int LIMB_MAXG = 16, LIMB_MAXS = 7, LIMB_BATCH = 4;
+struct LimbArgs { const u64 *col, *ev; u32 count, jlo, jhi, num_wires; u32 gi[LIMB_MAXG]; u32 extra_count, extra_gi[4]; };
 inline void limb_args(const glp_circuit *cc, LimbArgs &la) {
-    la.desc = cc->dev_limb_desc; la.groups = cc->limb_groups; la.num_wires = cc->d.num_wires;
-    for (int g = 0; g < LIMB_GROUPS; g++) {
-        la.count[g] = cc->limb_gcount[g]; la.jlo[g] = cc->limb_jlo[g]; la.jhi[g] = cc->limb_jhi[g];
-        for (int i = 0; i < LIMB_SLOTS; i++) la.gi[g][i] = cc->limb_gi[g * LIMB_SLOTS + i];
-    }
+    la.col = cc->dev_limb_desc; la.ev = cc->dev_limb_desc + 2 * (size_t)cc->d.num_wires;
+    la.count = cc->limb_count; la.jlo = cc->limb_jlo; la.jhi = cc->limb_jhi; la.num_wires = cc->d.num_wires;
+    for (int g = 0; g < LIMB_MAXG; g++) la.gi[g] = cc->limb_gi[g];
+    la.extra_count = cc->limb_extra_count;
+    for (int i = 0; i < 4; i++) la.extra_gi[i] = cc->limb_extra_gi[i];
 }
 template <int NCH>
-__global__ __launch_bounds__(256, 2) void k_quotient_limbs(QArgs a, QProof p0, QBatch qb, LimbArgs la) {
+__global__ __launch_bounds__(256, 4) void k_quotient_limbs(QArgs a, QProof p0, QBatch qb, LimbArgs la) {
+    __shared__ u64 fl[LIMB_MAXG][256];
     const QProof p = q_proof(p0, qb);
     const size_t n = (size_t)1 << a.lg, N = n << a.rb;
     const size_t q = (size_t)blockIdx.x * 256 + threadIdx.x;
     if (q >= n) return;
     const u32 rq = blockIdx.y, r = rq * a.step;
     const size_t slot = (size_t)r * n + q;
-    const u32 k0 = (u32)NCH + (u32)NCH * (a.npp + 1), nt = a.nterms;
+    const u32 k0 = (u32)NCH + (u32)NCH * (a.npp + 1), nt = a.nterms, W0 = la.num_wires, xt = nt + 2 * W0;
     const u64 *W = p.wl + slot;
-    const u64 *ap = p.apl + APL_WORDS * (size_t)k0;
-    u64 acc[MAXCH];
-    _Pragma("unroll") for (int c = 0; c < NCH; c++) acc[c] = 0;
-#define LIMB_EMIT(S, K, V)                                                                                     \
-    do {                                                                                                       \
-        const u64 _v = (V);                                                                                    \
-        _Pragma("unroll") for (int c2 = 0; c2 < NCH; c2++) acc3_fma(ga[S][c2], _v, ap + APL_WORDS * ((size_t)c2 * nt + (K)));   \
-    } while (0)
-#pragma unroll 1
-    for (u32 grp = 0; grp < la.groups; grp++) {
-        const u32 gcount = la.count[grp], jlo = la.jlo[grp], jhi = la.jhi[grp];
-        const u64 *desc = la.desc + (size_t)grp * la.num_wires * LIMB_SLOTS;
-        AccHL ga[LIMB_SLOTS][MAXCH];
-        Base4Sum bs[LIMB_SLOTS];
-        _Pragma("unroll") for (int s = 0; s < LIMB_SLOTS; s++) {
-            b4_zero(bs[s]);
-            _Pragma("unroll") for (int c = 0; c < NCH; c++) acc3_zero(ga[s][c]);
-        }
-        _Pragma("unroll") for (int s = 0; s < LIMB_SLOTS; s++) {
-            if ((u32)s < gcount) {
-                const DevGate g = a.gates[la.gi[grp][s]];
-                switch (g.type) {
-                case GLP_GATE_U32_ARITHMETIC: gate_terms<NCH, GLP_GATE_U32_ARITHMETIC, true>(a, p, g, N, slot, k0, ga[s]); break;
-                case GLP_GATE_U32_ADD_MANY: gate_terms<NCH, GLP_GATE_U32_ADD_MANY, true>(a, p, g, N, slot, k0, ga[s]); break;
-                case GLP_GATE_U32_SUBTRACTION: gate_terms<NCH, GLP_GATE_U32_SUBTRACTION, true>(a, p, g, N, slot, k0, ga[s]); break;
-                default: break;
+    const u64 *ax = p.apx + APL_WORDS * (size_t)(W0 + k0);
+    const int tid = threadIdx.x;
+    for (u32 g = 0; g < la.count; g++) fl[g][tid] = gate_filter(a, a.gates[la.gi[g]], N, slot);
+    AccHL acc[NCH], pm[NCH], pp[NCH];
+    _Pragma("unroll") for (int c = 0; c < NCH; c++) { acc3_zero(acc[c]); acc3_zero(pm[c]); acc3_zero(pp[c]); }
+    Base4Sum bs[LIMB_MAXS];
+    _Pragma("unroll") for (int s = 0; s < LIMB_MAXS; s++) b4_zero(bs[s]);
+    const u32 jlo = la.jlo, jhi = la.jhi;
+    for (u32 j0 = jlo; j0 <= jhi; j0 += LIMB_BATCH) {
+        u64 lv[LIMB_BATCH];
+        _Pragma("unroll") for (int t = 0; t < LIMB_BATCH; t++) if (j0 + t <= jhi) lv[t] = W[(size_t)(j0 + t) * N];
+        _Pragma("unroll") for (int t = 0; t < LIMB_BATCH; t++) if (j0 + t <= jhi) {
+            const u32 j = j0 + t;
+            const u64 v = lv[t];
+            const u64 w0 = la.col[2 * (size_t)j], w1 = la.col[2 * (size_t)j + 1];
+            if (w0 & 0x300) {
+                const u64 rp = range_product(v, 4);
+                if (w0 & 0x100) _Pragma("unroll") for (int c = 0; c < NCH; c++) acc3_fma(pm[c], rp, ax + (long)APL_WORDS * ((long)c * xt - (long)k0 - (long)j));
+                if (w0 & 0x200) _Pragma("unroll") for (int c = 0; c < NCH; c++) acc3_fma(pp[c], rp, ax + (long)APL_WORDS * ((long)c * xt - (long)k0 + (long)j));
+            }
+            _Pragma("unroll") for (int s = 0; s < LIMB_MAXS; s++) {
+                if ((w0 >> s) & 1) {
+                    const u32 pos = (u32)(w1 >> (4 * s)) & 15u;
+                    if (pos == 0) { bs[s].lo = (u32)v; bs[s].hi = v >> 32; }
+                    else b4_add(bs[s], v, pos);
                 }
             }
-        }
-        for (u32 j0 = jlo; j0 <= jhi; j0 += 8) {
-            u64 lv[8];
-            _Pragma("unroll") for (int t = 0; t < 8; t++) if (j0 + t <= jhi) lv[t] = W[(size_t)(j0 + t) * N];
-            _Pragma("unroll") for (int t = 0; t < 8; t++) if (j0 + t <= jhi) {
-                const u64 v = lv[t];
-                const u64 *dj = desc + (size_t)(j0 + t) * LIMB_SLOTS;
-                const u64 rp = range_product(v, 4);
-                _Pragma("unroll") for (int s = 0; s < LIMB_SLOTS; s++) {
-                    const u64 d = dj[s];
-                    if (d & 1) {
-                        const u32 kl = (u32)(d >> 6) & 0x3FFu;
-                        _Pragma("unroll") for (int c2 = 0; c2 < NCH; c2++) acc3_fma(ga[s][c2], rp, ap + APL_WORDS * ((size_t)c2 * nt + kl));
-                        b4_add(bs[s], v, (u32)(d >> 1) & 15u);
-                        if (d & 32) {
-                            const u32 kf = (u32)(d >> 16) & 0x3FFu, ref = (u32)(d >> 26) & 0xFFu;
-                            LIMB_EMIT(s, kf, sub(b4_value(bs[s]), W[(size_t)ref * N]));
-                            b4_zero(bs[s]);
+            const u32 ne = (u32)(w0 >> 16) & 0xFFu;
+            if (ne) {
+                u64 rr[NCH];
+                u32 have = 0;
+                const u64 *ev = la.ev + (w0 >> 32);
+                for (u32 e = 0; e < ne; e++) {
+                    const u64 d = ev[e];
+                    const u32 kind = (u32)d & 3u, g = (u32)(d >> 3) & 31u;
+                    const int k = (int)((u32)(d >> 16) & 0xFFFFu) - 0x8000;
+                    const u64 f = fl[g][tid];
+                    if (kind == 0) {
+                        const u32 s = (u32)(d >> 8) & 15u, ref = (u32)(d >> 32) & 0xFFu;
+                        u64 b4 = 0;
+                        _Pragma("unroll") for (int s2 = 0; s2 < LIMB_MAXS; s2++) if ((u32)s2 == s) b4 = b4_value(bs[s2]);
+                        const u64 tv = mul(f, sub(b4, W[(size_t)ref * N]));
+                        _Pragma("unroll") for (int c = 0; c < NCH; c++) acc3_fma(acc[c], tv, ax + (long)APL_WORDS * ((long)c * xt + k));
+                    } else {
+                        if (kind != have) {
+                            _Pragma("unroll") for (int c = 0; c < NCH; c++) rr[c] = acc3_reduce(kind == 1 ? pm[c] : pp[c]);
+                            have = kind;
+                        }
+                        _Pragma("unroll") for (int c = 0; c < NCH; c++) {
+                            u64 tv = mul(f, rr[c]);
+                            if (d & 4) tv = neg(tv);
+                            acc3_fma(acc[c], tv, ax + (long)APL_WORDS * ((long)c * xt + k));
                         }
                     }
                 }
             }
         }
-        _Pragma("unroll") for (int s = 0; s < LIMB_SLOTS; s++) {
-            if ((u32)s < gcount) {
-                const u64 filter = gate_filter(a, a.gates[la.gi[grp][s]], N, slot);
-                _Pragma("unroll") for (int c = 0; c < NCH; c++) acc[c] = add(acc[c], mul(filter, acc3_reduce(ga[s][c])));
-            }
-        }
-    }
-#undef LIMB_EMIT
+    }
+    u64 res[MAXCH];
+    _Pragma("unroll") for (int c = 0; c < NCH; c++) res[c] = acc3_reduce(acc[c]);
+    for (u32 g = 0; g < la.count; g++) {
+        const DevGate gt = a.gates[la.gi[g]];
+        if (gt.type == GLP_GATE_U32_RANGE_CHECK) continue;
+        AccHL ga[MAXCH];
+        _Pragma("unroll") for (int c = 0; c < NCH; c++) acc3_zero(ga[c]);
+        switch (gt.type) {
+        case GLP_GATE_U32_ARITHMETIC: gate_terms<NCH, GLP_GATE_U32_ARITHMETIC, true>(a, p, gt, N, slot, k0, ga); break;
+        case GLP_GATE_U32_ADD_MANY: gate_terms<NCH, GLP_GATE_U32_ADD_MANY, true>(a, p, gt, N, slot, k0, ga); break;
+        default: gate_terms<NCH, GLP_GATE_U32_SUBTRACTION, true>(a, p, gt, N, slot, k0, ga); break;
+        }
+        const u64 f = fl[g][tid];
+        _Pragma("unroll") for (int c = 0; c < NCH; c++) res[c] = add(res[c], mul(f, acc3_reduce(ga[c])));
+    }
     for (u32 t = 0; t < la.extra_count; t++) {
         const DevGate g = a.gates[la.extra_gi[t]];
-        if (g.type == GLP_GATE_COMPARISON) gate_contrib<NCH, GLP_GATE_COMPARISON>(a, p, g, N, slot, k0, acc);
+        if (g.type == GLP_GATE_COMPARISON) gate_contrib<NCH, GLP_GATE_COMPARISON>(a, p, g, N, slot, k0, res);
     }
     const size_t Rq = (size_t)gridDim.y;
     _Pragma("unroll") for (int c = 0; c < NCH; c++) {
         u64 *o = p.out + ((size_t)c * Rq + rq) * n + q;
-        *o = add(*o, mul(acc[c], a.zh_inv[rq]));
+        *o = add(*o, mul(res[c], a.zh_inv[rq]));
     }
 }
 
@@ -1441,7 +1464,8 @@
         while ((1u << qdb) < qdf) qdb++;
         const u32 Rq = 1u << qdb, step = 1u << (rb - qdb);
         const u32 nchunks = npp + 1, nterms = nch + nch * nchunks + d.num_gate_constraints;
-        std::vector<u64> apow((size_t)(1 + APL_WORDS) * nch * nterms);
+        const u32 xt = nterms + 2 * d.num_wires;
+        std::vector<u64> apow((size_t)(1 + APL_WORDS) * nch * nterms + (size_t)APL_WORDS * nch * xt);
         for (u32 i = 0; i < nch; i++) {
             u64 x = 1;
             for (u32 k = 0; k < nterms; k++) {
@@ -1450,6 +1474,7 @@
                 apl_words(x, &apow[(size_t)nch * nterms + APL_WORDS * e]);
                 x = mul(x, alphas[i]);
             }
+            apx_words(alphas[i], nterms, d.num_wires, &apow[(size_t)(1 + APL_WORDS) * nch * nterms + (size_t)APL_WORDS * i * xt]);
         }
         u64 *dev_apow, *qv, *qV, *qc;
         GLP_TRY(tmp.get(&dev_apow, apow.size()));
@@ -1464,6 +1489,7 @@
         memset(&qbt, 0, sizeof(qbt));
         a.cs = cc->cs->lde; qp.wl = wb.b->lde; qp.zl = zb.b->lde; qp.out = qv;
         a.gates = cc->dev_gates; a.k_is = cc->dev_k_is; qp.apow = dev_apow; qp.apl = dev_apow + (size_t)nch * nterms; a.k_ratio = cc->k_ratio;
+        qp.apx = dev_apow + (size_t)(1 + APL_WORDS) * nch * nterms;
         for (u32 i = 0; i < nch; i++) { qp.betas[i] = betas[i]; qp.gammas[i] = gammas[i]; }
         memcpy(qp.pih, pih, 32);
         const u64 WN = root_of_unity(lg + rb), gn = pow(GEN, (u64)n), wR = root_of_unity(rb);
@@ -1502,8 +1528,6 @@
                 if (cc->limb_count) {
                     LimbArgs la;
                     limb_args(cc, la);
-                    la.extra_count = cc->limb_extra_count;
-                    for (int i = 0; i < 4; i++) la.extra_gi[i] = cc->limb_extra_gi[i];
                     hipLaunchKernelGGL(HIP_KERNEL_NAME(k_quotient_limbs<2>), dim3(nblk(n), Rq), dim3(256), 0, c->stream, a, qp, qbt, la);
                     GLP_HIP(hipGetLastError());
                 }
@@ -1830,47 +1854,15 @@
 
 static int build_quotient_plan(glp_ctx *c, glp_circuit *cc) {
     const glp_circuit_desc &d = cc->d;
-    std::vector<u64> desc((size_t)LIMB_GROUPS * d.num_wires * LIMB_SLOTS, 0);
-    for (int g = 0; g < LIMB_GROUPS; g++) { cc->limb_jlo[g] = d.num_wires; cc->limb_jhi[g] = 0; }
-    auto put = [&](u32 s, u32 col, u32 pos, u32 kl, bool flush, u32 kf, u32 ref) {
-        const u32 grp = s / LIMB_SLOTS, slot = s % LIMB_SLOTS;
-        desc[((size_t)grp * d.num_wires + col) * LIMB_SLOTS + slot] = 1ull | ((u64)pos << 1) | (flush ? 32ull : 0ull) | ((u64)kl << 6) | ((u64)kf << 16) | ((u64)ref << 26);
-        cc->limb_jlo[grp] = std::min(cc->limb_jlo[grp], col); cc->limb_jhi[grp] = std::max(cc->limb_jhi[grp], col);
-    };
+    const u32 W = d.num_wires;
     std::vector<u32> limb_list;
-    auto fill = [&](u32 s, u32 gi) {
-        const glp_gate &g = cc->gates[gi];
-        cc->limb_gi[s] = gi;
-        if (g.type == GLP_GATE_U32_ARITHMETIC) {
-            for (u32 i = 0; i < g.p0; i++)
-                for (u32 j = 0; j < 32; j++)
-                    put(s, 6 * g.p0 + 32 * i + j, j & 15, 36 * i + 2 + (31 - j), (j & 15) == 15, 36 * i + 34 + (j >> 4), 6 * i + 3 + (j >> 4));
-        } else if (g.type == GLP_GATE_U32_ADD_MANY) {
-            const u32 na = g.p0, nops = g.p1, wd = na + 3;
-            for (u32 i = 0; i < nops; i++)
-                for (u32 j = 0; j < 18; j++)
-                    put(s, wd * nops + 18 * i + j, j & 15, 21 * i + 1 + (17 - j), j == 15 || j == 17, 21 * i + 19 + (j >> 4), wd * i + na + 1 + (j >> 4));
-        } else if (g.type == GLP_GATE_U32_SUBTRACTION) {
-            for (u32 i = 0; i < g.p0; i++)
-                for (u32 j = 0; j < 16; j++)
-                    put(s, 5 * g.p0 + 16 * i + j, j, 19 * i + 1 + (15 - j), j == 15, 19 * i + 17, 5 * i + 3);
-        } else {
-            for (u32 i = 0; i < g.p0; i++)
-                for (u32 j = 0; j < 16; j++)
-                    put(s, g.p0 + 16 * i + j, j, 17 * i + 1 + j, j == 15, 17 * i, i);
-        }
-    };
-    auto limb_weight = [&](u32 gi) -> u32 {
-        const glp_gate &g = cc->gates[gi];
-        return g.type == GLP_GATE_U32_ARITHMETIC ? 32 * g.p0 : g.type == GLP_GATE_U32_ADD_MANY ? 18 * g.p1 : 16 * g.p0;
-    };
     for (u32 gi = 0; gi < d.num_gates; gi++) {
         const glp_gate &g = cc->gates[gi];
         const bool limb_gate = g.type == GLP_GATE_U32_ARITHMETIC || g.type == GLP_GATE_U32_ADD_MANY ||
                                g.type == GLP_GATE_U32_SUBTRACTION || g.type == GLP_GATE_U32_RANGE_CHECK;
         const bool light = g.type == GLP_GATE_CONSTANT || g.type == GLP_GATE_PUBLIC_INPUT || g.type == GLP_GATE_ARITHMETIC ||
                            g.type == GLP_GATE_BASE_SUM || g.type == GLP_GATE_RANDOM_ACCESS;
-        if (limb_gate && limb_list.size() < (size_t)(LIMB_SLOTS * LIMB_GROUPS) && d.num_wires <= 256) {
+        if (limb_gate && limb_list.size() < (size_t)LIMB_MAXG && W <= 256) {
             limb_list.push_back(gi);
         } else if (g.type == GLP_GATE_ARITHMETIC && cc->arith_ops == 0 && 4 * g.p0 <= d.num_routed_wires && d.quotient_degree_factor % 4 == 0 &&
                    d.num_selectors + 2 <= d.num_constants) {
@@ -1881,27 +1873,103 @@
             cc->single_gates.push_back(gi);
         }
     }
-    if (limb_list.size() == 1) {
-        cc->single_gates.push_back(limb_list[0]);
+    struct Win { u32 s, e, slot; };
+    struct Close { u32 win, g, kf, ref; };
+    struct Bound { u32 col, dir, sub, g; int k; };
+    std::vector<Win> wins;
+    std::vector<Close> closes;
+    std::vector<Bound> bounds;
+    std::vector<u32> rdir(W, 0);
+    u32 jlo = W, jhi = 0;
+    auto window = [&](u32 s, u32 e) -> u32 {
+        for (u32 i = 0; i < wins.size(); i++) if (wins[i].s == s && wins[i].e == e) return i;
+        wins.push_back({s, e, 0});
+        return (u32)wins.size() - 1;
+    };
+    auto op = [&](u32 t, u32 a, u32 len, u32 dir, int K, const u32 *kf, const u32 *ref) {
+        const u32 b = a + len - 1;
+        jlo = std::min(jlo, a); jhi = std::max(jhi, b);
+        for (u32 col = a; col <= b; col++) rdir[col] |= 1u << dir;
+        bounds.push_back({b, dir, 0, t, K});
+        if (a > 0) bounds.push_back({a - 1, dir, 1, t, K});
+        for (u32 w = 0, s = a; s <= b; w++, s += 16) closes.push_back({window(s, std::min(b, s + 15)), t, kf[w], ref[w]});
+    };
+    for (u32 t = 0; t < limb_list.size(); t++) {
+        const glp_gate &g = cc->gates[limb_list[t]];
+        if (g.type == GLP_GATE_U32_ARITHMETIC) {
+            for (u32 i = 0; i < g.p0; i++) {
+                const u32 kf[2] = {36 * i + 34, 36 * i + 35}, ref[2] = {6 * i + 3, 6 * i + 4};
+                op(t, 6 * g.p0 + 32 * i, 32, 0, (int)(36 * i + 33 + 6 * g.p0 + 32 * i), kf, ref);
+            }
+        } else if (g.type == GLP_GATE_U32_ADD_MANY) {
+            const u32 na = g.p0, nops = g.p1, wd = na + 3;
+            for (u32 i = 0; i < nops; i++) {
+                const u32 kf[2] = {21 * i + 19, 21 * i + 20}, ref[2] = {wd * i + na + 1, wd * i + na + 2};
+                op(t, wd * nops + 18 * i, 18, 0, (int)(21 * i + 18 + wd * nops + 18 * i), kf, ref);
+            }
+        } else if (g.type == GLP_GATE_U32_SUBTRACTION) {
+            for (u32 i = 0; i < g.p0; i++) {
+                const u32 kf[1] = {19 * i + 17}, ref[1] = {5 * i + 3};
+                op(t, 5 * g.p0 + 16 * i, 16, 0, (int)(19 * i + 16 + 5 * g.p0 + 16 * i), kf, ref);
+            }
+        } else {
+            for (u32 i = 0; i < g.p0; i++) {
+                const u32 kf[1] = {17 * i}, ref[1] = {i};
+                op(t, g.p0 + 16 * i, 16, 1, (int)(17 * i + 1) - (int)(g.p0 + 16 * i), kf, ref);
+            }
+        }
+    }
+    bool fits = limb_list.size() > 1;
+    {
+        std::vector<u32> order(wins.size());
+        for (u32 i = 0; i < order.size(); i++) order[i] = i;
+        std::stable_sort(order.begin(), order.end(), [&](u32 x, u32 y) { return wins[x].s < wins[y].s; });
+        std::vector<int> busy_until(LIMB_MAXS, -1);
+        for (u32 i : order) {
+            int s = 0;
+            while (s < LIMB_MAXS && busy_until[s] >= (int)wins[i].s) s++;
+            if (s == LIMB_MAXS) { fits = false; break; }
+            busy_until[s] = (int)wins[i].e; wins[i].slot = (u32)s;
+        }
+    }
+    std::vector<std::vector<u64>> evs(W);
+    if (fits) {
+        for (const Close &cl : closes)
+            evs[wins[cl.win].e].push_back((u64)wins[cl.win].slot << 8 | (u64)cl.g << 3 | (u64)(cl.kf + 0x8000u) << 16 | (u64)cl.ref << 32);
+        size_t terms = closes.size();
+        for (const Bound &bd : bounds) {
+            if (bd.col < jlo) continue;
+            evs[bd.col].push_back((u64)(1 + bd.dir) | (u64)bd.sub << 2 | (u64)bd.g << 3 | (u64)(u32)(bd.k + 0x8000) << 16);
+            terms++;
+        }
+        if (terms > ACC3_MAX_TERMS) fits = false;
+        for (std::vector<u64> &e : evs) {
+            if (e.size() > 255) fits = false;
+            std::stable_sort(e.begin(), e.end(), [](u64 x, u64 y) { return (x & 3) < (y & 3); });
+        }
+    }
+    if (!fits) {
+        for (u32 gi : limb_list) cc->single_gates.push_back(gi);
         limb_list.clear();
     }
     if (!limb_list.empty()) {
-        const u32 cnt = (u32)limb_list.size();
-        const u32 G = (cnt + LIMB_SLOTS - 1) / LIMB_SLOTS;
-        u32 used[LIMB_GROUPS] = {0, 0, 0, 0};
-        auto limb_start = [&](u32 gi) -> u32 {
-            const glp_gate &g = cc->gates[gi];
-            return g.type == GLP_GATE_U32_ARITHMETIC ? 6 * g.p0 : g.type == GLP_GATE_U32_ADD_MANY ? (g.p0 + 3) * g.p1 : g.type == GLP_GATE_U32_SUBTRACTION ? 5 * g.p0 : g.p0;
-        };
-        std::stable_sort(limb_list.begin(), limb_list.end(), [&](u32 x, u32 y) {
-            return limb_start(x) != limb_start(y) ? limb_start(x) < limb_start(y) : limb_weight(x) > limb_weight(y); });
-        for (u32 t = 0; t < cnt; t++) {
-            const u32 grp = t / LIMB_SLOTS;
-            fill(grp * LIMB_SLOTS + used[grp], limb_list[t]);
-            used[grp]++;
-        }
-        cc->limb_count = cnt; cc->limb_groups = G;
-        for (u32 g = 0; g < G; g++) cc->limb_gcount[g] = used[g];
+        std::vector<u64> prog(2 * (size_t)W, 0);
+        for (const Win &w : wins)
+            for (u32 col = w.s; col <= w.e; col++) {
+                prog[2 * col] |= 1ull << w.slot;
+                prog[2 * col + 1] |= (u64)(col - w.s) << (4 * w.slot);
+            }
+        std::vector<u64> flat;
+        for (u32 col = 0; col < W; col++) {
+            prog[2 * col] |= (u64)rdir[col] << 8;
+            prog[2 * col] |= (u64)evs[col].size() << 16 | (u64)flat.size() << 32;
+            flat.insert(flat.end(), evs[col].begin(), evs[col].end());
+        }
+        prog.insert(prog.end(), flat.begin(), flat.end());
+        cc->limb_count = (u32)limb_list.size(); cc->limb_jlo = jlo; cc->limb_jhi = jhi;
+        for (u32 t = 0; t < limb_list.size(); t++) cc->limb_gi[t] = limb_list[t];
+        GLP_TRY(c->alloc((void **)&cc->dev_limb_desc, prog.size() * 8));
+        GLP_TRY(h2d(c, cc->dev_limb_desc, prog.data(), prog.size() * 8));
     }
     if (cc->limb_count) {
         std::vector<u32> keep;
@@ -1910,10 +1978,6 @@
             else keep.push_back(gi);
         }
         cc->single_gates.swap(keep);
-    }
-    if (cc->limb_count) {
-        GLP_TRY(c->alloc((void **)&cc->dev_limb_desc, desc.size() * 8));
-        GLP_TRY(h2d(c, cc->dev_limb_desc, desc.data(), desc.size() * 8));
     }
     return GLP_OK;
 }
diff --git a/plonky2-lib_amd/csrc/prover_batch.inc b/plonky2-lib_amd/csrc/prover_batch.inc
--- a/plonky2-lib_amd/csrc/prover_batch.inc
+++ b/plonky2-lib_amd/csrc/prover_batch.inc
@@ -88,7 +88,8 @@
     const u32 Rq = 1u << qdb, step = 1u << (rb - qdb);
     const u32 nchunks = npp + 1, nterms = nch + nch * nchunks + d.num_gate_constraints;
     const size_t apn = (size_t)nch * nterms;
-    std::vector<u64> apow((size_t)(1 + APL_WORDS) * K * apn), qpp((size_t)K * 3 * MAXCH, 0);
+    const size_t apx = (size_t)nch * (nterms + 2 * d.num_wires);
+    std::vector<u64> apow((size_t)(1 + APL_WORDS) * K * apn + (size_t)APL_WORDS * K * apx), qpp((size_t)K * 3 * MAXCH, 0);
     pool.run(K, [&](size_t k) {
         memcpy(P((u32)k) + L.caps + capn * 4, &caps[k * capn * 4], (size_t)capn * 32);
         ch[k].observe_hashes(&caps[k * capn * 4], capn);
@@ -101,6 +102,7 @@
                 apl_words(x, &apow[(size_t)K * apn + APL_WORDS * e]);
                 x = mul(x, alpha);
             }
+            apx_words(alpha, nterms, d.num_wires, &apow[(size_t)(1 + APL_WORDS) * K * apn + APL_WORDS * (k * apx + (size_t)i * (nterms + 2 * d.num_wires))]);
         }
         for (u32 i = 0; i < nch; i++) { qpp[k * 3 * MAXCH + i] = chal[k * 2 * MAXCH + i]; qpp[k * 3 * MAXCH + MAXCH + i] = chal[k * 2 * MAXCH + MAXCH + i]; }
         memcpy(&qpp[k * 3 * MAXCH + 2 * MAXCH], &pih[4 * k], 32);
@@ -124,7 +126,9 @@
         memset(&qp, 0, sizeof(qp));
         a.cs = cc->cs->lde; a.gates = cc->dev_gates; a.k_is = cc->dev_k_is; a.k_ratio = cc->k_ratio;
         qp.wl = wb.b->lde; qp.zl = zb.b->lde; qp.out = qv; qp.apow = dev_apow; qp.apl = dev_apow + (size_t)K * apn;
+        qp.apx = dev_apow + (size_t)(1 + APL_WORDS) * K * apn;
         qbt.pp = dev_qpp; qbt.wl_stride = (size_t)nw * N; qbt.zl_stride = (size_t)nzp * N; qbt.out_stride = qstride; qbt.apow_stride = (size_t)nch * nterms;
+        qbt.apx_stride = APL_WORDS * apx;
         const u64 WN = root_of_unity(lg + rb), wR = root_of_unity(rb);
         for (u32 rq = 0; rq < Rq; rq++) {
             const u32 r = rq * step;
@@ -148,8 +152,6 @@
         if (cc->limb_count) {
             LimbArgs la;
             limb_args(cc, la);
-            la.extra_count = cc->limb_extra_count;
-            for (int i = 0; i < 4; i++) la.extra_gi[i] = cc->limb_extra_gi[i];
             hipLaunchKernelGGL(HIP_KERNEL_NAME(k_quotient_limbs<2>), g, dim3(256), 0, c->stream, a, qp, qbt, la);
             GLP_HIP(hipGetLastError());
         }
diff --git a/plonky2-lib_amd/csrc/prover_batch_dev.inc b/plonky2-lib_amd/csrc/prover_batch_dev.inc
--- a/plonky2-lib_amd/csrc/prover_batch_dev.inc
+++ b/plonky2-lib_amd/csrc/prover_batch_dev.inc
@@ -77,9 +77,10 @@
     const u32 nchunks = npp + 1, nterms = nch + nch * nchunks + d.num_gate_constraints;
     const size_t apn = (size_t)nch * nterms;
     u64 *dev_apow, *qv, *qV, *qc, *l0t;
-    GLP_TRY(tmp.get(&dev_apow, (size_t)(1 + APL_WORDS) * K * apn));
+    const size_t apx = (size_t)nch * (nterms + 2 * d.num_wires);
+    GLP_TRY(tmp.get(&dev_apow, (size_t)(1 + APL_WORDS) * K * apn + (size_t)APL_WORDS * K * apx));
     hipLaunchKernelGGL(k_tr_alphas, dim3(tgrid), dim3(256), 0, c->stream, g, zb.b->digests + 4 * cap_off, ndig * 4, L.caps + (size_t)capn * 4, nterms, dev_apow,
-                       dev_apow + (size_t)K * apn);
+                       dev_apow + (size_t)K * apn, d.num_wires, dev_apow + (size_t)(1 + APL_WORDS) * K * apn);
     GLP_HIP(hipGetLastError());
     mark("partial products + commit + transcript 2");
 
@@ -96,7 +97,9 @@
         memset(&qp, 0, sizeof(qp));
         a.cs = cc->cs->lde; a.gates = cc->dev_gates; a.k_is = cc->dev_k_is; a.k_ratio = cc->k_ratio;
         qp.wl = wb.b->lde; qp.zl = zb.b->lde; qp.out = qv; qp.apow = dev_apow; qp.apl = dev_apow + (size_t)K * apn;
+        qp.apx = dev_apow + (size_t)(1 + APL_WORDS) * K * apn;
         qbt.pp = dev_qpp; qbt.wl_stride = (size_t)nw * N; qbt.zl_stride = (size_t)nzp * N; qbt.out_stride = qstride; qbt.apow_stride = (size_t)nch * nterms;
+        qbt.apx_stride = APL_WORDS * apx;
         const u64 WN = root_of_unity(lg + rb), wR = root_of_unity(rb);
         for (u32 rq = 0; rq < Rq; rq++) {
             const u32 r = rq * step;
@@ -120,8 +123,6 @@
         if (cc->limb_count) {
             LimbArgs la;
             limb_args(cc, la);
-            la.extra_count = cc->limb_extra_count;
-            for (int i = 0; i < 4; i++) la.extra_gi[i] = cc->limb_extra_gi[i];
             hipLaunchKernelGGL(HIP_KERNEL_NAME(k_quotient_limbs<2>), gq, dim3(256), 0, c->stream, a, qp, qbt, la);
             GLP_HIP(hipGetLastError());
         }
diff --git a/plonky2-lib_amd/csrc/prover_types.h b/plonky2-lib_amd/csrc/prover_types.h
--- a/plonky2-lib_amd/csrc/prover_types.h
+++ b/plonky2-lib_amd/csrc/prover_types.h
@@ -33,7 +33,7 @@
     u64 *dev_sigmas = nullptr;
     u64 *dev_consts = nullptr;
     u64 *dev_limb_desc = nullptr;
-    u32 limb_count = 0, limb_groups = 0, limb_gcount[4] = {0, 0, 0, 0}, limb_gi[20] = {0}, limb_jlo[4] = {0, 0, 0, 0}, limb_jhi[4] = {0, 0, 0, 0};
+    u32 limb_count = 0, limb_gi[16] = {0}, limb_jlo = 0, limb_jhi = 0;
     u32 limb_extra_count = 0, limb_extra_gi[4] = {0, 0, 0, 0};
     u32 arith_gi = 0, arith_ops = 0;
     u32 light_count = 0, light_gi[8] = {0, 0, 0, 0, 0, 0, 0, 0};
diff --git a/plonky2-lib_amd/csrc/transcript_dev.h b/plonky2-lib_amd/csrc/transcript_dev.h
--- a/plonky2-lib_amd/csrc/transcript_dev.h
+++ b/plonky2-lib_amd/csrc/transcript_dev.h
@@ -93,27 +93,42 @@
     if (live && l == 0) { qk[2 * MAXCH] = pih0; qk[2 * MAXCH + 1] = pih1; qk[2 * MAXCH + 2] = pih2; qk[2 * MAXCH + 3] = pih3; }
     ds_store(s, dch, l, live);
 }
-__global__ __launch_bounds__(256) void k_tr_alphas(TrGeo g, const u64 *cap_b, size_t cap_stride, size_t caps_off, u32 nterms, u64 *apow, u64 *apl) {
-    TR_PROLOGUE;
-    DSponge s;
-    ds_load(s, dch, l);
-    tr_cap(s, cap_b + (size_t)k * cap_stride, img + caps_off, g.capn, live, l, gb);
+__device__ __forceinline__ void tr_apl(u64 x, u64 *o) {
+    const u64 mp = mul(x, 1ull << 32);
+    o[0] = (x & 0x3FFFFFull) | (((x >> 22) & 0x3FFFFFull) << 32); o[1] = x >> 44;
+    o[2] = (mp & 0x3FFFFFull) | (((mp >> 22) & 0x3FFFFFull) << 32); o[3] = mp >> 44;
+}
+__global__ __launch_bounds__(256) void k_tr_alphas(TrGeo g, const u64 *cap_b, size_t cap_stride, size_t caps_off, u32 nterms, u64 *apow, u64 *apl,
+                                                   u32 nw, u64 *apx) {
+    TR_PROLOGUE;
+    DSponge s;
+    ds_load(s, dch, l);
+    tr_cap(s, cap_b + (size_t)k * cap_stride, img + caps_off, g.capn, live, l, gb);
+    const u32 xt = nterms + 2 * nw;
     for (u32 i = 0; i < g.nch; i++) {
         const u64 alpha = ds_get(s, l, gb);
+        u64 *ox = apx + APL_WORDS * ((size_t)k * g.nch + i) * xt;
         u64 a16 = alpha;
 #pragma unroll
         for (int j = 0; j < 4; j++) a16 = sqr(a16);
         u64 x = tr_pow(alpha, (u64)l);
-        for (u32 t = (u32)l; t < nterms; t += 16) {
+        for (u32 t = (u32)l; t < nterms + nw; t += 16) {
             const size_t e = ((size_t)k * g.nch + i) * nterms + t;
             if (live) {
-                apow[e] = x;
-                const u64 mp = mul(x, 1ull << 32);
-                u64 *o = apl + APL_WORDS * e;
-                o[0] = (x & 0x3FFFFFull) | (((x >> 22) & 0x3FFFFFull) << 32); o[1] = x >> 44;
-                o[2] = (mp & 0x3FFFFFull) | (((mp >> 22) & 0x3FFFFFull) << 32); o[3] = mp >> 44;
+                if (t < nterms) { apow[e] = x; tr_apl(x, apl + APL_WORDS * e); }
+                if (nw) tr_apl(x, ox + APL_WORDS * (size_t)(nw + t));
             }
             x = mul(x, a16);
+        }
+        if (!nw) continue;
+        const u64 ai = inv(alpha);
+        u64 i16 = ai;
+#pragma unroll
+        for (int j = 0; j < 4; j++) i16 = sqr(i16);
+        u64 y = tr_pow(ai, (u64)l + 1);
+        for (u32 m = (u32)l + 1; m <= nw; m += 16) {
+            if (live) tr_apl(y, ox + APL_WORDS * (size_t)(nw - m));
+            y = mul(y, i16);
         }
     }
     ds_store(s, dch, l, live);
diff --git a/plonky2-lib_amd/csrc/verifier.hip b/plonky2-lib_amd/csrc/verifier.hip
--- a/plonky2-lib_amd/csrc/verifier.hip
+++ b/plonky2-lib_amd/csrc/verifier.hip
@@ -751,7 +751,7 @@
         const size_t cap4 = (size_t)capn * 4;
         hipLaunchKernelGGL(k_tr_begin, tg, tb, 0, c->stream, g, cc->digest[0], cc->digest[1], cc->digest[2], cc->digest[3], L.pis, d.num_public_inputs,
                            dev_proofs + L.caps, L.total, L.caps, dev_chal, dev_qpp);
-        hipLaunchKernelGGL(k_tr_alphas, tg, tb, 0, c->stream, g, dev_proofs + L.caps + cap4, L.total, L.caps + cap4, 2u, dev_apow, dev_apl);
+        hipLaunchKernelGGL(k_tr_alphas, tg, tb, 0, c->stream, g, dev_proofs + L.caps + cap4, L.total, L.caps + cap4, 2u, dev_apow, dev_apl, 0u, nullptr);
         hipLaunchKernelGGL(k_tr_zeta, tg, tb, 0, c->stream, g, dev_proofs + L.caps + 2 * cap4, L.total, L.caps + 2 * cap4, d.degree_bits,
                            root_of_unity((int)d.degree_bits), dev_zetas, dev_err);
         OpenGeo og;
```
